# oooolga/Ctrl-V

Hardware: AMD Instinct MI355X
Metric: denoising steps/sec, SVD+ControlNet 25f 576x1024 (higher is better)
Workload: dtype bf16; 1 GPU; box2video: ControlNet + UNet forward, CFG batch 2, 25 frames, latent 72x128, 25-step Karras Euler schedule, random-init SVD-XT weights; clips_per_gpu=1, parallelism=clip-shard x1, hip_graph=True

## Files before the change

ctrlv_amd/_lib.py:

```python
import ctypes
import os
import threading

_HERE = os.path.dirname(os.path.abspath(__file__))
LIB_PATH = os.path.join(_HERE, "lib", "libctrlv_hip.so")
LIB_PATH_F16 = os.path.join(_HERE, "lib", "libctrlv_hip_f16.so")

c_void_p, c_int, c_float, c_size_t = ctypes.c_void_p, ctypes.c_int32, ctypes.c_float, ctypes.c_size_t


class GemmDesc(ctypes.Structure):
    _fields_ = [
        ("A", c_void_p), ("A2", c_void_p), ("W", c_void_p), ("out", c_void_p),
        ("bias", c_void_p), ("R1", c_void_p), ("R2", c_void_p), ("V", c_void_p),
        ("M", c_int), ("N", c_int), ("Cin", c_int), ("taps", c_int),
        ("lda", c_int), ("lda2", c_int), ("c_split", c_int),
        ("mode", c_int),
        ("H", c_int), ("Wd", c_int), ("Ho", c_int), ("Wo", c_int), ("stride", c_int), ("up", c_int),
        ("F", c_int), ("S", c_int),
        ("ldo", c_int), ("n_store", c_int),
        ("ldr1", c_int), ("ldr2", c_int),
        ("s_acc", c_float), ("s1", c_float), ("s2", c_float),
        ("vmode", c_int), ("vdiv", c_int), ("vmod", c_int), ("vS", c_int), ("ldv", c_int),
        ("act", c_int), ("geglu", c_int), ("out_f32", c_int), ("tile", c_int),
# ... 30 lines not shown

class TemporalFusedDesc(ctypes.Structure):
    _fields_ = [
        ("x", c_void_p), ("ldx", c_int), ("wf", c_void_p), ("bias", c_void_p),
        ("R1", c_void_p), ("R1_lo", c_void_p), ("ldr1", c_int),
        ("V", c_void_p), ("vmode", c_int), ("vdiv", c_int), ("vmod", c_int), ("vS", c_int), ("ldv", c_int),
        ("out", c_void_p), ("out_lo", c_void_p), ("ldo", c_int),
        ("B", c_int), ("F", c_int), ("S", c_int), ("C", c_int),
        ("ln_gamma", c_void_p), ("ln_beta", c_void_p), ("ln_eps", c_float),
    ]


class SpatialEntryDesc(ctypes.Structure):
    _fields_ = [
        ("x", c_void_p), ("x_lo", c_void_p), ("ldx", c_int), ("wf", c_void_p),
        ("bias_in", c_void_p), ("bias_qkv", c_void_p), ("stats", c_void_p),
        ("gn_gamma", c_void_p), ("gn_beta", c_void_p),
        ("ln_gamma", c_void_p), ("ln_beta", c_void_p), ("ln_eps", c_float),
        ("h0", c_void_p), ("h0_lo", c_void_p), ("ldh", c_int),
        ("qkv", c_void_p), ("ldq", c_int),
        ("n_img", c_int), ("S", c_int), ("C", c_int), ("head_dim", c_int),
        ("q_scale", c_float),
    ]


class LoraDesc(ctypes.Structure):
    _fields_ = [
        ("X", c_void_p), ("dY", c_void_p), ("A", c_void_p), ("B", c_void_p), ("dA", c_void_p), ("dB", c_void_p),
        ("M", c_int), ("Cin", c_int), ("N", c_int), ("g", c_int), ("r", c_int), ("ldx", c_int), ("ldy", c_int),
        ("scale", c_float),
    ]


class TensorDesc(ctypes.Structure):
    _fields_ = [("name", ctypes.c_char_p), ("data", c_void_p), ("dtype", c_int), ("on_device", c_int),
                ("numel", ctypes.c_int64)]


class GemmTokensDesc(ctypes.Structure):
    _fields_ = [
        ("A", c_void_p), ("W", c_void_p), ("bias", c_void_p), ("R1", c_void_p), ("out", c_void_p),
        ("workspace", c_void_p), ("workspace_bytes", c_size_t),
        ("M", c_int), ("N", c_int), ("K", c_int), ("lda", c_int), ("ldr1", c_int), ("ldo", c_int),
        ("act", c_int), ("ws_zeroed", c_int),
    ]


class ClipConfig(ctypes.Structure):
    _fields_ = [
        ("hidden_size", c_int), ("intermediate_size", c_int), ("num_hidden_layers", c_int), ("num_attention_heads", c_int),
        ("image_size", c_int), ("patch_size", c_int), ("projection_dim", c_int), ("hidden_act", c_int),
        ("layer_norm_eps", c_float),
    ]


class VaeConfig(ctypes.Structure):
    _fields_ = [
        ("in_channels", c_int), ("out_channels", c_int), ("latent_channels", c_int), ("layers_per_block", c_int),
        ("n_blocks", c_int), ("block_out_channels", c_int * CTRLV_MAX_BLOCKS), ("scaling_factor", c_float),
        ("offset_limit_bytes", ctypes.c_int64),
    ]


class ClipRequest(ctypes.Structure):
    _fields_ = [
        ("n_clips", c_int), ("num_frames", c_int), ("height", c_int), ("width", c_int),
        ("image_u8", c_void_p), ("cond", c_void_p), ("cond_channels", c_int), ("cond_dtype", c_int),
        ("aug_noise", c_void_p), ("noise_aug_strength", c_float), ("num_steps", c_int),
        ("latents", c_void_p), ("sigmas", ctypes.POINTER(c_float)), ("timesteps", ctypes.POINTER(c_float)),
        ("fps", c_int), ("motion_bucket_id", c_int),
        ("min_guidance", c_float), ("max_guidance", c_float), ("conditioning_scale", c_float), ("decode_chunk", c_int),
        ("clip_mean", c_float * 3), ("clip_std", c_float * 3),
        ("out_latents", c_void_p), ("out_frames", c_void_p), ("out_frames_u8", c_void_p),
    ]


class BoxCondition(ctypes.Structure):
    _fields_ = [("frames", c_void_p), ("channels", c_int), ("dtype", c_int), ("num_cond_frames", c_int), ("reserved", c_int)]


class TwoStageRequest(ctypes.Structure):
    _fields_ = [("boxes", ClipRequest), ("box_cond", BoxCondition), ("video", ClipRequest), ("out_box_frames_u8", c_void_p),
                ("clean_threshold", c_float), ("reserved", c_int)]


class SeedRequest(ctypes.Structure):
    _fields_ = [("seed", ctypes.c_uint64), ("clip_index0", ctypes.c_uint32), ("call", ctypes.c_uint32),
                ("src_image_u8", c_void_p), ("src_height", c_int), ("src_width", c_int),
                ("sigma_min", c_float), ("sigma_max", c_float),
                ("sigmas_host", ctypes.POINTER(c_float)), ("timesteps_host", ctypes.POINTER(c_float)), ("reserved", c_int)]


class BestBoxesRequest(ctypes.Structure):
    _fields_ = [("n_candidates", c_int), ("reserved", c_int), ("candidates", ctypes.POINTER(ClipRequest)),
                ("box_cond", BoxCondition), ("gt_u8", c_void_p), ("clean_threshold", c_float), ("reserved2", c_int),
                ("out_pt", c_void_p), ("out_cond", c_void_p), ("out_u8", c_void_p), ("out_counts", c_void_p),
                ("out_winner", c_void_p)]


class BestChainRequest(ctypes.Structure):
    _fields_ = [("boxes", BestBoxesRequest), ("video", ClipRequest), ("reserved", c_int)]


class TrainBatchRequest(ctypes.Structure):
    _fields_ = [
        ("n_clips", c_int), ("num_frames", c_int), ("height", c_int), ("width", c_int),
        ("clips", c_void_p), ("box_frames", c_void_p), ("clips_dtype", c_int), ("box_dtype", c_int),
        ("mode", c_int), ("num_cond_frames", c_int), ("dropout_prob", ctypes.c_double),
        ("seed", ctypes.c_uint64), ("clip_index0", ctypes.c_uint32), ("call", ctypes.c_uint32),
        ("sigma_table", c_void_p), ("timestep_table", c_void_p), ("table_size", c_int), ("scaling_factor", c_float),
        ("clip_mean", c_float * 3), ("clip_std", c_float * 3), ("sample_dtype", c_int), ("reserved", c_int),
        ("target_latents", c_void_p), ("noisy_latents", c_void_p), ("sample", c_void_p), ("control_cond", c_void_p),
        ("encoder_hidden_states", c_void_p), ("sigmas", c_void_p), ("timesteps", c_void_p), ("indices", c_void_p),
        ("random_p", c_void_p), ("noise", c_void_p),
    ]


SIGNATURES = {
    "ctrlv_abi_version": (c_int, []),
    "ctrlv_elem_dtype": (c_int, []),
    "ctrlv_build_id": (c_int, [ctypes.c_char_p, c_size_t]),
    "ctrlv_last_error": (c_int, [ctypes.c_char_p, c_size_t]),
    "ctrlv_gemm": (c_int, [ctypes.POINTER(GemmDesc), c_void_p]),
    "ctrlv_gemm_gn_partials_serves": (c_int, [ctypes.POINTER(GemmDesc)]),
    "ctrlv_gemm_splitk_ws_bytes": (c_size_t, [ctypes.POINTER(GemmDesc)]),
    "ctrlv_gemm_up_phase_serves": (c_int, [ctypes.POINTER(GemmDesc)]),
    "ctrlv_pack_up_phase_weight": (c_int, [c_void_p, c_int, c_int, c_int, c_void_p, c_void_p]),
    "ctrlv_groupnorm_from_partials": (c_int, [c_void_p, c_int, c_int, c_int, c_int, c_float, c_void_p, c_void_p, c_void_p,
                                              c_int, c_void_p, c_void_p]),
    "ctrlv_groupnorm_from_partials_split": (c_int, [c_void_p, c_void_p, c_int, c_int, c_int, c_int, c_float, c_void_p, c_void_p, c_void_p,
                                              c_int, c_void_p, c_void_p]),
    "ctrlv_groupnorm_chunks": (c_int, [c_int, c_int, c_int, c_int]),
    "ctrlv_groupnorm_stats_split": (c_int, [c_void_p, c_void_p, c_void_p, c_void_p, c_int, c_int, c_int, c_int, c_int, c_float,
                                            c_void_p, c_void_p]),
    "ctrlv_groupnorm_apply_split": (c_int, [c_void_p, c_void_p, c_void_p, c_void_p, c_int, c_int, c_int, c_int, c_int, c_void_p,
                                            c_void_p, c_void_p, c_int, c_void_p, c_void_p]),
    "ctrlv_layernorm_split": (c_int, [c_void_p, c_void_p, c_int, c_int, c_void_p, c_void_p, c_float, c_void_p, c_int, c_int,
                                      c_int, c_void_p, c_void_p]),
    "ctrlv_axpby_split": (c_int, [c_void_p, c_void_p, c_void_p, c_float, c_float, c_void_p, c_void_p, c_size_t, c_void_p]),
    "ctrlv_plan_set_trunk_mode": (c_int, [c_void_p, c_int]),
    "ctrlv_plan_set_ff_precision": (c_int, [c_void_p, c_int]),
    "ctrlv_groupnorm_stats": (c_int, [c_void_p, c_void_p, c_int, c_int, c_int, c_int, c_int, c_float, c_void_p,
                                      c_void_p]),
    "ctrlv_groupnorm_apply": (c_int, [c_void_p, c_void_p, c_int, c_int, c_int, c_int, c_int, c_void_p, c_void_p,
                                      c_void_p, c_int, c_void_p, c_void_p]),
    "ctrlv_layernorm": (c_int, [c_void_p, c_int, c_int, c_void_p, c_void_p, c_float, c_void_p, c_int, c_int, c_int,
                                c_void_p, c_void_p]),
    "ctrlv_softmax_rows": (c_int, [c_void_p, c_int, c_int, ctypes.c_long, c_void_p, ctypes.c_long, c_void_p]),
    "ctrlv_softmax_rows_bwd": (c_int, [c_void_p, ctypes.c_long, c_void_p, ctypes.c_long, c_int, c_int, c_float, c_void_p,
                                       ctypes.c_long, c_void_p]),
    "ctrlv_ff_fused_w1f_bytes": (c_int, []),
    "ctrlv_ff_fused_pack": (c_int, [c_void_p, c_void_p, c_void_p, c_void_p, c_void_p, c_void_p]),
    "ctrlv_ff_fused_serves": (c_int, [ctypes.POINTER(GemmDesc), c_int]),
    "ctrlv_ff_fused": (c_int, [c_void_p, c_int, c_void_p, c_void_p, ctypes.POINTER(GemmDesc), c_void_p]),
    "ctrlv_ff_fused_ln": (c_int, [c_void_p, c_int, c_void_p, c_void_p, c_float, c_void_p, c_int, c_int, c_int, c_void_p,
                                  c_void_p, ctypes.POINTER(GemmDesc), c_void_p]),
    "ctrlv_quant_rows_f8": (c_int, [c_void_p, c_int, c_int, c_int, c_void_p, c_void_p, c_float, c_void_p, c_int, c_int, c_int,
                                    c_void_p, c_int, c_void_p, c_void_p]),
    "ctrlv_gemm_f8": (c_int, [ctypes.POINTER(GemmDesc), c_void_p, c_void_p, c_void_p]),
    "ctrlv_gemm_f8_serves": (c_int, [ctypes.POINTER(GemmDesc)]),
    "ctrlv_temporal_fused_weight_bytes": (c_size_t, []),
    "ctrlv_temporal_fused_pack": (c_int, [c_void_p, c_int, c_void_p, c_int, c_void_p, c_void_p]),
    "ctrlv_temporal_fused": (c_int, [ctypes.POINTER(TemporalFusedDesc), c_void_p]),
    "ctrlv_temporal_fused_serves": (c_int, [ctypes.POINTER(TemporalFusedDesc)]),
    "ctrlv_spatial_entry_fused_weight_bytes": (c_size_t, []),
    "ctrlv_spatial_entry_fused_pack": (c_int, [c_void_p, c_int, c_void_p, c_int, c_void_p, c_void_p]),
    "ctrlv_spatial_entry_fused": (c_int, [ctypes.POINTER(SpatialEntryDesc), c_void_p]),
    "ctrlv_spatial_entry_fused_serves": (c_int, [ctypes.POINTER(SpatialEntryDesc)]),
    "ctrlv_groupnorm_finalize": (c_int, [c_int, c_int, c_int, c_int, c_float, c_void_p, c_void_p]),
    "ctrlv_attention_spatial": (c_int, [c_void_p, c_void_p, c_int, c_int, c_int, c_void_p]),
    "ctrlv_attention_spatial_prescaled": (c_int, [c_void_p, c_void_p, c_int, c_int, c_int, c_void_p]),
    "ctrlv_attention_temporal": (c_int, [c_void_p, c_void_p, c_int, c_int, c_int, c_int, c_void_p]),
    "ctrlv_attention_spatial_lse": (c_int, [c_void_p, c_void_p, c_void_p, c_int, c_int, c_int, c_void_p]),
    "ctrlv_attention_bwd_scratch_floats": (ctypes.c_size_t, [c_int, c_int, c_int]),
    "ctrlv_attention_spatial_bwd": (c_int, [c_void_p, c_void_p, c_void_p, c_void_p, c_void_p, c_void_p, c_int, c_int, c_int,
                                            c_void_p]),
    "ctrlv_attention_temporal_bwd": (c_int, [c_void_p, c_void_p, c_void_p, c_void_p, c_int, c_int, c_int, c_int, c_void_p]),
    "ctrlv_attention_tokens": (c_int, [c_void_p, c_void_p, c_int, c_int, c_int, c_int, c_void_p]),
    "ctrlv_clip_patch_rows": (c_int, [c_void_p, c_int, c_int, c_int, c_int, c_int, c_void_p, c_int, c_void_p]),
    "ctrlv_clip_tokens": (c_int, [c_void_p, c_void_p, c_void_p, c_int, c_int, c_int, c_void_p, c_void_p]),
    "ctrlv_act_rows": (c_int, [c_void_p, c_int, c_int, c_int, c_int, c_void_p]),
    "ctrlv_gemm_tokens": (c_int, [ctypes.POINTER(GemmTokensDesc), c_void_p]),
    "ctrlv_gemm_tokens_plan": (c_int, [c_int, c_int, ctypes.POINTER(c_int), ctypes.POINTER(c_int)]),
    "ctrlv_gemm_tokens_ws_bytes": (c_size_t, [c_int, c_int, c_int]),
    "ctrlv_nchw_to_rows": (c_int, [c_void_p, c_int, c_int, c_int, c_int, c_void_p, c_int, c_int, c_void_p]),
    "ctrlv_rows_to_nchw": (c_int, [c_void_p, c_int, c_int, c_int, c_int, c_void_p, c_int, c_void_p]),
    "ctrlv_time_conv_rows_to_nchw": (c_int, [c_void_p, c_int, c_int, c_int, c_int, c_void_p, c_void_p, c_void_p, c_int,
                                             c_void_p]),
    "ctrlv_vae_posterior": (c_int, [c_void_p, c_int, c_int, c_int, c_int, c_void_p, c_void_p, c_void_p, c_float, c_void_p,
                                    c_void_p, c_int, c_void_p]),
    "ctrlv_time_conv_rows_to_nchw_bwd": (c_int, [c_void_p, c_void_p, c_int, c_int, c_int, c_int, c_int, c_void_p, c_void_p,
                                                 c_int, c_void_p, c_void_p, c_void_p, c_void_p]),
    "ctrlv_im2col3x3": (c_int, [c_void_p, c_int, c_int, c_int, c_int, c_void_p, c_int, c_void_p]),
    "ctrlv_axpby": (c_int, [c_void_p, c_void_p, c_float, c_float, c_void_p, c_size_t, c_void_p]),
    "ctrlv_timestep_embedding": (c_int, [c_void_p, c_int, c_int, c_void_p, c_void_p]),
    "ctrlv_silu": (c_int, [c_void_p, c_void_p, c_size_t, c_void_p]),
    "ctrlv_cfg_euler_step": (c_int, [c_void_p, c_void_p, c_int, c_int, c_void_p, c_int, c_int, c_int, c_float,
                                     c_float, c_void_p, c_void_p]),
    "ctrlv_pack_weight": (c_int, [c_void_p, c_int, c_int, c_int, c_int, c_int, c_int, c_void_p, c_int, c_void_p]),
    "ctrlv_gemm_wgrad_scratch_bytes": (c_size_t, [ctypes.POINTER(GemmDesc)]),
    "ctrlv_gemm_wgrad": (c_int, [ctypes.POINTER(GemmDesc), c_void_p, c_int, c_void_p, c_void_p, c_float, c_int, c_void_p, c_size_t,
                                 c_void_p]),
    "ctrlv_colsum_scratch_floats": (c_size_t, [c_int, c_int, c_int, c_int]),
    "ctrlv_colsum": (c_int, [c_void_p, c_int, c_int, c_int, c_int, c_int, c_int, c_float, c_void_p, c_int, c_void_p, c_void_p]),
    "ctrlv_dot_diff": (c_int, [c_void_p, c_void_p, c_void_p, c_size_t, c_float, c_void_p, c_void_p, c_void_p]),
    "ctrlv_groupnorm_bwd_scratch_floats": (c_int, [c_int, c_int, c_int, c_int]),
    "ctrlv_groupnorm_bwd": (c_int, [c_void_p, c_void_p, c_int, c_int, c_int, c_int, c_void_p, c_void_p, c_void_p, c_int,
                                    c_void_p, c_void_p, c_void_p, c_void_p, c_void_p]),
    "ctrlv_groupnorm_bwd_add": (c_int, [c_void_p, c_void_p, c_void_p, c_int, c_int, c_int, c_int, c_void_p, c_void_p, c_void_p, c_int,
                                        c_void_p, c_void_p, c_void_p, c_void_p, c_void_p]),
    "ctrlv_layernorm_bwd_add": (c_int, [c_void_p, c_void_p, c_void_p, c_int, c_int, c_void_p, c_float, c_void_p, c_int, c_int, c_int,
                                        c_void_p, c_void_p, c_void_p, c_void_p, c_void_p]),
    "ctrlv_layernorm_bwd_scratch_floats": (ctypes.c_size_t, [c_int, c_int]),
    "ctrlv_layernorm_bwd": (c_int, [c_void_p, c_void_p, c_int, c_int, c_void_p, c_float, c_void_p, c_int, c_int, c_int,
                                    c_void_p, c_void_p, c_void_p, c_void_p, c_void_p]),
    "ctrlv_geglu_bwd": (c_int, [c_void_p, c_void_p, c_size_t, c_int, c_void_p, c_void_p]),
    "ctrlv_lora_grad_scratch_bytes": (c_size_t, [ctypes.POINTER(LoraDesc)]),
    "ctrlv_lora_grad": (c_int, [ctypes.POINTER(LoraDesc), c_void_p, c_size_t, c_void_p]),
    "ctrlv_lora_merge": (c_int, [c_void_p, c_int, c_void_p, c_void_p, c_int, c_int, c_int, c_float, c_void_p, c_void_p]),
    "ctrlv_plan_create": (c_int, [ctypes.POINTER(ModelConfig), c_int, ctypes.POINTER(c_void_p)]),
    "ctrlv_plan_load_weights": (c_int, [c_void_p, ctypes.POINTER(TensorDesc), c_size_t]),
    "ctrlv_plan_set_time_context_order": (c_int, [c_void_p, c_int]),
    "ctrlv_plan_workspace_bytes": (c_size_t, [c_void_p, c_int, c_int, c_int, c_int]),
    "ctrlv_plan_num_down_residuals": (c_int, [c_void_p]),
    "ctrlv_plan_residual_shape": (c_int, [c_void_p, c_int, c_int, c_int, c_int, c_int, ctypes.POINTER(ctypes.c_int64),
                                          ctypes.POINTER(c_int)]),
    "ctrlv_unet_forward": (c_int, [c_void_p, c_void_p, c_int, c_void_p, c_int, c_void_p, c_void_p, c_int,
                                   ctypes.POINTER(c_void_p), c_void_p, c_void_p, c_void_p, c_int, c_int, c_int, c_int,
                                   c_void_p, c_size_t, c_void_p]),
    "ctrlv_unet_encoder_forward": (c_int, [c_void_p, c_void_p, c_int, c_void_p, c_int, c_void_p, c_void_p, c_int,
                                           ctypes.POINTER(c_void_p), c_void_p, c_int, c_int, c_int, c_int, c_void_p,
                                           c_size_t, c_void_p]),
    "ctrlv_controlnet_forward": (c_int, [c_void_p, c_void_p, c_void_p, c_int, c_void_p, c_int, c_void_p, c_void_p, c_int,
                                         c_float, ctypes.POINTER(c_void_p), c_void_p, c_int, c_int, c_int, c_int, c_void_p,
                                         c_size_t, c_void_p]),
    "ctrlv_plan_destroy": (c_int, [c_void_p]),
    "ctrlv_plan_profile": (c_int, [c_void_p, c_int]),
    "ctrlv_plan_profile_read": (c_int, [c_void_p, ctypes.POINTER(ProfileRecord), c_int]),
    "ctrlv_clip_plan_create": (c_int, [ctypes.POINTER(ClipConfig), c_int, ctypes.POINTER(c_void_p)]),
    "ctrlv_clip_plan_load_weights": (c_int, [c_void_p, ctypes.POINTER(TensorDesc), c_size_t]),
    "ctrlv_clip_plan_workspace_bytes": (c_size_t, [c_void_p, c_int]),
    "ctrlv_clip_forward": (c_int, [c_void_p, c_void_p, c_int, c_int, c_void_p, c_void_p, c_void_p, c_size_t, c_void_p]),
    "ctrlv_clip_plan_destroy": (c_int, [c_void_p]),
    "ctrlv_vae_plan_create": (c_int, [ctypes.POINTER(VaeConfig), c_int, ctypes.POINTER(c_void_p)]),
    "ctrlv_vae_plan_load_weights": (c_int, [c_void_p, ctypes.POINTER(TensorDesc), c_size_t]),
    "ctrlv_vae_plan_workspace_bytes": (c_size_t, [c_void_p, c_int, c_int, c_int, c_int, c_int]),
    "ctrlv_vae_encode": (c_int, [c_void_p, c_void_p, c_int, c_int, c_int, c_int, c_void_p, c_float, c_void_p, c_void_p, c_int,
                                 c_void_p, c_size_t, c_void_p]),
    "ctrlv_vae_decode": (c_int, [c_void_p, c_void_p, c_int, c_int, c_int, c_int, c_int, c_void_p, c_int, c_void_p, c_size_t,
                                 c_void_p]),
    "ctrlv_vae_plan_destroy": (c_int, [c_void_p]),
    "ctrlv_resize_antialias": (c_int, [c_void_p, c_int, c_int, c_int, c_int, c_void_p, c_int, c_int, c_int,
                                       ctypes.POINTER(c_float), ctypes.POINTER(c_float), c_void_p]),
    "ctrlv_pixels_prepare": (c_int, [c_void_p, c_void_p, c_float, c_int, c_int, c_int, c_void_p, c_void_p]),
    "ctrlv_frames_to_u8": (c_int, [c_void_p, c_int, c_int, c_int, c_void_p, c_void_p]),
    "ctrlv_pipeline_create": (c_int, [c_void_p, c_void_p, c_void_p, c_void_p, c_int, ctypes.POINTER(c_void_p)]),
    "ctrlv_pipeline_set_overlap": (c_int, [c_void_p, c_int]),
    "ctrlv_pipeline_workspace_bytes": (c_size_t, [c_void_p, ctypes.POINTER(ClipRequest)]),
    "ctrlv_pipeline_generate": (c_int, [c_void_p, ctypes.POINTER(ClipRequest), c_void_p, c_size_t, c_void_p]),
    "ctrlv_pipeline_destroy": (c_int, [c_void_p]),
    "ctrlv_pipeline_boxes_workspace_bytes": (c_size_t, [c_void_p, ctypes.POINTER(ClipRequest), ctypes.POINTER(BoxCondition)]),
    "ctrlv_pipeline_predict_boxes": (c_int, [c_void_p, ctypes.POINTER(ClipRequest), ctypes.POINTER(BoxCondition), c_void_p,
                                             c_size_t, c_void_p]),
    "ctrlv_box_frames_post_ws_bytes": (c_size_t, [c_int, c_int]),
    "ctrlv_box_frames_post": (c_int, [c_void_p, c_int, c_int, c_int, c_int, c_float, c_void_p, c_void_p, c_void_p, c_void_p,
                                      c_size_t, c_void_p]),
    "ctrlv_mask_counts": (c_int, [c_void_p, c_void_p, c_int, c_int, c_int, c_int, c_void_p, c_void_p]),
    "ctrlv_pipeline_chain_workspace_bytes": (c_size_t, [c_void_p, c_void_p, ctypes.POINTER(TwoStageRequest)]),
    "ctrlv_pipeline_boxes_to_video": (c_int, [c_void_p, c_void_p, ctypes.POINTER(TwoStageRequest), c_void_p, c_size_t, c_void_p]),
    "ctrlv_randn": (c_int, [ctypes.c_uint64, ctypes.c_uint32, ctypes.c_uint32, ctypes.c_uint32, c_int, c_size_t, c_float, c_int,
                            c_void_p, c_int, c_void_p]),
    "ctrlv_euler_schedule": (c_int, [c_int, c_float, c_float, ctypes.POINTER(c_float), ctypes.POINTER(c_float),
                                     ctypes.POINTER(ctypes.c_double)]),
    "ctrlv_resize_lanczos_ws_bytes": (c_size_t, [c_int, c_int, c_int, c_int, c_int]),
    "ctrlv_resize_lanczos_u8": (c_int, [c_void_p, c_int, c_int, c_int, c_void_p, c_int, c_int, c_void_p, c_size_t, c_void_p]),
    "ctrlv_pipeline_prepare_bytes": (c_size_t, [c_void_p, ctypes.POINTER(ClipRequest), ctypes.POINTER(SeedRequest)]),
    "ctrlv_pipeline_prepare": (c_int, [c_void_p, ctypes.POINTER(ClipRequest), ctypes.POINTER(SeedRequest),
                                       ctypes.POINTER(ClipRequest), c_void_p, c_size_t, c_void_p]),
    "ctrlv_pipeline_seeded_workspace_bytes": (c_size_t, [c_void_p, ctypes.POINTER(ClipRequest), ctypes.POINTER(SeedRequest)]),
    "ctrlv_pipeline_generate_seeded": (c_int, [c_void_p, ctypes.POINTER(ClipRequest), ctypes.POINTER(SeedRequest), c_void_p,
                                               c_size_t, c_void_p]),
    "ctrlv_best_candidate": (c_int, [c_void_p, c_int, c_int, c_void_p, c_void_p]),
    "ctrlv_gather_clips": (c_int, [c_void_p, c_void_p, c_int, c_int, c_size_t, c_void_p, c_void_p]),
    "ctrlv_pipeline_best_boxes_workspace_bytes": (c_size_t, [c_void_p, ctypes.POINTER(BestBoxesRequest)]),
    "ctrlv_pipeline_best_boxes": (c_int, [c_void_p, ctypes.POINTER(BestBoxesRequest), c_void_p, c_size_t, c_void_p]),
    "ctrlv_pipeline_best_chain_workspace_bytes": (c_size_t, [c_void_p, c_void_p, ctypes.POINTER(BestChainRequest)]),
    "ctrlv_pipeline_best_boxes_to_video": (c_int, [c_void_p, c_void_p, ctypes.POINTER(BestChainRequest), c_void_p, c_size_t,
                                                   c_void_p]),
    "ctrlv_boundary_radius": (c_int, [c_int, c_int, ctypes.c_double]),
    "ctrlv_boundary_counts": (c_int, [c_void_p, c_void_p, c_int, c_int, c_int, c_int, c_int, c_int, c_void_p, c_void_p]),
    "ctrlv_frame_stats": (c_int, [c_void_p, c_void_p, c_int, c_int, c_int, c_int, c_void_p, c_void_p]),
    "ctrlv_frame_ssim_ws_bytes": (c_size_t, [c_int, c_int, c_int, c_int]),
    "ctrlv_frame_ssim": (c_int, [c_void_p, c_void_p, c_int, c_int, c_int, c_int, c_void_p, c_void_p, c_void_p, c_size_t, c_void_p]),
    "ctrlv_resize_frames_ws_bytes": (c_size_t, [c_int, c_int, c_int, c_int, c_int, c_int]),
    "ctrlv_resize_frames_u8": (c_int, [c_void_p, c_int, c_int, c_int, c_void_p, c_int, c_int, c_int, c_void_p, c_size_t, c_void_p]),
    "ctrlv_lpips_im2col_split": (c_int, [c_void_p, c_int, c_int, c_int, c_int, c_int, c_int, c_int, c_int, c_void_p, c_void_p]),
    "ctrlv_lpips_pack_weight": (c_int, [c_void_p, c_int, c_int, c_int, c_int, c_int, c_void_p, c_void_p]),
    "ctrlv_relu_maxpool_rows": (c_int, [c_void_p, c_int, c_int, c_int, c_int, c_int, c_void_p, c_int, c_void_p]),
    "ctrlv_lpips_distance_blocks": (c_int, [c_int]),
    "ctrlv_lpips_layer_distance": (c_int, [c_void_p, c_void_p, c_int, c_void_p, c_int, c_int, c_int, c_void_p, c_void_p]),
    "ctrlv_lpips_finish": (c_int, [c_void_p, c_int, c_int, ctypes.POINTER(c_int), c_void_p, c_void_p]),
    "ctrlv_lpips_plan_create": (c_int, [c_int, ctypes.POINTER(c_void_p)]),
    "ctrlv_lpips_plan_load_weights": (c_int, [c_void_p, ctypes.POINTER(TensorDesc), c_size_t]),
    "ctrlv_lpips_ws_bytes": (c_size_t, [c_void_p, c_int, c_int, c_int]),
    "ctrlv_lpips_frames": (c_int, [c_void_p, c_void_p, c_void_p, c_int, c_int, c_int, c_int, c_int, c_void_p, c_void_p, c_size_t,
                                   c_void_p]),
    "ctrlv_lpips_plan_destroy": (c_int, [c_void_p]),
    "ctrlv_resize_antialias_clamped": (c_int, [c_void_p, c_int, c_int, c_int, c_int, c_void_p, c_int, c_int, c_int,
                                               ctypes.POINTER(c_float), ctypes.POINTER(c_float), c_void_p]),
    "ctrlv_train_draws": (c_int, [ctypes.c_uint64, ctypes.c_uint32, ctypes.c_uint32, c_int, c_void_p, c_void_p, c_int,
                                  ctypes.c_double, c_void_p, c_void_p, c_void_p, c_void_p, c_void_p, c_void_p, c_void_p]),
    "ctrlv_train_assemble": (c_int, [c_void_p, c_void_p, c_void_p, c_void_p, c_void_p, c_void_p, c_int, c_int, c_int, c_int, c_int,
                                     c_int, c_int, ctypes.c_uint64, ctypes.c_uint32, ctypes.c_uint32, c_void_p, c_void_p, c_int,
                                     c_void_p, c_void_p]),
    "ctrlv_train_batch_workspace_bytes": (c_size_t, [c_void_p, c_void_p, ctypes.POINTER(TrainBatchRequest)]),
    "ctrlv_train_batch_prepare": (c_int, [c_void_p, c_void_p, ctypes.POINTER(TrainBatchRequest), c_void_p, c_size_t, c_void_p]),
    "ctrlv_adamw_step": (c_int, [c_void_p, c_void_p, c_void_p, c_void_p, c_void_p, c_size_t, c_float, c_float, c_float, c_float,
                                 c_float, c_float, c_float, c_float, c_float, c_void_p]),
    "ctrlv_ema_step": (c_int, [c_void_p, c_void_p, c_size_t, c_float, c_void_p]),
    "ctrlv_grad_sumsq_partials": (c_size_t, [c_size_t]),
    "ctrlv_grad_sumsq": (c_int, [c_void_p, c_size_t, c_void_p, c_size_t, c_size_t, c_void_p]),
    "ctrlv_grad_finish": (c_int, [c_void_p, c_size_t, c_float, c_float, c_void_p, c_void_p]),
    "ctrlv_adamw_step_dev": (c_int, [c_void_p, c_void_p, c_void_p, c_void_p, c_void_p, c_size_t, c_float, c_float, c_float, c_float,
                                     c_float, c_float, c_float, c_float, c_float, c_void_p, c_void_p]),
    "ctrlv_grad_finish_scaled": (c_int, [c_void_p, c_size_t, c_float, c_float, c_void_p, c_void_p, c_void_p]),
    "ctrlv_adamw_step_scaled": (c_int, [c_void_p, c_void_p, c_void_p, c_void_p, c_void_p, c_size_t, c_float, c_float, c_float, c_float,
                                        c_float, c_float, c_float, c_float, c_void_p, c_void_p, c_void_p]),
}

_libs = {}
_tls = threading.local()
_NO_STATUS = {"ctrlv_abi_version", "ctrlv_elem_dtype", "ctrlv_build_id", "ctrlv_last_error", "ctrlv_ff_fused_w1f_bytes",
              "ctrlv_gemm_gn_partials_serves", "ctrlv_gemm_up_phase_serves", "ctrlv_ff_fused_serves", "ctrlv_plan_num_down_residuals",
              "ctrlv_temporal_fused_serves", "ctrlv_gemm_f8_serves", "ctrlv_spatial_entry_fused_serves",
              "ctrlv_gemm_tokens_ws_bytes", "ctrlv_clip_plan_workspace_bytes", "ctrlv_vae_plan_workspace_bytes",
              "ctrlv_pipeline_workspace_bytes", "ctrlv_pipeline_boxes_workspace_bytes", "ctrlv_box_frames_post_ws_bytes",
              "ctrlv_pipeline_chain_workspace_bytes", "ctrlv_resize_lanczos_ws_bytes", "ctrlv_pipeline_prepare_bytes",
              "ctrlv_pipeline_seeded_workspace_bytes", "ctrlv_pipeline_best_boxes_workspace_bytes",
              "ctrlv_pipeline_best_chain_workspace_bytes", "ctrlv_frame_ssim_ws_bytes", "ctrlv_resize_frames_ws_bytes",
              "ctrlv_train_batch_workspace_bytes", "ctrlv_lpips_ws_bytes",
              "ctrlv_lpips_distance_blocks",
              "ctrlv_boundary_radius"}


def _status_recorder(lib, fn):
    def call(*args):
        rc = fn(*args)
        _tls.failed = lib if rc < 0 else None
        return rc
    call.__name__ = getattr(fn, "__name__", "ctrlv_fn")
    return call
ABI_VERSION = 22


class CtrlvHipError(RuntimeError):
    pass


def source_build_id():
    import hashlib
    csrc = os.path.join(_HERE, "csrc")
    inc = os.path.join(os.path.dirname(_HERE), "include")
    if not os.path.isdir(csrc) or not os.path.isdir(inc):
        return None
    files = [os.path.join(csrc, f) for f in sorted(os.listdir(csrc)) if f.endswith((".hip", ".h"))]
    files += [os.path.join(inc, f) for f in sorted(os.listdir(inc)) if f.endswith(".h")]
    h = hashlib.sha256()
    for f in files:
        h.update(os.path.basename(f).encode() + b"\0")
        h.update(open(f, "rb").read())
    return h.hexdigest()[:16]


def build_id(lib=None):
    buf = ctypes.create_string_buffer(128)
    (lib or load()).ctrlv_build_id(buf, 128)
    return buf.value.decode()


def elem_code(dtype=None):
    if dtype is None or dtype == 2:
        return 2
    if dtype == 1:
        return 1
    name = str(dtype)
    if name == "torch.float16":
        return 1
    if name == "torch.bfloat16":
        return 2
    raise CtrlvHipError(f"ctrlv_amd: activations are stored as bf16 or fp16, not {dtype}")


def load(dtype=None):
    code = elem_code(dtype)
    lib = _libs.get(code)
    if lib is not None:
        return lib
    env = "CTRLV_HIP_LIB" if code == 2 else "CTRLV_HIP_LIB_F16"
    path = os.environ.get(env, LIB_PATH if code == 2 else LIB_PATH_F16)
    if not os.path.exists(path):
        raise CtrlvHipError(
            f"{path} not found: build it with `python -c 'import __graft_entry__ as g; g.build()'` "
            "(hipcc --offload-arch=gfx950).  ctrlv_amd has no CPU / eager fallback.")
    lib = ctypes.CDLL(path)
    for name, (res, args) in SIGNATURES.items():
        fn = getattr(lib, name)
        fn.restype, fn.argtypes = res, args
        if res is c_int and name not in _NO_STATUS:
            setattr(lib, name, _status_recorder(lib, fn))
    if lib.ctrlv_abi_version() != ABI_VERSION:
        raise CtrlvHipError(f"{path}: ABI version {lib.ctrlv_abi_version()}, this host layer needs {ABI_VERSION}")
    if lib.ctrlv_elem_dtype() != code:
        raise CtrlvHipError(f"{path}: element dtype code {lib.ctrlv_elem_dtype()}, expected {code}")
    want = source_build_id()
    if want is not None and env not in os.environ and build_id(lib) != want:
        raise CtrlvHipError(f"{path} is stale: built from sources {build_id(lib)}, tree is {want}; rebuild with "
                            "`python -c 'import __graft_entry__ as g; g.build()'`")
    _libs[code] = lib
    return lib


def last_error(lib=None):
    buf = ctypes.create_string_buffer(512)
    if lib is not None:
        lib.ctrlv_last_error(buf, 512)
        return buf.value.decode("utf-8", "replace")
    msgs = []
    for l in (_libs.values() or [load()]):
        l.ctrlv_last_error(buf, 512)
        if buf.value:
            msgs.append(buf.value.decode("utf-8", "replace"))
    return " | ".join(msgs)


def check(rc, what, lib=None):
    if rc == 0:
        return
    failed, _tls.failed = getattr(_tls, "failed", None), None
    msg = f"{what}: {last_error(lib or failed)} (status {rc})"
    if rc in (-1, -2, -4, -5):
        raise ValueError(msg)
    raise CtrlvHipError(msg)
```

ctrlv_amd/csrc/abi.hip:

```cpp
#include <stdarg.h>
#include <stdlib.h>

#include <mutex>

#include "common.h"

#ifndef CTRLV_BUILD_ID
#define CTRLV_BUILD_ID "unstamped"
#endif

static thread_local char g_err[512] = "";
void ctrlv_set_error(const char* fmt, ...) {
  va_list ap;
  va_start(ap, fmt);
  vsnprintf(g_err, sizeof(g_err), fmt, ap);
  va_end(ap);
}

const ctrlv_debug_t& ctrlv_debug() {
  static const ctrlv_debug_t dbg = [] {
    auto env = [](const char* name, int dflt) { const char* e = getenv(name); return e ? atoi(e) : dflt; };
    ctrlv_debug_t d;
    d.w16 = env("CTRLV_W16", 1);
    d.splitk = env("CTRLV_SPLITK", 1);
    d.force_tile = env("CTRLV_GEMM_FORCE_TILE", 0);
    d.conv_halo = env("CTRLV_CONV_HALO", 1);
    d.gn_fused = env("CTRLV_GN_FUSED", 1);
    d.gn_cross = env("CTRLV_GN_CROSS", 1);
    d.gn_rev = env("CTRLV_GN_REV", 1);
    d.gn_rows = env("CTRLV_GN_ROWS", 256);
    if (d.gn_rows < 32 || d.gn_rows > 1024) d.gn_rows = 256;
    d.ln_rows = env("CTRLV_LN_ROWS", 1);
    d.ff_fused = env("CTRLV_FF_FUSED", 1);
    d.ff_ln = env("CTRLV_FF_LN", 0);
    d.pp_balanced = env("CTRLV_PP_BALANCED", 1);
    d.pp_cgrp = env("CTRLV_PP_CGRP", 0);
    d.attn_rows = env("CTRLV_ATTN_ROWS", 0);
    d.temporal_fused = env("CTRLV_TEMPORAL_FUSED", 1);
    d.wgrad_pp = env("CTRLV_WGRAD_PP", 1);
    d.wgrad_slabs = env("CTRLV_WGRAD_SLABS", 0);
    d.up_phase = env("CTRLV_UP_PHASE", 1);
    d.spatial_entry = env("CTRLV_SPATIAL_ENTRY", 1);
    return d;
  }();
  return dbg;
}

int ctrlv_current_device() {
  int dev = 0;
  if (hipGetDevice(&dev) != hipSuccess || dev < 0 || dev >= CTRLV_MAX_DEVICES) dev = 0;
  return dev;
}

int ctrlv_num_cu(int dev) {
  static int cu[CTRLV_MAX_DEVICES] = {};
  static std::mutex mu;
  std::lock_guard<std::mutex> lk(mu);
  if (cu[dev] == 0) {
    int n = 0;
    if (hipDeviceGetAttribute(&n, hipDeviceAttributeMultiprocessorCount, dev) != hipSuccess || n <= 0) n = 256;
    cu[dev] = n;
  }
  return cu[dev];
}

extern "C" int ctrlv_last_error(char* buf, size_t n) {
  if (buf && n) {
    strncpy(buf, g_err, n - 1);
    buf[n - 1] = 0;
  }
  return (int)strlen(g_err);
}

extern "C" int ctrlv_abi_version(void) { return 22; }
static_assert(sizeof(ctrlv_gemm_desc) == 264 && offsetof(ctrlv_gemm_desc, ld_raw) == 192 && offsetof(ctrlv_gemm_desc, pad_br) == 196 &&
                  offsetof(ctrlv_gemm_desc, raw_out) == 200,
              "ctrlv_gemm_desc layout changed: that is an ABI bump");
extern "C" int ctrlv_elem_dtype(void) { return CTRLV_ELEM_DTYPE; }

extern "C" int ctrlv_build_id(char* buf, size_t n) {
  static const char marker[] = "CTRLV_BUILD_ID=" CTRLV_BUILD_ID;
  const char* id = marker + 15;
  if (buf && n) {
    strncpy(buf, id, n - 1);
    buf[n - 1] = 0;
  }
  return (int)strlen(id);
}
```

ctrlv_amd/csrc/common.h:

```cpp
#pragma once
#include <hip/hip_runtime.h>
#include <stdint.h>
#include <stdio.h>
#include <string.h>

#include "../../include/ctrlv_hip.h"

#ifdef CTRLV_ELEM_F16
typedef _Float16 el_native_t;
#define CTRLV_ELEM_DTYPE 1
#define CTRLV_MFMA_32x32x16_ASM "v_mfma_f32_32x32x16_f16"
#else
typedef __bf16 el_native_t;
#define CTRLV_ELEM_DTYPE 2
#define CTRLV_MFMA_32x32x16_ASM "v_mfma_f32_32x32x16_bf16"
#endif
typedef __attribute__((ext_vector_type(8))) el_native_t elx8;
typedef __attribute__((ext_vector_type(4))) el_native_t elx4;
typedef __attribute__((ext_vector_type(2))) el_native_t elx2;
typedef __attribute__((ext_vector_type(16))) float f32x16;
typedef __attribute__((ext_vector_type(4))) float f32x4;
typedef __attribute__((ext_vector_type(4))) short s16x4;
typedef uint16_t el_t;
typedef uint16_t bf16_t;

#define LDS_PTR(p) ((__attribute__((address_space(3))) void*)(p))
#define GLB_PTR(p) ((const __attribute__((address_space(1))) void*)(p))

static __device__ __attribute__((aligned(256), used)) unsigned char g_ctrlv_zeros[256];

__device__ __forceinline__ f32x16 mfma_32x32x16(const elx8& a, const elx8& b, const f32x16& c) {
#ifdef CTRLV_ELEM_F16
  return __builtin_amdgcn_mfma_f32_32x32x16_f16(a, b, c, 0, 0, 0);
#else
  return __builtin_amdgcn_mfma_f32_32x32x16_bf16(a, b, c, 0, 0, 0);
#endif
}

__device__ __forceinline__ float bf16_to_f32(bf16_t v) { return __uint_as_float(((uint32_t)v) << 16); }
__device__ __forceinline__ bf16_t f32_to_bf16(float f) {
  __bf16 b = (__bf16)f;
  return __builtin_bit_cast(bf16_t, b);
}
#ifdef CTRLV_ELEM_F16
__device__ __forceinline__ float el_to_f32(el_t v) { return (float)__builtin_bit_cast(_Float16, v); }
__device__ __forceinline__ el_t f32_to_el(float f) { return __builtin_bit_cast(el_t, (_Float16)f); }
__device__ __forceinline__ uint32_t pack_elx2(float lo, float hi) {
  typedef _Float16 h2 __attribute__((ext_vector_type(2)));
  const h2 v = {(_Float16)lo, (_Float16)hi};
  return __builtin_bit_cast(uint32_t, v);
}
__device__ __forceinline__ void unpack_elx8(const uint4& v, float* f) {
  typedef _Float16 h2 __attribute__((ext_vector_type(2)));
  const h2 a = __builtin_bit_cast(h2, v.x), b = __builtin_bit_cast(h2, v.y), c = __builtin_bit_cast(h2, v.z),
           d = __builtin_bit_cast(h2, v.w);
  f[0] = (float)a.x; f[1] = (float)a.y; f[2] = (float)b.x; f[3] = (float)b.y;
  f[4] = (float)c.x; f[5] = (float)c.y; f[6] = (float)d.x; f[7] = (float)d.y;
}
#else
__device__ __forceinline__ float el_to_f32(el_t v) { return bf16_to_f32(v); }
__device__ __forceinline__ el_t f32_to_el(float f) { return f32_to_bf16(f); }
__device__ __forceinline__ uint32_t pack_elx2(float lo, float hi) {
  typedef __bf16 b2 __attribute__((ext_vector_type(2)));
  const b2 v = {(__bf16)lo, (__bf16)hi};
  return __builtin_bit_cast(uint32_t, v);
}
__device__ __forceinline__ void unpack_elx8(const uint4& v, float* f) {
  f[0] = __uint_as_float(v.x << 16); f[1] = __uint_as_float(v.x & 0xffff0000u);
  f[2] = __uint_as_float(v.y << 16); f[3] = __uint_as_float(v.y & 0xffff0000u);
  f[4] = __uint_as_float(v.z << 16); f[5] = __uint_as_float(v.z & 0xffff0000u);
  f[6] = __uint_as_float(v.w << 16); f[7] = __uint_as_float(v.w & 0xffff0000u);
}
#endif
__device__ __forceinline__ float el_lo_f32(uint32_t v) { return el_to_f32((el_t)(v & 0xffffu)); }
__device__ __forceinline__ float el_hi_f32(uint32_t v) { return el_to_f32((el_t)(v >> 16)); }
__device__ __forceinline__ uint4 pack_elx8(const float* f) {
  uint4 v;
  v.x = pack_elx2(f[0], f[1]); v.y = pack_elx2(f[2], f[3]);
  v.z = pack_elx2(f[4], f[5]); v.w = pack_elx2(f[6], f[7]);
  return v;
}
typedef uint8_t lo_t;
__device__ __forceinline__ uint2 split_lo8(const float* v, const uint4& hi) {
#pragma clang fp contract(off)
  float h[8], dl[8];
  unpack_elx8(hi, h);
#pragma unroll
  for (int e = 0; e < 8; ++e) dl[e] = v[e] - h[e];
  int w0 = 0, w1 = 0;
  w0 = __builtin_amdgcn_cvt_pk_bf8_f32(dl[0], dl[1], w0, false);
  w0 = __builtin_amdgcn_cvt_pk_bf8_f32(dl[2], dl[3], w0, true);
  w1 = __builtin_amdgcn_cvt_pk_bf8_f32(dl[4], dl[5], w1, false);
  w1 = __builtin_amdgcn_cvt_pk_bf8_f32(dl[6], dl[7], w1, true);
  return make_uint2((unsigned)w0, (unsigned)w1);
}
__device__ __forceinline__ lo_t split_lo1(float v, el_t hi) {
#pragma clang fp contract(off)
  const float dl = v - el_to_f32(hi);
  return (lo_t)(__builtin_amdgcn_cvt_pk_bf8_f32(dl, 0.f, 0, false) & 0xff);
}
__device__ __forceinline__ void unpack_lo4(unsigned w, float* l) {
  typedef float f32x2_lo __attribute__((ext_vector_type(2)));
  const f32x2_lo a = __builtin_amdgcn_cvt_pk_f32_bf8((int)w, false), b = __builtin_amdgcn_cvt_pk_f32_bf8((int)w, true);
  l[0] = a.x; l[1] = a.y; l[2] = b.x; l[3] = b.y;
}
__device__ __forceinline__ unsigned pack_lo4(float l0, float l1, float l2, float l3) {
  int w = 0;
  w = __builtin_amdgcn_cvt_pk_bf8_f32(l0, l1, w, false);
  w = __builtin_amdgcn_cvt_pk_bf8_f32(l2, l3, w, true);
  return (unsigned)w;
}
__device__ __forceinline__ void unpack_lo8(const uint2& lo, float* l) {
  typedef float f32x2_lo __attribute__((ext_vector_type(2)));
  const f32x2_lo a = __builtin_amdgcn_cvt_pk_f32_bf8((int)lo.x, false), b = __builtin_amdgcn_cvt_pk_f32_bf8((int)lo.x, true);
  const f32x2_lo c = __builtin_amdgcn_cvt_pk_f32_bf8((int)lo.y, false), d = __builtin_amdgcn_cvt_pk_f32_bf8((int)lo.y, true);
  l[0] = a.x; l[1] = a.y; l[2] = b.x; l[3] = b.y; l[4] = c.x; l[5] = c.y; l[6] = d.x; l[7] = d.y;
}
__device__ __forceinline__ void add_lo8(float* f, const uint2& lo) {
#pragma clang fp contract(off)
  float l[8];
  unpack_lo8(lo, l);
#pragma unroll
  for (int e = 0; e < 8; ++e) f[e] = f[e] + l[e];
}

__device__ __forceinline__ float silu_f(float x) {
  return x * __builtin_amdgcn_rcpf(1.0f + __builtin_amdgcn_exp2f(-1.44269504088896340736f * x));
}
typedef float f32x2_t __attribute__((ext_vector_type(2)));
typedef float f32x4_t __attribute__((ext_vector_type(4)));
__device__ __forceinline__ f32x4_t fma4(f32x4_t a, f32x4_t b, f32x4_t c) {
  f32x4_t r;
  r.x = __builtin_fmaf(a.x, b.x, c.x); r.y = __builtin_fmaf(a.y, b.y, c.y);
  r.z = __builtin_fmaf(a.z, b.z, c.z); r.w = __builtin_fmaf(a.w, b.w, c.w);
  return r;
}
__device__ __forceinline__ f32x4_t splat4(float v) { return f32x4_t{v, v, v, v}; }
__device__ __forceinline__ f32x4_t gelu_phi4(f32x4_t x) {
#pragma clang fp contract(off)
  f32x4_t xc;
  xc.x = __builtin_amdgcn_fmed3f(x.x, -5.0f, 5.0f);
  xc.y = __builtin_amdgcn_fmed3f(x.y, -5.0f, 5.0f);
  xc.z = __builtin_amdgcn_fmed3f(x.z, -5.0f, 5.0f);
  xc.w = __builtin_amdgcn_fmed3f(x.w, -5.0f, 5.0f);
  const f32x4_t t = fma4(xc * xc, splat4(0.08f), splat4(-1.0f));
  f32x4_t p = fma4(t, splat4(7.353763795e-04f), splat4(-1.676730928e-03f));
  p = fma4(p, t, splat4(1.374596148e-03f));
  p = fma4(p, t, splat4(-2.526916796e-03f));
  p = fma4(p, t, splat4(6.766527425e-03f));
  p = fma4(p, t, splat4(-1.130712498e-02f));
  p = fma4(p, t, splat4(1.623608917e-02f));
  p = fma4(p, t, splat4(-2.321312763e-02f));
  p = fma4(p, t, splat4(3.147675842e-02f));
  p = fma4(p, t, splat4(-4.045128077e-02f));
  p = fma4(p, t, splat4(5.151792988e-02f));
  p = fma4(p, t, splat4(-7.029590756e-02f));
  p = fma4(p, t, splat4(1.413638145e-01f));
  return fma4(xc, p, splat4(0.5f));
}
__device__ __forceinline__ f32x4_t gelu_erf4(f32x4_t x) {
#pragma clang fp contract(off)
  return x * gelu_phi4(x);
}
__device__ __forceinline__ float gelu_phi1(float x) {
#pragma clang fp contract(off)
  const float xc = __builtin_amdgcn_fmed3f(x, -5.0f, 5.0f);
  const float t = __builtin_fmaf(xc * xc, 0.08f, -1.0f);
  float p = __builtin_fmaf(t, 7.353763795e-04f, -1.676730928e-03f);
  p = __builtin_fmaf(p, t, 1.374596148e-03f);
  p = __builtin_fmaf(p, t, -2.526916796e-03f);
  p = __builtin_fmaf(p, t, 6.766527425e-03f);
  p = __builtin_fmaf(p, t, -1.130712498e-02f);
  p = __builtin_fmaf(p, t, 1.623608917e-02f);
  p = __builtin_fmaf(p, t, -2.321312763e-02f);
  p = __builtin_fmaf(p, t, 3.147675842e-02f);
  p = __builtin_fmaf(p, t, -4.045128077e-02f);
  p = __builtin_fmaf(p, t, 5.151792988e-02f);
  p = __builtin_fmaf(p, t, -7.029590756e-02f);
  p = __builtin_fmaf(p, t, 1.413638145e-01f);
  return __builtin_fmaf(xc, p, 0.5f);
}

constexpr int kGeluTabN = 1024;
constexpr int kGeluTabBytes = kGeluTabN * 8;
__device__ __forceinline__ void gelu_table_fill(char* tab, int tid, int nthreads) {
#pragma clang fp contract(off)
  for (int i = tid; i < kGeluTabN; i += nthreads) {
    const float a = gelu_phi1(__builtin_fmaf((float)i, 0.01f, -5.12f));
    const float b = gelu_phi1(__builtin_fmaf((float)(i + 1), 0.01f, -5.12f));
    *(float2*)(tab + i * 8) = make_float2(a, b - a);
  }
}
__device__ __forceinline__ float gelu_phi_tab(float x, const char* tab) {
#pragma clang fp contract(off)
  float t = __builtin_fmaf(x, 100.0f, 512.0f);
  t = __builtin_amdgcn_fmed3f(t, 0.0f, 1023.99994f);
  const float fr = __builtin_amdgcn_fractf(t);
  const int i = (int)t;
  const float2 e = *(const float2*)(tab + i * 8);
  return __builtin_fmaf(fr, e.y, e.x);
}
__device__ __forceinline__ float geglu_tab(float a, float g, const char* tab) {
#pragma clang fp contract(off)
  return a * (g * gelu_phi_tab(g, tab));
}
__device__ __forceinline__ void gelu_tab_lookup(float x, const char* tab, float& fr, float2& e) {
#pragma clang fp contract(off)
  float t = __builtin_fmaf(x, 100.0f, 512.0f);
  t = __builtin_amdgcn_fmed3f(t, 0.0f, 1023.99994f);
  fr = __builtin_amdgcn_fractf(t);
  e = *(const float2*)(tab + (int)t * 8);
}
__device__ __forceinline__ float geglu_tab_finish(float a, float g, float fr, float2 e) {
#pragma clang fp contract(off)
  float phi;
  asm volatile("v_fma_f32 %0, %1, %2, %3" : "=v"(phi) : "v"(fr), "v"(e.y), "v"(e.x));
  return a * (g * phi);
}

typedef __attribute__((ext_vector_type(2))) el_native_t elx2n;
__device__ __forceinline__ float el_pair_sum(elx2n a, float acc) {
  const elx2n ones = {(el_native_t)1.0f, (el_native_t)1.0f};
#ifdef CTRLV_ELEM_F16
  return __builtin_amdgcn_fdot2(a, ones, acc, false);
#else
  return __builtin_amdgcn_fdot2_f32_bf16(a, ones, acc, false);
#endif
}
__device__ __forceinline__ float wave_sum(float v) {
#pragma unroll
  for (int o = 32; o > 0; o >>= 1) v += __shfl_xor(v, o);
  return v;
}
// ... 111 lines not shown
```

ctrlv_amd/csrc/ff_fused.hip:

```cpp
#include <type_traits>

#include "common.h"
#include "gemm_pp_kernel.h"

namespace {

constexpr int kC = 320, kHid = 1280, kChunks = kHid / 16;
constexpr int kTileM = 128;
#ifndef CTRLV_FF_GEA
#define CTRLV_FF_GEA 6
#endif
constexpr int kGeA = CTRLV_FF_GEA;
constexpr int kNQ = 6;
constexpr int kW1Pieces = 21;
constexpr int kW1Slot = kW1Pieces * 1024, kW2Slot = 10 * 1024;
constexpr int kStgOff = 0;
constexpr int kHfOff = kStgOff + 8 * 4096;
constexpr int kW1Off = kHfOff + 16 * 1024;
constexpr int kW2Off = kW1Off + 3 * kW1Slot;
constexpr int kTabOff = kW2Off + 4 * kW2Slot;
constexpr int kSmem = kTabOff + kGeluTabBytes;
static_assert(kSmem <= 160 * 1024, "fused feed-forward tile does not fit the LDS");

struct FfArgs {
  const el_t* x; int ldx;
  const el_t* w1f; const el_t* w2f;
  ctrlv_gemm_desc o;
  const float* vtab; int vdiv, vmod, ldv;
  const float* ln_g; const float* ln_b; float ln_eps;
  const float* lnv; int ln_vdiv, ln_vmod, ln_ldv;
};

template <int EPI, bool LO = false, bool LN = false>
__global__ __launch_bounds__(512) void ff_fused_kernel(const FfArgs a) {
#if defined(__HIP_DEVICE_COMPILE__)
  extern __shared__ __attribute__((aligned(1024))) char smem[];
  const int lane = threadIdx.x & 63;
  const int wid = __builtin_amdgcn_readfirstlane(threadIdx.x >> 6);
  const int rg = wid & 3, hh = wid >> 2;
  const int r32 = lane & 31, hsel = lane >> 5;
  const ctrlv_gemm_desc& d = a.o;
  const int M = d.M;
  const int tiles = (M + kTileM - 1) / kTileM, G = gridDim.x;

  CTRLV_CLOCK_BEGIN();
  gelu_table_fill(smem + kTabOff, threadIdx.x, 512);

  const __amdgpu_buffer_rsrc_t rsW1 = __builtin_amdgcn_make_buffer_rsrc((void*)a.w1f, 0, kChunks * kW1Slot, 0x00020000);
  const __amdgpu_buffer_rsrc_t rsW2 = __builtin_amdgcn_make_buffer_rsrc((void*)a.w2f, 0, kChunks * kW2Slot, 0x00020000);
  const __amdgpu_buffer_rsrc_t rsX = __builtin_amdgcn_make_buffer_rsrc((void*)a.x, 0, (int)((long)d.M * a.ldx * 2), 0x00020000);
  const __amdgpu_buffer_rsrc_t rsB2 = __builtin_amdgcn_make_buffer_rsrc((void*)(d.bias ? d.bias : (const float*)a.w1f), 0,
                                                                         d.bias ? kC * 4 : 0, 0x00020000);
  auto dma_w1 = [&](int chunk, int g) {
    char* s1 = smem + kW1Off + (g % 3) * kW1Slot;
#pragma unroll
    for (int k = 0; k < 6; ++k) {
      const int pi = k * 4 + rg;
      if (pi < kW1Pieces)
        __builtin_amdgcn_raw_ptr_buffer_load_lds(rsW1, LDS_PTR(s1 + pi * 1024), 16, lane * 16, chunk * kW1Slot + pi * 1024, 0, 0);
    }
  };
  auto dma_w2 = [&](int chunk, int g) {
    char* s2 = smem + kW2Off + (g & 3) * kW2Slot;
#pragma unroll
    for (int k = 0; k < 3; ++k) {
      const int pi = k * 4 + rg;
      if (pi < 10)
        __builtin_amdgcn_raw_ptr_buffer_load_lds(rsW2, LDS_PTR(s2 + pi * 1024), 16, lane * 16, chunk * kW2Slot + pi * 1024, 0, 0);
    }
  };
  for (int i = threadIdx.x * 16; i < 4 * kW2Slot; i += 512 * 16) *(uint4*)(smem + kW2Off + i) = make_uint4(0, 0, 0, 0);
  if (hh == 0) dma_w1(0, 0); else dma_w1(1, 1);
  wait_vmcnt<0>();
  __syncthreads();
  const char* tab = smem + kTabOff;
  const unsigned tab_lds = (unsigned)(unsigned long)LDS_PTR(smem + kTabOff);
  char* const hfx = smem + kHfOff + rg * 4096 + lane * 16;
  const unsigned xone1 = hsel == 0 ? (CTRLV_ELEM_DTYPE == 1 ? 0x3C003C00u : 0x3F803F80u) : 0u;

  int gbase = 0;
  elx8 xr[20];
  u32x4_t ini_b, ini_v;
  const __amdgpu_buffer_rsrc_t rsVt = __builtin_amdgcn_make_buffer_rsrc(
      (void*)(a.vtab ? a.vtab : (const float*)a.w1f), 0, a.vtab ? (int)((long)a.vmod * a.ldv * 4) : 0, 0x00020000);
  auto tile_loads = [&](int tile) {
    const int bm = tile * kTileM;
    const unsigned xoff = (unsigned)(bm + rg * 32 + r32) * (unsigned)(a.ldx * 2) + 16 * hsel;
#pragma unroll
    for (int ks = 0; ks < 20; ++ks)
      xr[ks] = __builtin_bit_cast(elx8, __builtin_amdgcn_raw_buffer_load_b128(rsX, xoff, ks * 32, 0));
    const unsigned col4 = lane < 40 ? (unsigned)(hh * 160 + lane * 4) * 4 : 0xFFFFFFFFu;
    ini_b = __builtin_amdgcn_raw_buffer_load_b128(rsB2, col4, 0, 0);
    ini_v = __builtin_amdgcn_raw_buffer_load_b128(rsVt, col4, a.vtab ? ((bm / a.vdiv) % a.vmod) * (a.ldv * 4) : 0, 0);
  };
  tile_loads(blockIdx.x);
  for (int tile = blockIdx.x; tile < tiles; tile += G, gbase += kChunks) {
    const int bm = tile * kTileM;
    const int m = bm + rg * 32 + r32;
#ifdef CTRLV_FF_STAMP
    unsigned long long st_tb; asm volatile("s_memtime %0\n\ts_waitcnt lgkmcnt(0)" : "=s"(st_tb)::"memory");
#endif
    if constexpr (LN) {
      const float* lv = a.lnv ? a.lnv + (long)((m / a.ln_vdiv) % a.ln_vmod) * a.ln_ldv + 8 * hsel : nullptr;
      auto raw8 = [&](int ks, float* f) {
        unpack_elx8(__builtin_bit_cast(uint4, xr[ks]), f);
        if (lv) {
          const float4 p = *(const float4*)(lv + ks * 16), q = *(const float4*)(lv + ks * 16 + 4);
          f[0] += p.x; f[1] += p.y; f[2] += p.z; f[3] += p.w; f[4] += q.x; f[5] += q.y; f[6] += q.z; f[7] += q.w;
        }
      };
      float pilot;
      {
        float f0[8];
        raw8(0, f0);
        pilot = __shfl(f0[0], r32);
      }
      float sm = 0.f, sq = 0.f;
#pragma unroll
      for (int ks = 0; ks < 20; ++ks) {
        float f[8];
        raw8(ks, f);
#pragma unroll
        for (int e = 0; e < 8; ++e) { const float dl = f[e] - pilot; sm += dl; sq += dl * dl; }
        if (ks % 5 == 4) __builtin_amdgcn_sched_barrier(0);
      }
      sm += __shfl_xor(sm, 32);
      sq += __shfl_xor(sq, 32);
      const float dm = sm * (1.0f / kC);
      const float var = sq * (1.0f / kC) - dm * dm;
      const float mean = pilot + dm, rstd = rsqrtf((var > 0.f ? var : 0.f) + a.ln_eps);
      const float* gp = a.ln_g + 8 * hsel;
      const float* bp = a.ln_b + 8 * hsel;
#pragma unroll
      for (int ks = 0; ks < 20; ++ks) {
        float f[8];
        raw8(ks, f);
        const float4 g0 = *(const float4*)(gp + ks * 16), g1 = *(const float4*)(gp + ks * 16 + 4);
        const float4 b0 = *(const float4*)(bp + ks * 16), b1v = *(const float4*)(bp + ks * 16 + 4);
        const float gg[8] = {g0.x, g0.y, g0.z, g0.w, g1.x, g1.y, g1.z, g1.w};
        const float bb[8] = {b0.x, b0.y, b0.z, b0.w, b1v.x, b1v.y, b1v.z, b1v.w};
#pragma unroll
        for (int e = 0; e < 8; ++e) f[e] = (f[e] - mean) * rstd * gg[e] + bb[e];
        uint4 o = pack_elx8(f);
        if (!(m < M)) o = make_uint4(0, 0, 0, 0);
        xr[ks] = __builtin_bit_cast(elx8, o);
        if (ks % 5 == 4) __builtin_amdgcn_sched_barrier(0);
      }
    }
    f32x16 acc[1][5];
    char* const stg = smem + kStgOff + wid * 4096;
    {
      const f32x4 b = __builtin_bit_cast(f32x4, ini_b), w = __builtin_bit_cast(f32x4, ini_v);
      if (lane < 40) *(float4*)(stg + lane * 16) = make_float4(b.x + w.x, b.y + w.y, b.z + w.z, b.w + w.w);
      __builtin_amdgcn_wave_barrier();
#pragma unroll
      for (int i = 0; i < 20; ++i) {
        const int n = i >> 2, q = i & 3;
        const float4 v = *(const float4*)(stg + (n * 32 + 8 * q + 4 * hsel) * 4);
        acc[0][n][4 * q] = v.x; acc[0][n][4 * q + 1] = v.y; acc[0][n][4 * q + 2] = v.z; acc[0][n][4 * q + 3] = v.w;
      }
      asm volatile("s_waitcnt lgkmcnt(0)" ::: "memory");
    }
#ifdef CTRLV_FF_STAMP
#define FSTAMP(v) unsigned long long v; asm volatile("s_memtime %0\n\ts_waitcnt lgkmcnt(0)" : "=s"(v)::"memory")
    unsigned long long st_g1 = 0, st_ge = 0, st_b = 0, st_bar = 0, st_dma = 0, st_tile0;
    { FSTAMP(tt0); st_tile0 = tt0; }
#else
#define FSTAMP(v)
#endif
    elx8 hcur, hprev;
    {
      const uint4 z = make_uint4(0, 0, 0, 0);
      hcur = hprev = __builtin_bit_cast(elx8, z);
    }
    auto geglu_part = [&](auto e0c, auto e1c, const float* av, const float* gv, float* h) {
      constexpr int E0 = decltype(e0c)::value, E1 = decltype(e1c)::value, NE = E1 - E0;
      float fr[NE ? NE : 1];
      f32x2_t te[NE ? NE : 1];
#pragma unroll
      for (int e = 0; e < NE; ++e) {
#pragma clang fp contract(off)
        float tq = __builtin_fmaf(gv[E0 + e], 100.0f, 512.0f);
        tq = __builtin_amdgcn_fmed3f(tq, 0.0f, 1023.99994f);
        fr[e] = __builtin_amdgcn_fractf(tq);
        const unsigned addr = tab_lds + (unsigned)((int)tq) * 8u;
        asm volatile("ds_read_b64 %0, %1" : "=v"(te[e]) : "v"(addr));
      }
      static_assert(NE == 0 || NE == 2 || NE == 4 || NE == 6 || NE == 8, "columns per part");
      if constexpr (NE == 8)
        asm volatile("s_waitcnt lgkmcnt(0)"
                     : "+v"(te[0]), "+v"(te[1]), "+v"(te[2]), "+v"(te[3]), "+v"(te[4]), "+v"(te[5]), "+v"(te[6]), "+v"(te[7]));
      if constexpr (NE == 2) asm volatile("s_waitcnt lgkmcnt(0)" : "+v"(te[0]), "+v"(te[1]));
      if constexpr (NE == 4) asm volatile("s_waitcnt lgkmcnt(0)" : "+v"(te[0]), "+v"(te[1]), "+v"(te[2]), "+v"(te[3]));
      if constexpr (NE == 6)
        asm volatile("s_waitcnt lgkmcnt(0)" : "+v"(te[0]), "+v"(te[1]), "+v"(te[2]), "+v"(te[3]), "+v"(te[4]), "+v"(te[5]));
#pragma unroll
      for (int e = 0; e < NE; ++e) h[E0 + e] = geglu_tab_finish(av[E0 + e], gv[E0 + e], fr[e], make_float2(te[e].x, te[e].y));
    };
    uint32_t hpk[kGeA / 2];
    float ak[kGeA < 8 ? 8 - kGeA : 1], gk[kGeA < 8 ? 8 - kGeA : 1];
    auto seg_g1 = [&](int t) {
      FSTAMP(t0);
      __builtin_amdgcn_s_setprio(2);
      const char* s1 = smem + kW1Off + ((gbase + t) % 3) * kW1Slot + lane * 16;
      elx8 wq[kNQ];
#pragma unroll
      for (int i = 0; i < kNQ; ++i) wq[i] = *(const elx8*)(s1 + i * 1024);
      f32x16 a1;
#pragma unroll
      for (int e = 0; e < 16; ++e) a1[e] = 0.f;
      __builtin_amdgcn_sched_barrier(0);
#pragma unroll
      for (int ks = 0; ks < 21; ++ks) {
        elx8 xf;
        if (ks == 20) {
          unsigned one = xone1;
          asm volatile("" : "+v"(one));
          xf = __builtin_bit_cast(elx8, make_uint4(one, 0, 0, 0));
        } else {
          xf = xr[ks];
        }
        a1 = mfma_32x32x16(wq[ks % kNQ], xf, a1);
        if (ks + kNQ < 21) wq[ks % kNQ] = *(const elx8*)(s1 + (ks + kNQ) * 1024);
        __builtin_amdgcn_sched_barrier(0);
      }
      FSTAMP(t1);
      float av[8], gv[8], h[8];
#pragma unroll
      for (int e = 0; e < 8; ++e) { av[e] = a1[e]; gv[e] = a1[8 + e]; }
      geglu_part(std::integral_constant<int, 0>{}, std::integral_constant<int, kGeA>{}, av, gv, h);
#pragma unroll
      for (int e = 0; e < kGeA / 2; ++e) hpk[e] = pack_elx2(h[2 * e], h[2 * e + 1]);
#pragma unroll
      for (int e = 0; e < 8 - kGeA; ++e) { ak[e] = av[kGeA + e]; gk[e] = gv[kGeA + e]; }
      __builtin_amdgcn_s_setprio(0);
#ifdef CTRLV_FF_STAMP
      FSTAMP(t2);
      st_g1 += t1 - t0; st_ge += t2 - t1;
#endif
    };
    auto seg_ge = [&](int t) {
      FSTAMP(t1b);
      float av[8], gv[8], h[8];
#pragma unroll
      for (int e = 0; e < 8 - kGeA; ++e) { av[kGeA + e] = ak[e]; gv[kGeA + e] = gk[e]; }
      geglu_part(std::integral_constant<int, kGeA>{}, std::integral_constant<int, 8>{}, av, gv, h);
      uint32_t hw[4];
#pragma unroll
      for (int e = 0; e < 4; ++e) hw[e] = e < kGeA / 2 ? hpk[e] : pack_elx2(h[2 * e], h[2 * e + 1]);
      const uint4 hp = make_uint4(hw[0], hw[1], hw[2], hw[3]);
      *(uint4*)(hfx + (t & 3) * 1024) = hp;
      hprev = hcur;
      hcur = __builtin_bit_cast(elx8, hp);
#ifdef CTRLV_FF_STAMP
      FSTAMP(t2);
      st_ge += t2 - t1b;
#endif
    };
    auto seg_dma = [&](int t) {
      FSTAMP(t0);
      dma_w1((t + 2) % kChunks, gbase + t + 2);
      if ((t & 1) == 0) { dma_w2(t, gbase + t); dma_w2(t + 1, gbase + t + 1); }
#ifdef CTRLV_FF_STAMP
      FSTAMP(t1);
      st_dma += t1 - t0;
#endif
    };
    auto seg_b = [&](int j) {
      FSTAMP(t0);
      const int c0 = 2 * j;
      const bool live = j >= 0 && j < kChunks / 2;
      const elx8 hpart = *(const elx8*)(hfx + ((c0 + (hh ^ 1)) & 3) * 1024);
      const char* s2a = smem + kW2Off + ((gbase + c0) & 3) * kW2Slot + (5 * hh) * 1024 + lane * 16;
      const char* s2b = smem + kW2Off + ((gbase + c0 + 1) & 3) * kW2Slot + (5 * hh) * 1024 + lane * 16;
      elx8 vq[6];
#pragma unroll
      for (int i = 0; i < 6; ++i) vq[i] = *(const elx8*)((i < 5 ? s2a + i * 1024 : s2b + (i - 5) * 1024));
      const uint4 hz = make_uint4(0, 0, 0, 0);
      const uint4 hp_u = __builtin_bit_cast(uint4, hpart);
      const uint4 own_u = hh == 0 ? __builtin_bit_cast(uint4, hprev) : __builtin_bit_cast(uint4, hcur);
      const uint4 h0_u = !live ? hz : hh == 0 ? own_u : hp_u;
      const uint4 h1_u = !live ? hz : hh == 0 ? hp_u : own_u;
      const elx8 h0 = __builtin_bit_cast(elx8, h0_u), h1 = __builtin_bit_cast(elx8, h1_u);
      __builtin_amdgcn_sched_barrier(0);
#pragma unroll
      for (int i = 0; i < 10; ++i) {
        acc[0][i % 5] = mfma_32x32x16(vq[i % 6], i < 5 ? h0 : h1, acc[0][i % 5]);
        if (i + 6 < 10) vq[i % 6] = *(const elx8*)(s2b + (i + 6 - 5) * 1024);
        __builtin_amdgcn_sched_barrier(0);
      }
#ifdef CTRLV_FF_STAMP
      FSTAMP(t1);
      st_b += t1 - t0;
#endif
    };
    auto slot_barrier = [&](bool dma_wave) {
      FSTAMP(b0);
      if (dma_wave) wait_vmcnt<0>();
      lds_done_barrier();
#ifdef CTRLV_FF_STAMP
      FSTAMP(b1);
      st_bar += b1 - b0;
#endif
    };
    if (hh == 1) { slot_barrier(true); seg_dma(0); }
    for (int k = 0; k < kChunks / 2; ++k) {
      slot_barrier(false);
      seg_g1(2 * k + hh);
      slot_barrier(true);
      seg_ge(2 * k + hh);
      if (2 * k + 1 + hh < kChunks) seg_dma(2 * k + 1 + hh);
      seg_b(k - 1 + hh);
    }
    tile_loads(tile + G);
    slot_barrier(false);
    if (hh == 0) {
      FSTAMP(b0);
      wait_vmcnt<22>();
      lds_done_barrier();
#ifdef CTRLV_FF_STAMP
      FSTAMP(b1);
      st_bar += b1 - b0;
#endif
    }
    hprev = hcur;
    seg_b(kChunks / 2 - 1 + hh);
#ifdef CTRLV_FF_STAMP
    if (lane == 0 && a.lnv) {
      FSTAMP(tt1);
      unsigned long long* o = (unsigned long long*)a.lnv + ((long)blockIdx.x * 8 + wid) * 8;
      o[0] += st_g1; o[1] += st_ge; o[2] += st_dma; o[3] += st_b; o[4] += st_bar; o[5] += tt1 - st_tile0;
      o[6] += st_tile0 - st_tb;
    }
    unsigned long long st_e0; asm volatile("s_memtime %0\n\ts_waitcnt lgkmcnt(0)" : "=s"(st_e0)::"memory");
#endif
    int lane_e = lane;
    asm volatile("" : "+v"(lane_e));
    gemm_epilogue_lds<1, 5, false, EPI, false, false, LO>(d, acc, bm, 0, rg, hh, 32, 160, lane_e, stg, stg + 1024, stg + 2048,
                                                          stg + 3072, nullptr, tab);
    asm volatile("s_waitcnt lgkmcnt(0)" ::: "memory");
#ifdef CTRLV_FF_STAMP
    if (lane == 0 && a.lnv) {
      asm volatile("s_waitcnt vmcnt(0)" ::: "memory");
      unsigned long long st_e1; asm volatile("s_memtime %0\n\ts_waitcnt lgkmcnt(0)" : "=s"(st_e1)::"memory");
      ((unsigned long long*)a.lnv + ((long)blockIdx.x * 8 + wid) * 8)[7] += st_e1 - st_e0;
    }
#endif
  }
  wait_vmcnt<0>();
  CTRLV_CLOCK_END();
#endif
}

__global__ void ff_pack_kernel(const el_t* __restrict__ w1p, const float* __restrict__ b1, const el_t* __restrict__ w2p,
                               el_t* __restrict__ w1f, el_t* __restrict__ w2f) {
  const long i = (long)blockIdx.x * blockDim.x + threadIdx.x;
  const long n1 = (long)kChunks * kW1Pieces * 64 * 8, n2 = (long)kChunks * 10 * 64 * 8;
  if (i < n1) {
    const int j = i & 7, lane = (i >> 3) & 63;
    const int ks = (int)((i >> 9) % kW1Pieces), chunk = (int)(i / (kW1Pieces * 512));
    el_t v = 0;
    if (ks < 20) {
      v = w1p[(long)(chunk * 32 + (lane & 31)) * kC + ks * 16 + 8 * (lane >> 5) + j];
    } else if (lane < 32 && j < 2) {
      const float b = b1[chunk * 32 + lane];
      const el_t hi = f32_to_el(b);
      v = j == 0 ? hi : f32_to_el(b - el_to_f32(hi));
    }
    w1f[i] = v;
  } else if (i < n1 + n2) {
    const long k = i - n1;
    const int j = k & 7, lane = (k >> 3) & 63;
    const int n = (int)((k >> 9) % 10), chunk = (int)(k / (10 * 512));
    w2f[k] = w2p[(long)(n * 32 + (lane & 31)) * kHid + chunk * 16 + 8 * (j >> 2) + 4 * (lane >> 5) + (j & 3)];
  }
}

template <int EPI, bool LO, bool LN>
int launch_ff_ln(const FfArgs& a, hipStream_t stream) {
  static bool attr_set[CTRLV_MAX_DEVICES] = {};
  auto kfn = ff_fused_kernel<EPI, LO, LN>;
  const int dev = ctrlv_current_device();
  if (!attr_set[dev]) {
    CTRLV_HIP_TRY(hipFuncSetAttribute((const void*)kfn, hipFuncAttributeMaxDynamicSharedMemorySize, kSmem));
    attr_set[dev] = true;
  }
  const int num_cu = ctrlv_num_cu(dev);
  const int tiles = (a.o.M + kTileM - 1) / kTileM;
  int grid = tiles;
  if (tiles > num_cu) {
    const int rounds = (tiles + num_cu - 1) / num_cu;
    grid = (tiles + rounds - 1) / rounds;
  }
  hipLaunchKernelGGL(kfn, dim3(grid), dim3(512), kSmem, stream, a);
  CTRLV_LAUNCH_CHECK();
  return CTRLV_OK;
}

template <int EPI, bool LO = false>
int launch_ff(const FfArgs& a, hipStream_t stream) {
  return a.ln_g ? launch_ff_ln<EPI, LO, true>(a, stream) : launch_ff_ln<EPI, LO, false>(a, stream);
}

}

CTRLV_CLOCK_READER(ff_fused)

extern "C" int ctrlv_ff_fused_w1f_bytes(void) { return kChunks * kW1Slot; }

extern "C" int ctrlv_ff_fused_pack(const void* w1_packed, const float* b1, const void* w2_packed, void* w1f, void* w2f,
                                   ctrlv_stream_t stream) {
  CTRLV_CHECK_ARG(w1_packed && b1 && w2_packed && w1f && w2f, "ctrlv_ff_fused_pack: null pointer");
  const long n = (long)kChunks * (kW1Pieces + 10) * 64 * 8;
  hipLaunchKernelGGL(ff_pack_kernel, dim3((unsigned)((n + 255) / 256)), dim3(256), 0, (hipStream_t)stream,
                     (const el_t*)w1_packed, b1, (const el_t*)w2_packed, (el_t*)w1f, (el_t*)w2f);
  CTRLV_LAUNCH_CHECK();
  return CTRLV_OK;
}

static int ff_check(const ctrlv_gemm_desc& d, int ldx, bool report, bool* fold) {
#define FF_REQ(cond, code, ...)                        \
  do {                                                 \
    if (!(cond)) {                                     \
      if (report) ctrlv_set_error(__VA_ARGS__);        \
      return code;                                     \
    }                                                  \
  } while (0)
  *fold = false;
  FF_REQ(d.out != nullptr, CTRLV_E_BAD_ARG, "ctrlv_ff_fused: null pointer");
  FF_REQ(d.M > 0 && d.N == kC && d.Cin == kHid && d.taps == 1 && d.mode == 0 && ldx >= kC && ldx % 8 == 0, CTRLV_E_BAD_SHAPE,
         "ctrlv_ff_fused: serves M x 320 <- 1280 <- 320 only (N=%d Cin=%d ldx=%d)", d.N, d.Cin, ldx);
  FF_REQ(!d.geglu && !d.act && !d.out_f32 && !d.raw_out && !d.A2 && d.n_scale2 == 0, CTRLV_E_BAD_ARG,
         "ctrlv_ff_fused: plain element-type output only");
  FF_REQ(d.n_store == kC && d.ldo % 8 == 0 && (!d.R1 || d.ldr1 % 8 == 0) && (!d.R2 || d.ldr2 % 8 == 0), CTRLV_E_BAD_SHAPE,
         "ctrlv_ff_fused: n_store must be 320 and the row pitches multiples of 8");
  FF_REQ(d.ldo >= kC && (!d.R1 || d.ldr1 >= kC) && (!d.R2 || d.ldr2 >= kC), CTRLV_E_BAD_SHAPE,
         "ctrlv_ff_fused: a row pitch is smaller than the 320 stored columns (ldo=%d ldr1=%d ldr2=%d)", d.ldo, d.ldr1, d.ldr2);
  const long lim = 0xFFFFFFF0L;
  FF_REQ((long)d.M * d.ldo * 2 <= lim && (long)d.M * ldx * 2 <= lim && (!d.R1 || (long)d.M * d.ldr1 * 2 <= lim) &&
             (!d.R2 || (long)d.M * d.ldr2 * 2 <= lim),
         CTRLV_E_BAD_SHAPE, "ctrlv_ff_fused: operands beyond 32-bit byte offsets");
  FF_REQ(!d.R2 || d.R1, CTRLV_E_BAD_ARG, "ctrlv_ff_fused: R2 without R1");
  if (pp_split_io(d)) {
    FF_REQ(CTRLV_ELEM_DTYPE == 1 && d.R1 && (!d.R1_lo || d.R1) && (!d.R2_lo || d.R2), CTRLV_E_BAD_ARG,
           "ctrlv_ff_fused: split trunk planes need the fp16 element library and an R1 operand");
  }
  if (d.vmode) {
    FF_REQ((d.vmode == 1 || d.vmode == 2) && d.V && d.vdiv > 0 && d.vmod > 0 && d.ldv >= kC && d.ldv % 4 == 0 &&
               (d.vmode == 1 || d.vS > 0),
           CTRLV_E_BAD_ARG, "ctrlv_ff_fused: bad row-vector operand");
    *fold = d.vmode == 1 && d.vdiv % 256 == 0 && d.s_acc == 1.0f;
    FF_REQ(*fold || !d.R2, CTRLV_E_BAD_ARG,
           "ctrlv_ff_fused: R1 + R2 + a row vector is served only in the per-tile form (vmode 1, vdiv %% 256 == 0, s_acc 1)");
    FF_REQ(*fold || !pp_split_io(d), CTRLV_E_BAD_ARG, "ctrlv_ff_fused: split trunk planes with a row vector: per-tile form only");
  }
  return CTRLV_OK;
#undef FF_REQ
}

extern "C" int ctrlv_ff_fused_ln(const void* x, int ldx, const float* ln_gamma, const float* ln_beta, float ln_eps,
                                 const float* ln_V, int ln_vdiv, int ln_vmod, int ln_ldv, const void* w1f, const void* w2f,
                                 const ctrlv_gemm_desc* out_desc, ctrlv_stream_t stream) {
  CTRLV_CHECK_ARG(x && w1f && w2f && out_desc && out_desc->out, "ctrlv_ff_fused: null pointer");
  CTRLV_CHECK_ARG((ln_gamma == nullptr) == (ln_beta == nullptr), "ctrlv_ff_fused: LayerNorm needs gamma and beta");
#ifndef CTRLV_FF_STAMP
  CTRLV_CHECK_ARG(!ln_V || (ln_gamma && ln_vdiv > 0 && ln_vmod > 0 && ln_ldv >= 320 && ln_ldv % 4 == 0),
                  "ctrlv_ff_fused: bad LayerNorm row-vector table");
#endif
  FfArgs a;
  a.ln_g = ln_gamma; a.ln_b = ln_beta; a.ln_eps = ln_eps;
  a.lnv = ln_V; a.ln_vdiv = ln_V ? ln_vdiv : 1; a.ln_vmod = ln_V ? ln_vmod : 1; a.ln_ldv = ln_ldv;
  a.x = (const el_t*)x; a.ldx = ldx; a.w1f = (const el_t*)w1f; a.w2f = (const el_t*)w2f;
  a.o = *out_desc;
  a.vtab = nullptr; a.vdiv = 1; a.vmod = 1; a.ldv = 0;
  bool fold = false;
  const int rc = ff_check(a.o, ldx, true, &fold);
  if (rc != CTRLV_OK) return rc;
  if (fold) {
    a.vtab = a.o.V; a.vdiv = a.o.vdiv; a.vmod = a.o.vmod; a.ldv = a.o.ldv;
    a.o.vmode = 0; a.o.V = nullptr;
  }
  const ctrlv_gemm_desc& d = a.o;
  hipStream_t st = (hipStream_t)stream;
#ifdef CTRLV_ELEM_F16
  if (pp_split_io(d)) {
    if (pp_epi_of(d) == 2) return launch_ff<2, true>(a, st);
    if (pp_epi_of(d) == 6) return launch_ff<6, true>(a, st);
  }
#endif
  switch (pp_split_io(d) ? -1 : pp_epi_of(d)) {
    case 0: return launch_ff<0>(a, st);
    case 1: return launch_ff<1>(a, st);
    case 2: return launch_ff<2>(a, st);
    case 3: return launch_ff<3>(a, st);
    case 6: return launch_ff<6>(a, st);
    default: break;
  }
  ctrlv_set_error("ctrlv_ff_fused: epilogue operand combination not served (bias [+ V], + R1 [+ V], + R1 + R2 [+ a per-tile V])");
  return CTRLV_E_BAD_ARG;
}

extern "C" int ctrlv_ff_fused(const void* x, int ldx, const void* w1f, const void* w2f,
                              const ctrlv_gemm_desc* out_desc, ctrlv_stream_t stream) {
  return ctrlv_ff_fused_ln(x, ldx, nullptr, nullptr, 0.f, nullptr, 1, 1, 0, w1f, w2f, out_desc, stream);
}

extern "C" int ctrlv_ff_fused_serves(const ctrlv_gemm_desc* out_desc, int ldx) {
  if (!out_desc) return 0;
  bool fold = false;
  if (ff_check(*out_desc, ldx, false, &fold) != CTRLV_OK) return 0;
  return (out_desc->act || (out_desc->out_f32 & 1)) ? 0 : 1;
}
```

ctrlv_amd/csrc/norm.hip:

```cpp
#include <stdlib.h>

#include "common.h"

namespace {

struct GnShape {
  int n_img, S, C, imgs_per_stat, c_split, n_chunks, rows_per_chunk, CV, RPP;
  int rev_stats, rev_apply;
};

__device__ __forceinline__ uint4 gn_load(const el_t* x, const el_t* x2, int c_split, int C, long row, int c0) {
  if (x2 != nullptr && c0 >= c_split) return *(const uint4*)(x2 + row * (C - c_split) + (c0 - c_split));
  const int ld = x2 != nullptr ? c_split : C;
  return *(const uint4*)(x + row * ld + c0);
}
struct GnLo { const lo_t* x; const lo_t* x2; };
__device__ __forceinline__ const lo_t* gn_lo_plane(const GnLo& lo, const el_t* x2, int c_split, int C, int c0, int* ld, int* first) {
  if (x2 != nullptr && c0 >= c_split) { *ld = C - c_split; *first = c_split; return lo.x2; }
  *ld = x2 != nullptr ? c_split : C; *first = 0;
  return lo.x;
}

template <bool SPLIT>
__global__ void gn_stats_kernel(const el_t* __restrict__ x, const el_t* __restrict__ x2, GnLo lo, GnShape s,
// ... 229 lines not shown
        }
#pragma unroll
        for (int e = 0; e < 8; ++e) s += f[k][e];
      }
    }
    const float mean = wave_sum(s) * inv_c;
    float q = 0.f;
#pragma unroll
    for (int k = 0; k < NV; ++k) {
      const int cv = lane + k * 64;
      if (cv < CV) {
#pragma unroll
        for (int e = 0; e < 8; ++e) { const float dlt = f[k][e] - mean; q += dlt * dlt; }
      }
    }
    const float rstd = rsqrtf(wave_sum(q) * inv_c + eps);
#pragma unroll
    for (int k = 0; k < NV; ++k) {
      const int cv = lane + k * 64;
      if (cv < CV) {
        float o[8];
#pragma unroll
        for (int e = 0; e < 8; ++e) o[e] = (f[k][e] - mean) * rstd * g[k][e] + b[k][e];
        *(uint4*)(y + m * C + cv * 8) = pack_elx8(o);
      }
    }
  }
}

constexpr int kSmxPer = 64;
__global__ __launch_bounds__(256) void softmax_rows_kernel(const float* __restrict__ s, int cols, long lds, el_t* __restrict__ p,
                                                           long ldp) {
  __shared__ float red[8];
  const float* row = s + (long)blockIdx.x * lds;
  el_t* out = p + (long)blockIdx.x * ldp;
  const int tid = threadIdx.x, lane = tid & 63, wid = tid >> 6;
  float v[kSmxPer];
  float mx = -INFINITY;
#pragma unroll
  for (int k = 0; k < kSmxPer; k += 4) {
    const int c = (k / 4 * 256 + tid) * 4;
    float4 q = make_float4(-INFINITY, -INFINITY, -INFINITY, -INFINITY);
    if (c < cols) q = *(const float4*)(row + c);
    v[k] = q.x; v[k + 1] = q.y; v[k + 2] = q.z; v[k + 3] = q.w;
    mx = fmaxf(fmaxf(mx, fmaxf(q.x, q.y)), fmaxf(q.z, q.w));
  }
#pragma unroll
  for (int o = 32; o > 0; o >>= 1) mx = fmaxf(mx, __shfl_xor(mx, o));
  if (lane == 0) red[wid] = mx;
  __syncthreads();
  mx = fmaxf(fmaxf(red[0], red[1]), fmaxf(red[2], red[3]));
  float sum = 0.f;
#pragma unroll
  for (int k = 0; k < kSmxPer; ++k) {
    v[k] = __builtin_amdgcn_exp2f((v[k] - mx) * 1.44269504088896340736f);
    sum += v[k];
  }
  sum = wave_sum(sum);
  if (lane == 0) red[4 + wid] = sum;
  __syncthreads();
  const float inv = 1.0f / ((red[4] + red[5]) + (red[6] + red[7]));
#pragma unroll
  for (int k = 0; k < kSmxPer; k += 4) {
    const int c = (k / 4 * 256 + tid) * 4;
    if (c < cols)
      *(uint2*)(out + c) = make_uint2(pack_elx2(v[k] * inv, v[k + 1] * inv), pack_elx2(v[k + 2] * inv, v[k + 3] * inv));
  }
}

__global__ __launch_bounds__(256) void softmax_rows_bwd_kernel(const el_t* __restrict__ p, long ldp, const float* __restrict__ dp,
                                                               long lddp, int cols, float scale, el_t* __restrict__ ds,
                                                               long ldds) {
  __shared__ float red[4];
  const el_t* prow = p + (long)blockIdx.x * ldp;
  const float* grow = dp + (long)blockIdx.x * lddp;
  el_t* out = ds + (long)blockIdx.x * ldds;
  const int tid = threadIdx.x, lane = tid & 63, wid = tid >> 6;
  float pv[kSmxPer], g[kSmxPer];
  float sum = 0.f;
#pragma unroll
  for (int k = 0; k < kSmxPer; k += 4) {
    const int c = (k / 4 * 256 + tid) * 4;
    uint2 q = make_uint2(0, 0);
    float4 d = make_float4(0.f, 0.f, 0.f, 0.f);
    if (c < cols) { q = *(const uint2*)(prow + c); d = *(const float4*)(grow + c); }
    pv[k] = el_lo_f32(q.x); pv[k + 1] = el_hi_f32(q.x); pv[k + 2] = el_lo_f32(q.y); pv[k + 3] = el_hi_f32(q.y);
    g[k] = d.x; g[k + 1] = d.y; g[k + 2] = d.z; g[k + 3] = d.w;
#pragma unroll
    for (int e = 0; e < 4; ++e) sum = __builtin_fmaf(pv[k + e], g[k + e], sum);
  }
  sum = wave_sum(sum);
  if (lane == 0) red[wid] = sum;
  __syncthreads();
  const float delta = (red[0] + red[1]) + (red[2] + red[3]);
#pragma unroll
  for (int k = 0; k < kSmxPer; k += 4) {
    const int c = (k / 4 * 256 + tid) * 4;
    if (c < cols)
      *(uint2*)(out + c) = make_uint2(pack_elx2(scale * pv[k] * (g[k] - delta), scale * pv[k + 1] * (g[k + 1] - delta)),
                                      pack_elx2(scale * pv[k + 2] * (g[k + 2] - delta), scale * pv[k + 3] * (g[k + 3] - delta)));
  }
}

template <int NCH, bool SPLIT>
__global__ __launch_bounds__(256) void ln_rows_kernel(const el_t* __restrict__ x, const lo_t* __restrict__ xlo, int M, int C, int lpr_log2,
                                                      const float* __restrict__ gamma, const float* __restrict__ beta,
                                                      float eps, const float* __restrict__ V, int vdiv, int vmod, int ldv,
                                                      el_t* __restrict__ y) {
  extern __shared__ float gb[];
  for (int i = threadIdx.x; i < C; i += 256) { gb[i] = gamma[i]; gb[C + i] = beta[i]; }
  __syncthreads();
  const int lane = threadIdx.x & 63, wid = threadIdx.x >> 6;
  const int LPR = 1 << lpr_log2, RPW = 64 >> lpr_log2;
  const int j = lane & (LPR - 1), rsub = lane >> lpr_log2;
  const float inv_c = 1.0f / (float)C;
  const long step = (long)gridDim.x * 4 * RPW;
  long m = ((long)blockIdx.x * 4 + wid) * RPW + rsub;
  uint4 nxt[NCH];
  uint2 nxl[SPLIT ? NCH : 1];
#pragma unroll
  for (int k = 0; k < NCH; ++k) {
    nxt[k] = m < M ? *(const uint4*)(x + m * C + (j + k * LPR) * 8) : make_uint4(0, 0, 0, 0);
    if (SPLIT) nxl[k] = m < M ? *(const uint2*)(xlo + m * C + (j + k * LPR) * 8) : make_uint2(0, 0);
  }
  for (; m - rsub < M; m += step) {
    uint4 cur[NCH];
    uint2 cul[SPLIT ? NCH : 1];
#pragma unroll
    for (int k = 0; k < NCH; ++k) {
      cur[k] = nxt[k];
      nxt[k] = (m + step < M) ? *(const uint4*)(x + (m + step) * C + (j + k * LPR) * 8) : make_uint4(0, 0, 0, 0);
      if (SPLIT) {
        cul[k] = nxl[k];
        nxl[k] = (m + step < M) ? *(const uint2*)(xlo + (m + step) * C + (j + k * LPR) * 8) : make_uint2(0, 0);
      }
    }
    const bool ok = m < M;
    const float* vrow = (V && ok) ? V + (long)((m / vdiv) % vmod) * ldv : nullptr;
    float f[NCH][8];
    float sm = 0.f;
#pragma unroll
    for (int k = 0; k < NCH; ++k) {
      unpack_elx8(cur[k], f[k]);
      if (SPLIT) add_lo8(f[k], cul[k]);
      if (vrow) {
        const float4 a = *(const float4*)(vrow + (j + k * LPR) * 8), b = *(const float4*)(vrow + (j + k * LPR) * 8 + 4);
        f[k][0] += a.x; f[k][1] += a.y; f[k][2] += a.z; f[k][3] += a.w;
        f[k][4] += b.x; f[k][5] += b.y; f[k][6] += b.z; f[k][7] += b.w;
      }
#pragma unroll
      for (int e = 0; e < 8; ++e) sm += f[k][e];
    }
    for (int o = LPR >> 1; o > 0; o >>= 1) sm += __shfl_xor(sm, o);
    const float mean = sm * inv_c;
    float sq = 0.f;
#pragma unroll
    for (int k = 0; k < NCH; ++k)
#pragma unroll
      for (int e = 0; e < 8; ++e) { const float dl = f[k][e] - mean; sq += dl * dl; }
    for (int o = LPR >> 1; o > 0; o >>= 1) sq += __shfl_xor(sq, o);
    const float rstd = rsqrtf(sq * inv_c + eps);
    if (ok) {
#pragma unroll
      for (int k = 0; k < NCH; ++k) {
        const int c0 = (j + k * LPR) * 8;
        const float4 g0 = *(const float4*)(gb + c0), g1 = *(const float4*)(gb + c0 + 4);
        const float4 b0 = *(const float4*)(gb + C + c0), b1 = *(const float4*)(gb + C + c0 + 4);
        const float gg[8] = {g0.x, g0.y, g0.z, g0.w, g1.x, g1.y, g1.z, g1.w};
        const float bb[8] = {b0.x, b0.y, b0.z, b0.w, b1.x, b1.y, b1.z, b1.w};
        float o[8];
#pragma unroll
        for (int e = 0; e < 8; ++e) o[e] = (f[k][e] - mean) * rstd * gg[e] + bb[e];
        *(uint4*)(y + m * C + c0) = pack_elx8(o);
      }
    }
  }
}

}

extern "C" int ctrlv_softmax_rows(const float* scores, int rows, int cols, long ld_scores, void* probs, long ld_probs,
                                  ctrlv_stream_t stream) {
  CTRLV_CHECK_ARG(scores && probs, "softmax_rows: null pointer");
  CTRLV_CHECK_SHAPE(rows > 0 && cols > 0 && cols % 4 == 0 && cols <= kSmxPer * 256 && ld_scores % 4 == 0 && ld_probs % 4 == 0,
                    "softmax_rows: cols=%d must be a multiple of 4, <= %d", cols, kSmxPer * 256);
  hipLaunchKernelGGL(softmax_rows_kernel, dim3(rows), dim3(256), 0, (hipStream_t)stream, scores, cols, ld_scores,
                     (el_t*)probs, ld_probs);
  CTRLV_LAUNCH_CHECK();
  return CTRLV_OK;
}

extern "C" int ctrlv_softmax_rows_bwd(const void* probs, long ld_probs, const float* dprobs, long ld_dprobs, int rows, int cols,
                                      float scale, void* dscores, long ld_dscores, ctrlv_stream_t stream) {
  CTRLV_CHECK_ARG(probs && dprobs && dscores, "softmax_rows_bwd: null pointer");
  CTRLV_CHECK_SHAPE(rows > 0 && cols > 0 && cols % 4 == 0 && cols <= kSmxPer * 256 && ld_probs % 4 == 0 && ld_dprobs % 4 == 0 &&
                        ld_dscores % 4 == 0 && ld_probs >= cols && ld_dprobs >= cols && ld_dscores >= cols,
                    "softmax_rows_bwd: cols=%d must be a multiple of 4, <= %d, pitches multiples of 4 and >= cols", cols,
                    kSmxPer * 256);
  hipLaunchKernelGGL(softmax_rows_bwd_kernel, dim3(rows), dim3(256), 0, (hipStream_t)stream, (const el_t*)probs, ld_probs,
                     dprobs, ld_dprobs, cols, scale, (el_t*)dscores, ld_dscores);
  CTRLV_LAUNCH_CHECK();
  return CTRLV_OK;
}

extern "C" int ctrlv_groupnorm_chunks(int n_img, int S, int C, int imgs_per_stat) {
  GnShape s;
  int rc = gn_shape(n_img, S, C, imgs_per_stat, 0, false, &s);
  return rc < 0 ? rc : s.n_chunks;
}

extern "C" int ctrlv_groupnorm_stats(const void* x, const void* x2, int c_split, int n_img, int S, int C,
                                     int imgs_per_stat, float eps, float* partials, ctrlv_stream_t stream) {
  return ctrlv_groupnorm_stats_split(x, nullptr, x2, nullptr, c_split, n_img, S, C, imgs_per_stat, eps, partials, stream);
}
extern "C" int ctrlv_groupnorm_stats_split(const void* x, const void* x_lo, const void* x2, const void* x2_lo, int c_split,
                                           int n_img, int S, int C, int imgs_per_stat, float eps, float* partials,
                                           ctrlv_stream_t stream) {
  CTRLV_CHECK_ARG(x && partials, "groupnorm_stats: null pointer");
  CTRLV_CHECK_ARG(x2 || !x2_lo, "groupnorm_stats: x2_lo without x2");
  const GnLo lo{(const lo_t*)x_lo, (const lo_t*)x2_lo};
  GnShape s;
  int rc = gn_shape(n_img, S, C, imgs_per_stat, c_split, x2 != nullptr, &s);
  if (rc < 0) return rc;
  const int nt = s.CV * s.RPP;
  const size_t smem = ((size_t)s.RPP * C * 2 + C) * sizeof(float);
  if (x_lo || x2_lo)
    hipLaunchKernelGGL(gn_stats_kernel<true>, dim3(s.n_chunks, n_img), dim3(nt), smem, (hipStream_t)stream,
                       (const el_t*)x, (const el_t*)x2, lo, s, partials);
  else
    hipLaunchKernelGGL(gn_stats_kernel<false>, dim3(s.n_chunks, n_img), dim3(nt), smem, (hipStream_t)stream,
                       (const el_t*)x, (const el_t*)x2, lo, s, partials);
  CTRLV_LAUNCH_CHECK();
  hipLaunchKernelGGL(gn_finalize_kernel, dim3(n_img / imgs_per_stat, 32 / kFinGroups), dim3(1024), 0, (hipStream_t)stream, s,
                     partials, eps, partials + (size_t)n_img * s.n_chunks * 64);
  CTRLV_LAUNCH_CHECK();
  return CTRLV_OK;
}

extern "C" int ctrlv_groupnorm_apply(const void* x, const void* x2, int c_split, int n_img, int S, int C,
                                     int imgs_per_stat, const float* partials, const float* gamma, const float* beta,
                                     int silu, void* y, ctrlv_stream_t stream) {
  return ctrlv_groupnorm_apply_split(x, nullptr, x2, nullptr, c_split, n_img, S, C, imgs_per_stat, partials, gamma, beta, silu,
                                     y, stream);
}
extern "C" int ctrlv_groupnorm_apply_split(const void* x, const void* x_lo, const void* x2, const void* x2_lo, int c_split,
                                           int n_img, int S, int C, int imgs_per_stat, const float* partials,
                                           const float* gamma, const float* beta, int silu, void* y, ctrlv_stream_t stream) {
  CTRLV_CHECK_ARG(x && partials && gamma && beta && y, "groupnorm_apply: null pointer");
  CTRLV_CHECK_ARG(x2 || !x2_lo, "groupnorm_apply: x2_lo without x2");
  const GnLo lo{(const lo_t*)x_lo, (const lo_t*)x2_lo};
  GnShape s;
  int rc = gn_shape(n_img, S, C, imgs_per_stat, c_split, x2 != nullptr, &s);
  if (rc < 0) return rc;
  const int nt = s.CV * s.RPP;
  if (x_lo || x2_lo)
    hipLaunchKernelGGL(gn_apply_kernel<true>, dim3(s.n_chunks, n_img), dim3(nt), 0, (hipStream_t)stream, (const el_t*)x,
                       (const el_t*)x2, lo, s, partials + (size_t)n_img * s.n_chunks * 64, gamma, beta, silu, (el_t*)y);
  else
    hipLaunchKernelGGL(gn_apply_kernel<false>, dim3(s.n_chunks, n_img), dim3(nt), 0, (hipStream_t)stream, (const el_t*)x,
                       (const el_t*)x2, lo, s, partials + (size_t)n_img * s.n_chunks * 64, gamma, beta, silu, (el_t*)y);
  CTRLV_LAUNCH_CHECK();
  return CTRLV_OK;
}

extern "C" int ctrlv_groupnorm_from_partials(const void* x, int n_img, int S, int C, int imgs_per_stat, float eps,
                                             float* partials, const float* gamma, const float* beta, int silu, void* y,
                                             ctrlv_stream_t stream) {
  return ctrlv_groupnorm_from_partials_split(x, nullptr, n_img, S, C, imgs_per_stat, eps, partials, gamma, beta, silu, y, stream);
}
extern "C" int ctrlv_groupnorm_from_partials_split(const void* x, const void* x_lo, int n_img, int S, int C, int imgs_per_stat,
                                                   float eps, float* partials, const float* gamma, const float* beta, int silu,
                                                   void* y, ctrlv_stream_t stream) {
  CTRLV_CHECK_ARG(x && partials && gamma && beta && y, "groupnorm_from_partials: null pointer");
  CTRLV_CHECK_SHAPE(S > 0 && S % 64 == 0, "groupnorm_from_partials: S=%d must be a multiple of 64", S);
  GnShape s;
  int rc = gn_shape(n_img, S, C, imgs_per_stat, 0, false, &s);
  if (rc < 0) return rc;
  GnShape sp = s;
  sp.rows_per_chunk = 64;
  sp.n_chunks = S / 64;
  float* stats = partials + (size_t)n_img * sp.n_chunks * 64;
  hipLaunchKernelGGL(gn_finalize_kernel, dim3(n_img / imgs_per_stat, 32 / kFinGroups), dim3(1024), 0, (hipStream_t)stream, sp,
                     partials, eps, stats);
  CTRLV_LAUNCH_CHECK();
  const int nt = s.CV * s.RPP;
  if (x_lo)
    hipLaunchKernelGGL(gn_apply_kernel<true>, dim3(s.n_chunks, n_img), dim3(nt), 0, (hipStream_t)stream, (const el_t*)x,
                       (const el_t*)nullptr, GnLo{(const lo_t*)x_lo, nullptr}, s, stats, gamma, beta, silu, (el_t*)y);
  else
    hipLaunchKernelGGL(gn_apply_kernel<false>, dim3(s.n_chunks, n_img), dim3(nt), 0, (hipStream_t)stream, (const el_t*)x,
                       (const el_t*)nullptr, GnLo{nullptr, nullptr}, s, stats, gamma, beta, silu, (el_t*)y);
  CTRLV_LAUNCH_CHECK();
  return CTRLV_OK;
}

extern "C" int ctrlv_groupnorm_finalize(int n_img, int S, int C, int imgs_per_stat, float eps, float* partials,
                                        ctrlv_stream_t stream) {
  CTRLV_CHECK_ARG(partials, "groupnorm_finalize: null pointer");
  CTRLV_CHECK_SHAPE(S > 0 && S % 64 == 0, "groupnorm_finalize: S=%d must be a multiple of 64", S);
  GnShape sp;
  int rc = gn_shape(n_img, S, C, imgs_per_stat, 0, false, &sp);
  if (rc < 0) return rc;
  sp.rows_per_chunk = 64;
  sp.n_chunks = S / 64;
  hipLaunchKernelGGL(gn_finalize_kernel, dim3(n_img / imgs_per_stat, 32 / kFinGroups), dim3(1024), 0, (hipStream_t)stream, sp,
                     partials, eps, partials + (size_t)n_img * sp.n_chunks * 64);
  CTRLV_LAUNCH_CHECK();
  return CTRLV_OK;
}

extern "C" int ctrlv_layernorm(const void* x, int M, int C, const float* gamma, const float* beta, float eps,
                               const float* V, int vdiv, int vmod, int ldv, void* y, ctrlv_stream_t stream) {
  return ctrlv_layernorm_split(x, nullptr, M, C, gamma, beta, eps, V, vdiv, vmod, ldv, y, stream);
}
extern "C" int ctrlv_layernorm_split(const void* x, const void* x_lo, int M, int C, const float* gamma, const float* beta,
                                     float eps, const float* V, int vdiv, int vmod, int ldv, void* y, ctrlv_stream_t stream) {
  CTRLV_CHECK_ARG(x && gamma && beta && y, "layernorm: null pointer");
  CTRLV_CHECK_SHAPE(M > 0 && C > 0 && C % 8 == 0 && C <= 2048, "layernorm: C=%d must be a multiple of 8, <= 2048", C);
  if (V) CTRLV_CHECK_ARG(vdiv > 0 && vmod > 0 && ldv >= C, "layernorm: bad row-vector table");
  const int nv = (C / 8 + 63) / 64;
  hipStream_t st = (hipStream_t)stream;
  const int rows_path = ctrlv_debug().ln_rows;
  const int lpr = C / 40;
  if (rows_path && C % 40 == 0 && (lpr == 8 || lpr == 16 || lpr == 32) && (!V || (ldv % 4 == 0 && ((uintptr_t)V & 15) == 0))) {
    const int lg = lpr == 8 ? 3 : (lpr == 16 ? 4 : 5), rpb = 4 * (64 >> lg);
// ... 27 lines not shown
```

ctrlv_amd/csrc/plan.hip:

```cpp
#include <math.h>

#include <string>
#include <vector>

#include "plan_walk.h"
#include "weight_loader.h"

namespace {

using ctrlv_load::WeightLoader;
using ctrlv_walk::conv2d;
using ctrlv_walk::conv_t;
using ctrlv_walk::DeviceScope;
using ctrlv_walk::resid;
using Linear = ctrlv_load::PackedLinear;
using Norm = ctrlv_load::NormParams;

__global__ void arange_kernel(float* dst, int n) {
  const int i = blockIdx.x * blockDim.x + threadIdx.x;
  if (i < n) dst[i] = (float)i;
}
__global__ void expand_f32_kernel(const float* __restrict__ src, int n_src, float* __restrict__ dst, int n) {
  const int i = blockIdx.x * blockDim.x + threadIdx.x;
  if (i < n) dst[i] = src[n_src == 1 ? 0 : i];
// ... 341 lines not shown
              float eps, int silu, el_t* y) {
  const int chunks = ctrlv_groupnorm_chunks(n_img, S, C, ips);
  if (chunks < 0) return chunks;
  const size_t m = c.mark();
  float* part = (float*)c.alloc(((size_t)n_img * chunks + n_img / ips) * 64 * 4);
  const int rc = c.launch(gn_work(n_img, S, C, 0), [&]() -> int {
    CTRLV_TRY(ctrlv_groupnorm_stats_split(x.hi, x.lo, x2.hi, x2.lo, c_split, n_img, S, C, ips, eps, part, c.st));
    return ctrlv_groupnorm_apply_split(x.hi, x.lo, x2.hi, x2.lo, c_split, n_img, S, C, ips, part, nm.g, nm.b, silu, y, c.st);
  });
  c.release(m);
  return rc;
}
int gemm_groupnorm(Ctx& c, ctrlv_gemm_desc d, int n_img, int S, int C, int ips, const Norm& nm, float eps, int silu, el_t* y) {
  const Trk dout{(el_t*)d.out, (lo_t*)d.out_lo};
  if (S % 64 != 0) {
    CTRLV_TRY(gemm(c, d));
    return groupnorm(c, dout, Trk{}, 0, n_img, S, C, ips, nm, eps, silu, y);
  }
  const size_t m = c.mark();
  float* part = (float*)c.alloc(((size_t)n_img * (S / 64) + n_img / ips) * 64 * 4);
  if (!c.dry && ctrlv_gemm_gn_partials_serves(&d)) {
    d.gn_partials = part;
    int rc = gemm(c, d);
    if (rc == CTRLV_OK)
      rc = c.launch(gn_work(n_img, S, C, 1), [&] {
        return ctrlv_groupnorm_from_partials_split(d.out, d.out_lo, n_img, S, C, ips, eps, part, nm.g, nm.b, silu, y, c.st);
      });
    c.release(m);
    return rc;
  }
  c.release(m);
  CTRLV_TRY(gemm(c, d));
  return groupnorm(c, dout, Trk{}, 0, n_img, S, C, ips, nm, eps, silu, y);
}
int layernorm(Ctx& c, const Trk& x, int M, int C, const Norm& nm, el_t* y, const float* V = nullptr, int vdiv = 1,
              int vmod = 1 << 30, int ldv = 0) {
  return c.launch({CTRLV_FAM_LAYERNORM, 0.0, 2.0 * 2 * (double)M * C, M, C},
                  [&] { return ctrlv_layernorm_split(x.hi, x.lo, M, C, nm.g, nm.b, 1e-5f, V, vdiv, vmod, ldv, y, c.st); });
}

int run_res(Ctx& c, const ResBlock& r, const Trk& x, const Trk& x2, int c1, int H, int W, Trk* out_,
            bool feeds_norm = false) {
  const int N = c.B * c.F, S = H * W, F = c.F;
  const long M = (long)N * S;
  const int cin = r.cin, cout = r.cout;
  c.gn_cross_valid = false;
  if (feeds_norm && S % 64 == 0) {
    const size_t need = ((size_t)N * (S / 64) + N) * 64;
    if (c.gn_cross_floats < need) { c.gn_cross = (float*)c.alloc(need * 4); c.gn_cross_floats = need; }
  }
  const Trk out = c.trunk(M, cout);
  const size_t mk = c.mark();
  const int lda_x = x2.hi ? c1 : cin;
  el_t* xn = c.rows(M, cin);
  CTRLV_TRY(groupnorm(c, x, x2, x2.hi ? c1 : 0, N, S, cin, 1, r.n1, r.eps, 1, xn));
  el_t* h = c.rows(M, cout);
  el_t* hn = nullptr;
  {
    ctrlv_gemm_desc d = ctrlv_linear_desc(xn, cin, r.c1, h, cout, (int)M, cout, cin, cout);
    conv2d(d, H, W, H, W);
    d.V = c.temb + r.temb_off[0]; d.ldv = c.ldtemb; d.vmode = 1; d.vdiv = F * S;
    hn = c.rows(M, cout);
    CTRLV_TRY(gemm_groupnorm(c, d, N, S, cout, 1, r.n2, r.eps, 1, hn));
  }
  Trk res = x;
  int ldres = cin;
  if (r.has_sc) {
    const Trk rs = c.trunk(M, cout);
    ctrlv_gemm_desc d = ctrlv_linear_desc(x.hi, lda_x, r.sc, rs.hi, cout, (int)M, cout, cin, cout);
    set_out(d, rs);
    if (x2.hi) { d.A2 = x2.hi; d.lda2 = cin - c1; d.c_split = c1; }
    CTRLV_TRY(gemm(c, d));
    res = rs;
    ldres = cout;
  }
  const Trk xs = c.trunk(M, cout);
  {
    ctrlv_gemm_desc d = ctrlv_linear_desc(hn, cout, r.c2, xs.hi, cout, (int)M, cout, cout, cout);
    conv2d(d, H, W, H, W);
    set_out(d, xs);
    set_r1(d, res, ldres);
    CTRLV_TRY(gemm_groupnorm(c, d, N, S, cout, F, r.tn1, r.eps, 1, hn));
  }
  {
    ctrlv_gemm_desc d = ctrlv_linear_desc(hn, cout, r.tc1, h, cout, (int)M, cout, cout, cout);
    conv_t(d, F, S);
    d.V = c.temb + r.temb_off[1]; d.ldv = c.ldtemb; d.vmode = 1; d.vdiv = F * S;
    CTRLV_TRY(gemm_groupnorm(c, d, N, S, cout, F, r.tn2, r.eps, 1, hn));
  }
  {
    ctrlv_gemm_desc d = ctrlv_linear_desc(hn, cout, r.tc2, out.hi, cout, (int)M, cout, cout, cout);
    conv_t(d, F, S);
    d.s_acc = (float)(1.0 - r.alpha);
    set_out(d, out);
    set_r1(d, xs, cout);
    if (feeds_norm && S % 64 == 0 && !c.dry && ctrlv_gemm_gn_partials_serves(&d)) {
      d.gn_partials = c.gn_cross;
      c.gn_cross_valid = true;
    }
    CTRLV_TRY(gemm(c, d));
  }
  c.release(mk);
  *out_ = out;
  return CTRLV_OK;
}

int frame_embedding(Ctx& c, const Transformer& t, int F, float* e) {
  const int C = t.C, kp = t.tpe1.k;
  const size_t mk = c.mark();
  float* ar = (float*)c.alloc((size_t)F * 4);
  el_t* te = c.rows(F, kp);
  el_t* hh = c.rows(F, 4 * C);
  el_t* tmp = kp != C ? c.rows(F, C) : nullptr;
  CTRLV_TRY(c.launch({}, [&]() -> int {
    hipLaunchKernelGGL(arange_kernel, dim3((F + 63) / 64), dim3(64), 0, c.st, ar, F);
    CTRLV_LAUNCH_CHECK();
    if (kp == C) return ctrlv_timestep_embedding(ar, F, C, te, c.st);
    CTRLV_HIP_TRY(hipMemsetAsync(te, 0, (size_t)F * kp * 2, c.st));
    CTRLV_TRY(ctrlv_timestep_embedding(ar, F, C, tmp, c.st));
    CTRLV_HIP_TRY(hipMemcpy2DAsync(te, (size_t)kp * 2, tmp, (size_t)C * 2, (size_t)C * 2, F, hipMemcpyDeviceToDevice, c.st));
    return CTRLV_OK;
  }));
  {
    ctrlv_gemm_desc d = ctrlv_linear_desc(te, kp, t.tpe1, hh, 4 * C, F, t.tpe1.n, kp, 4 * C);
    d.act = 1;
    CTRLV_TRY(gemm(c, d));
  }
  {
    ctrlv_gemm_desc d = ctrlv_linear_desc(hh, 4 * C, t.tpe2, e, C, F, t.tpe2.n, 4 * C, C);
    d.out_f32 = 1;
    CTRLV_TRY(gemm(c, d));
  }
  c.release(mk);
  return CTRLV_OK;
}

int ff_pair(Ctx& c, const FeedFwd& f, ctrlv_gemm_desc proj, ctrlv_gemm_desc outd, int C, el_t** u) {
  if (ctrlv_debug().ff_fused && f.w1f && ctrlv_ff_fused_serves(&outd, proj.lda)) {
    return c.launch({CTRLV_FAM_GEMM_LINEAR, 2.0 * outd.M * 320.0 * (2560 + 1280),
                     (double)outd.M * 320 * (2 * (2 + (outd.R1 ? 1 : 0) + (outd.R2 ? 1 : 0)) + (outd.R1_lo ? 1 : 0) + (outd.R2_lo ? 1 : 0) +
                                             (outd.out_lo ? 1 : 0)), outd.M, 320, 320, 0x100},
                    [&] { return ctrlv_ff_fused(proj.A, proj.lda, f.w1f, f.w2f, &outd, c.st); });
  }
  if (*u == nullptr) *u = c.rows(proj.M, 4 * C);
  proj.out = *u;
  outd.A = *u;
  CTRLV_TRY(gemm(c, proj));
  CTRLV_TRY(gemm(c, outd));
  return CTRLV_OK;
}

int ln_ff(Ctx& c, const FeedFwd& f, const Norm& nm, const Trk& xraw, const float* lnV, int lnvdiv, int lnvmod, int lnldv,
          el_t* tt, const ctrlv_gemm_desc& proj, const ctrlv_gemm_desc& outd, int C, el_t** u) {
  if (ctrlv_debug().ff_fused && ctrlv_debug().ff_ln && f.w1f && !xraw.lo && ctrlv_ff_fused_serves(&outd, C)) {
    return c.launch({CTRLV_FAM_GEMM_LINEAR, 2.0 * outd.M * 320.0 * (2560 + 1280),
                     (double)outd.M * 320 * 2 * (2 + (outd.R1 ? 1 : 0) + (outd.R2 ? 1 : 0)), outd.M, 320, 320, 0x300}, [&] {
      return ctrlv_ff_fused_ln(xraw.hi, C, nm.g, nm.b, 1e-5f, lnV, lnvdiv, lnvmod, lnldv, f.w1f, f.w2f, &outd, c.st);
    });
  }
  if (c.p->ff_precision == 1 && f.proj8 && f.out8 && !xraw.lo) {
    ctrlv_gemm_desc p8 = proj, o8 = outd;
    p8.W = f.proj8; o8.W = f.out8; o8.lda = 4 * C; o8.S = 0;
    if (ctrlv_gemm_f8_serves(&p8) && ctrlv_gemm_f8_serves(&o8)) {
      if (*u == nullptr) *u = c.rows(proj.M, 4 * C);
      const size_t mk = c.mark();
      const long M = proj.M;
      uint8_t* q = (uint8_t*)c.alloc((size_t)M * 4 * C);
      float* qs = (float*)c.alloc((size_t)M * 4);
      p8.A = q; p8.lda = C; p8.out = *u;
      o8.A = q; o8.lda = 4 * C;
      int rc = c.launch({CTRLV_FAM_LAYERNORM, 0.0, 3.0 * (double)M * C, (int)M, C, 0, 0x400}, [&] {
        return ctrlv_quant_rows_f8(xraw.hi, (int)M, C, C, nm.g, nm.b, 1e-5f, lnV, lnvdiv, lnvmod, lnldv, q, C, qs, c.st);
      });
      if (rc == CTRLV_OK)
        rc = c.launch({CTRLV_FAM_GEMM_LINEAR, 2.0 * M * 8.0 * C * C, (double)M * C + (double)M * 4 * C * 2 + 8.0 * C * C, (int)M, 8 * C, C, 0x401},
                      [&] { return ctrlv_gemm_f8(&p8, qs, f.proj8_s, c.st); });
      if (rc == CTRLV_OK)
        rc = c.launch({CTRLV_FAM_LAYERNORM, 0.0, 3.0 * (double)M * 4 * C, (int)M, 4 * C, 0, 0x400}, [&] {
          return ctrlv_quant_rows_f8(*u, (int)M, 4 * C, 4 * C, nullptr, nullptr, 0.f, nullptr, 1, 1, 0, q, 4 * C, qs, c.st);
        });
      if (rc == CTRLV_OK)
        rc = c.launch({CTRLV_FAM_GEMM_LINEAR, 2.0 * M * 4.0 * C * C,
                       (double)M * 4 * C + (double)M * C * 2 * (1 + (o8.R1 ? 1 : 0) + (o8.R2 ? 1 : 0)) + 4.0 * C * C, (int)M, C, 4 * C,
                       0x400 | ((o8.R1 ? 1 : 0) + (o8.R2 ? 1 : 0)) << 1 | o8.vmode << 3},
                      [&] { return ctrlv_gemm_f8(&o8, qs, f.out8_s, c.st); });
      c.release(mk);
      return rc;
    }
  }
  CTRLV_TRY(layernorm(c, xraw, proj.M, C, nm, tt, lnV, lnvdiv, lnvmod, lnldv));
  return ff_pair(c, f, proj, outd, C, u);
}

int run_tr(Ctx& c, const Transformer& t, const Trk& x, int H, int W, Trk* out_) {
  const int B = c.B, F = c.F, C = t.C, N = B * F, S = H * W;
  const long M = (long)N * S;
  const Trk out = c.trunk(M, C);
  const size_t mk = c.mark();
  const float* emb = t.frame_emb;
  if (F != c.p->cfg.num_frames || emb == nullptr) {
    float* e = (float*)c.alloc((size_t)F * C * 4);
    CTRLV_TRY(frame_embedding(c, t, F, e));
    emb = e;
  }
  el_t* tt = c.rows(M, C);
  Trk h0;
  el_t* qkv = nullptr;
  ctrlv_spatial_entry_desc sd;
  memset(&sd, 0, sizeof(sd));
  sd.ldx = C; sd.ldh = C; sd.ldq = 3 * C; sd.n_img = N; sd.S = S; sd.C = C; sd.head_dim = 64;
  const bool split = c.p->trunk_mode == 1;
  const bool entry_fused = ctrlv_debug().spatial_entry && t.se_wf && !split && ctrlv_spatial_entry_fused_serves(&sd);
  if (entry_fused) {
    h0 = c.trunk(M, C);
    qkv = c.rows(M, 3 * C);
    const size_t mk2 = c.mark();
    if (c.gn_cross_valid) {
      c.gn_cross_valid = false;
      CTRLV_TRY(c.launch({CTRLV_FAM_GROUPNORM, 0.0, 0.0, N * S, C, 0, 3},
                         [&] { return ctrlv_groupnorm_finalize(N, S, C, 1, 1e-6f, c.gn_cross, c.st); }));
      sd.stats = c.gn_cross + (size_t)N * (S / 64) * 64;
    } else {
      const int chunks = ctrlv_groupnorm_chunks(N, S, C, 1);
      if (chunks < 0) return chunks;
      float* part = (float*)c.alloc(((size_t)N * chunks + N) * 64 * 4);
      CTRLV_TRY(c.launch({CTRLV_FAM_GROUPNORM, 0.0, 2.0 * (double)M * C, N * S, C, 0, 2},
                         [&] { return ctrlv_groupnorm_stats_split(x.hi, nullptr, nullptr, nullptr, 0, N, S, C, 1, 1e-6f, part, c.st); }));
      sd.stats = part + (size_t)N * chunks * 64;
    }
    sd.x = x.hi; sd.wf = t.se_wf; sd.bias_in = t.pin.b; sd.bias_qkv = t.s_qkv.b;
    sd.gn_gamma = t.gn.g; sd.gn_beta = t.gn.b; sd.ln_gamma = t.s_ln1.g; sd.ln_beta = t.s_ln1.b; sd.ln_eps = 1e-5f;
    sd.h0 = h0.hi; sd.qkv = qkv; sd.q_scale = 0.125f * 1.44269504088896340736f;
    CTRLV_TRY(c.launch({CTRLV_FAM_GEMM_SPATIAL_ENTRY, 2.0 * M * C * 4.0 * C, (double)M * C * 2 * 5, (int)M, 4 * C, C},
                       [&] { return ctrlv_spatial_entry_fused(&sd, c.st); }));
    c.release(mk2);
  } else {
    if (c.gn_cross_valid) {
      c.gn_cross_valid = false;
      CTRLV_TRY(c.launch(gn_work(N, S, C, 1), [&] {
        return ctrlv_groupnorm_from_partials_split(x.hi, x.lo, N, S, C, 1, 1e-6f, c.gn_cross, t.gn.g, t.gn.b, 0, tt, c.st);
      }));
    } else {
      CTRLV_TRY(groupnorm(c, x, Trk{}, 0, N, S, C, 1, t.gn, 1e-6f, 0, tt));
    }
    h0 = c.trunk(M, C);
    {
      ctrlv_gemm_desc d = ctrlv_linear_desc(tt, C, t.pin, h0.hi, C, (int)M, C, C, C);
      set_out(d, h0);
      CTRLV_TRY(gemm(c, d));
    }
    CTRLV_TRY(layernorm(c, h0, (int)M, C, t.s_ln1, tt));
    qkv = c.rows(M, 3 * C);
    {
      ctrlv_gemm_desc d = ctrlv_linear_desc(tt, C, t.s_qkv, qkv, 3 * C, (int)M, 3 * C, C, 3 * C);
      d.n_scale2 = C; d.s_acc2 = 0.125f * 1.44269504088896340736f;
      CTRLV_TRY(gemm(c, d));
    }
  }
  el_t* a = c.rows(M, C);
  CTRLV_TRY(c.launch({CTRLV_FAM_ATTENTION_SPATIAL, 4.0 * N * (C / 64) * (double)S * S * 64, 2.0 * 4 * N * (double)S * C, N, S, C},
                     [&] { return ctrlv_attention_spatial_prescaled(qkv, a, N, S, C, c.st); }));
  const Trk h1 = c.trunk(M, C);
  {
    ctrlv_gemm_desc d = ctrlv_linear_desc(a, C, t.s_o, h1.hi, C, (int)M, C, C, C);
    set_out(d, h1);
    set_r1(d, h0, C);
    d.V = c.xattn + t.xattn_off[0]; d.ldv = c.ldx; d.vmode = 1; d.vdiv = F * S;
    CTRLV_TRY(gemm(c, d));
  }
  el_t* u = nullptr;
  const Trk h2 = h0;
  {
    ctrlv_gemm_desc dp = ctrlv_linear_desc(tt, C, t.s_ff.proj, u, 4 * C, (int)M, 8 * C, C, 4 * C);
    dp.geglu = 1;
    ctrlv_gemm_desc d = ctrlv_linear_desc(u, 4 * C, t.s_ff.out, h2.hi, C, (int)M, C, 4 * C, C);
    set_out(d, h2);
    set_r1(d, h1, C);
    d.S = S;
    CTRLV_TRY(ln_ff(c, t.s_ff, t.s_ln3, h1, nullptr, 1, 1 << 30, 0, tt, dp, d, C, &u));
  }
  const Trk g0 = h1;
  {
    ctrlv_gemm_desc dp = ctrlv_linear_desc(tt, C, t.t_ffin.proj, u, 4 * C, (int)M, 8 * C, C, 4 * C);
    dp.geglu = 1;
    ctrlv_gemm_desc d = ctrlv_linear_desc(u, 4 * C, t.t_ffin.out, g0.hi, C, (int)M, C, 4 * C, C);
    set_out(d, g0);
    set_r1(d, h2, C);
    d.S = S;
    d.V = emb; d.ldv = C; d.vmode = 1; d.vdiv = S; d.vmod = F;
    CTRLV_TRY(ln_ff(c, t.t_ffin, t.t_lnin, h2, emb, S, F, C, tt, dp, d, C, &u));
  }
  const Trk g1 = c.trunk(M, C);
  {
    ctrlv_temporal_fused_desc fd;
    memset(&fd, 0, sizeof(fd));
    fd.x = tt; fd.ldx = C; fd.wf = t.t_wf; fd.bias = t.t_o.b;
    const bool fuse = ctrlv_debug().temporal_fused && t.t_wf;
    bool ln_in = fuse;
    if (ln_in) { fd.x = g0.hi; fd.ln_gamma = t.t_ln1.g; fd.ln_beta = t.t_ln1.b; fd.ln_eps = 1e-5f; }
    fd.R1 = g0.hi; fd.R1_lo = g0.lo; fd.ldr1 = C;
    fd.V = c.xattn + t.xattn_off[1]; fd.ldv = c.ldx; fd.vdiv = F * S; fd.vS = 1; fd.vmod = 1 << 30;
    if (c.quirk && B > 1) { fd.vmode = 2; fd.vS = S; fd.vmod = B; }
    else fd.vmode = 1;
    fd.out = g1.hi; fd.out_lo = g1.lo; fd.ldo = C;
    fd.B = B; fd.F = F; fd.S = S; fd.C = C;
    const bool fused = fuse && ctrlv_temporal_fused_serves(&fd);
    if (!fused || !ln_in) {
      if (ln_in) { ln_in = false; fd.x = tt; fd.ln_gamma = fd.ln_beta = nullptr; }
      CTRLV_TRY(layernorm(c, t.t_wf ? Trk{g0.hi, nullptr} : g0, (int)M, C, t.t_ln1, tt));
    }
    if (fused) {
      CTRLV_TRY(c.launch({CTRLV_FAM_GEMM_TEMPORAL_BLOCK, 2.0 * M * C * 4.0 * C + 4.0 * B * S * (C / 64) * (double)F * F * 64,
                          (double)M * C * (2 * (ln_in ? 2 : 3) + (g0.lo ? 1 : 0) + (g1.lo ? 1 : 0)), (int)M, 4 * C, C, ln_in ? 1 : 0},
                         [&] { return ctrlv_temporal_fused(&fd, c.st); }));
    } else {
      CTRLV_TRY(gemm(c, ctrlv_linear_desc(tt, C, t.t_qkv, qkv, 3 * C, (int)M, 3 * C, C, 3 * C)));
      CTRLV_TRY(c.launch({CTRLV_FAM_ATTENTION_TEMPORAL, 4.0 * B * S * (C / 64) * (double)F * F * 64, 2.0 * 4 * B * F * (double)S * C, B * S, F, C},
                         [&] { return ctrlv_attention_temporal(qkv, a, B, F, S, C, c.st); }));
      ctrlv_gemm_desc d = ctrlv_linear_desc(a, C, t.t_o, g1.hi, C, (int)M, C, C, C);
      set_out(d, g1);
      set_r1(d, g0, C);
      d.V = fd.V; d.ldv = fd.ldv; d.vdiv = fd.vdiv; d.vmode = fd.vmode;
      if (fd.vmode == 2) { d.vS = S; d.vmod = B; }
      CTRLV_TRY(gemm(c, d));
    }
  }
  const Trk h3 = g0;
  {
    ctrlv_gemm_desc dp = ctrlv_linear_desc(tt, C, t.t_ff.proj, u, 4 * C, (int)M, 8 * C, C, 4 * C);
    dp.geglu = 1;
    ctrlv_gemm_desc d = ctrlv_linear_desc(u, 4 * C, t.t_ff.out, h3.hi, C, (int)M, C, 4 * C, C);
    set_out(d, h3);
    d.s_acc = (float)(1.0 - t.alpha); d.s1 = (float)(1.0 - t.alpha); d.s2 = (float)t.alpha; d.S = S;
    set_r1(d, g1, C);
    set_r2(d, h2, C);
    CTRLV_TRY(ln_ff(c, t.t_ff, t.t_ln3, g1, nullptr, 1, 1 << 30, 0, tt, dp, d, C, &u));
  }
  {
    ctrlv_gemm_desc d = ctrlv_linear_desc(h3.hi, C, t.pout, out.hi, C, (int)M, C, C, C);
    set_out(d, out);
    set_r1(d, x, C);
// ... 564 lines not shown
```

ctrlv_amd/models/blocks.py:

```python
import math
import os

import torch
from torch import nn

from .. import ops, packing
from ..lora import merged_weight


class FwdCtx:

    def __init__(self, ws, B, F, temb, xattn, time_context_order):
        self.ws, self.B, self.F = ws, B, F
        self.temb = temb
        self.xattn = xattn
        self.quirk = time_context_order == "sb"
        self.gn_part = None
        self.gn_cross = None
        self.gn_cross_valid = False
        self.trace = None


def _sigmoid(x):
    return 1.0 / (1.0 + math.exp(-x))


class _TimestepEmbedding(nn.Module):
    def __init__(self, in_channels, time_embed_dim, out_dim=None):
        super().__init__()
        self.linear_1 = nn.Linear(in_channels, time_embed_dim)
        self.linear_2 = nn.Linear(time_embed_dim, out_dim if out_dim is not None else time_embed_dim)


class _ResnetBlock2D(nn.Module):
    def __init__(self, cin, cout, temb, eps):
        super().__init__()
        self.norm1 = nn.GroupNorm(32, cin, eps=eps)
        self.conv1 = nn.Conv2d(cin, cout, 3, padding=1)
        self.time_emb_proj = nn.Linear(temb, cout)
        self.norm2 = nn.GroupNorm(32, cout, eps=eps)
        self.conv2 = nn.Conv2d(cout, cout, 3, padding=1)
        self.conv_shortcut = nn.Conv2d(cin, cout, 1) if cin != cout else None


class _TemporalResnetBlock(nn.Module):
    def __init__(self, c, temb, eps):
        super().__init__()
        self.norm1 = nn.GroupNorm(32, c, eps=eps)
        self.conv1 = nn.Conv3d(c, c, (3, 1, 1), padding=(1, 0, 0))
        self.time_emb_proj = nn.Linear(temb, c)
        self.norm2 = nn.GroupNorm(32, c, eps=eps)
        self.conv2 = nn.Conv3d(c, c, (3, 1, 1), padding=(1, 0, 0))


class _AlphaBlender(nn.Module):
    def __init__(self, alpha=0.5):
        super().__init__()
        self.mix_factor = nn.Parameter(torch.Tensor([alpha]))


class _Attention(nn.Module):
    def __init__(self, query_dim, heads, dim_head, cross_attention_dim=None):
        super().__init__()
        inner = heads * dim_head
        kv = cross_attention_dim if cross_attention_dim is not None else query_dim
        self.to_q = nn.Linear(query_dim, inner, bias=False)
        self.to_k = nn.Linear(kv, inner, bias=False)
        self.to_v = nn.Linear(kv, inner, bias=False)
        self.to_out = nn.ModuleList([nn.Linear(inner, query_dim), nn.Dropout(0.0)])


class _GEGLU(nn.Module):
    def __init__(self, dim_in, dim_out):
        super().__init__()
        self.proj = nn.Linear(dim_in, dim_out * 2)


class _FeedForward(nn.Module):
    def __init__(self, dim, dim_out=None):
        super().__init__()
        self.net = nn.ModuleList([_GEGLU(dim, dim * 4), nn.Dropout(0.0), nn.Linear(dim * 4, dim_out or dim)])


class _BasicTransformerBlock(nn.Module):
    def __init__(self, dim, heads, dim_head, cross_dim):
        super().__init__()
        self.norm1 = nn.LayerNorm(dim)
        self.attn1 = _Attention(dim, heads, dim_head)
        self.norm2 = nn.LayerNorm(dim)
        self.attn2 = _Attention(dim, heads, dim_head, cross_dim)
        self.norm3 = nn.LayerNorm(dim)
        self.ff = _FeedForward(dim)


class _TemporalBasicTransformerBlock(nn.Module):
    def __init__(self, dim, heads, dim_head, cross_dim):
        super().__init__()
        self.norm_in = nn.LayerNorm(dim)
        self.ff_in = _FeedForward(dim, dim)
        self.norm1 = nn.LayerNorm(dim)
        self.attn1 = _Attention(dim, heads, dim_head)
        self.norm2 = nn.LayerNorm(dim)
        self.attn2 = _Attention(dim, heads, dim_head, cross_dim)
        self.norm3 = nn.LayerNorm(dim)
        self.ff = _FeedForward(dim)


def _f32(t):
    return t.detach().float().contiguous()


def _lo(t):
    return getattr(t, "lo", None) if t is not None else None


def _trk_epi(epi, out):
    e = dict(epi)
    for k in ("R1", "R2"):
        if _lo(e.get(k)) is not None:
            e[k + "_lo"] = _lo(e[k])
    if _lo(out) is not None:
        e["out_lo"] = _lo(out)
    return e


_FF_FUSED = os.environ.get("CTRLV_FF_FUSED", "1") != "0"
_TEMPORAL_FUSED = os.environ.get("CTRLV_TEMPORAL_FUSED", "1") != "0"
_SPATIAL_ENTRY = os.environ.get("CTRLV_SPATIAL_ENTRY", "1") != "0"


def _ff_pair(ws, x, ffp, ubox, out, C, rows_per_image=0, **epi):
    wproj, bproj, wout, bout = ffp[:4]
    epi = _trk_epi(epi, out)
    if _FF_FUSED and len(ffp) == 6 and ops.ff_fused_serves(x, out, **epi):
        ops.ff_fused(x, ffp[4], ffp[5], out, bias=bout, **epi)
        return
    M = x.shape[0]
    if ubox[0] is None:
        ubox[0] = ws.alloc((M, 4 * C))
    u = ubox[0]
    ops.gemm(x, wproj, u, N=8 * C, cin=C, bias=bproj, geglu=1)
    ops.gemm(u, wout, out, N=C, cin=4 * C, bias=bout, rows_per_image=rows_per_image, **epi)


def _f8_weight(w):
    f8 = getattr(w, "f8", None)
    if f8 is None:
        f8 = w.f8 = ops.quant_rows_f8(w.contiguous())
    return f8


def _ff_f8_route(ws, xraw, ln, ffp, ubox, out, C, ln_V, ln_vdiv, ln_vmod, epi):
    wproj, bproj, wout, bout = ffp[:4]
    if wproj.shape[1] % 128 or wout.shape[1] % 128 or wout.shape[1] > 5120:
        return False
    M = xraw.shape[0]
    epi = _trk_epi(epi, out)
    (q1w, s1w), (q2w, s2w) = _f8_weight(wproj), _f8_weight(wout)
    if ubox[0] is None:
        ubox[0] = ws.alloc((M, 4 * C))
    u = ubox[0]
    mk = ws.mark()
    q = ws.alloc((M * 4 * C,), torch.uint8)
    qs = ws.alloc((M,), torch.float32)
    qa, qu = q[:M * C].view(M, C), q.view(M, 4 * C)
    if not (ops.gemm_f8_serves(qa, q1w, u, N=8 * C, cin=C, bias=bproj, geglu=1)
            and ops.gemm_f8_serves(qu, q2w, out, N=C, cin=4 * C, bias=bout, **epi)):
        ws.release(mk)
        return False
    ops.quant_rows_f8(xraw, qa, qs, ln=(ln[0], ln[1], 1e-5), V=ln_V, vdiv=ln_vdiv, vmod=ln_vmod)
    ops.gemm_f8(qa, qs, q1w, s1w, u, N=8 * C, cin=C, bias=bproj, geglu=1)
    ops.quant_rows_f8(u, qu, qs)
    ops.gemm_f8(qu, qs, q2w, s2w, out, N=C, cin=4 * C, bias=bout, **epi)
    ws.release(mk)
    return True


_FF_LN = os.environ.get("CTRLV_FF_LN", "0") not in ("", "0")


def _ln_ff(ws, xraw, ln, t, ffp, ubox, out, C, ln_V=None, ln_vdiv=1, ln_vmod=1 << 30, rows_per_image=0, **epi):
    if _FF_FUSED and _FF_LN and len(ffp) == 6 and _lo(xraw) is None and ops.ff_fused_serves(xraw, out, **_trk_epi(epi, out)):
        ops.ff_fused(xraw, ffp[4], ffp[5], out, bias=ffp[3], ln=(ln[0], ln[1], 1e-5), ln_V=ln_V, ln_vdiv=ln_vdiv,
                     ln_vmod=ln_vmod, **_trk_epi(epi, out))
        return
    if getattr(ws, "ff_f8", False) and _lo(xraw) is None and _ff_f8_route(ws, xraw, ln, ffp, ubox, out, C, ln_V, ln_vdiv, ln_vmod, epi):
        return
    if ln_V is not None:
        ops.layernorm(xraw, ln[0], ln[1], 1e-5, t, V=ln_V, vdiv=ln_vdiv, vmod=ln_vmod, x_lo=_lo(xraw))
    else:
        ops.layernorm(xraw, ln[0], ln[1], 1e-5, t, x_lo=_lo(xraw))
    _ff_pair(ws, t, ffp, ubox, out, C, rows_per_image=rows_per_image, **epi)


def _gn_scratch(ctx, n_img, S, C, ips):
    need = ops.groupnorm_scratch_floats(n_img, S, C, ips)
    if ctx.gn_part is None or ctx.gn_part.numel() < need:
        ctx.gn_part = torch.empty(max(need, 1 << 18), dtype=torch.float32, device=ctx.ws.device)
    return ctx.gn_part


def _gemm_groupnorm(ctx, A, W, out, gkw, n_img, S, C, ips, gamma, beta, eps, y):
    gkw = _trk_epi(gkw, out)
    if S % 64 == 0 and ops.gemm_gn_partials_serves(A, W, out, **gkw):
        need = ops.groupnorm_fused_scratch_floats(n_img, S, ips)
        if ctx.gn_part is None or ctx.gn_part.numel() < need:
            ctx.gn_part = torch.empty(max(need, 1 << 18), dtype=torch.float32, device=ctx.ws.device)
        ops.gemm(A, W, out, gn_partials=ctx.gn_part, **gkw)
        ops.groupnorm_from_partials(out, n_img, S, C, ips, gamma, beta, eps, True, y, ctx.gn_part, x_lo=_lo(out))
    else:
        ops.gemm(A, W, out, **gkw)
        ops.groupnorm(out, None, n_img, S, C, ips, gamma, beta, eps, True, y, _gn_scratch(ctx, n_img, S, C, ips),
                      x_lo=_lo(out))


class SpatioTemporalResBlock(nn.Module):
    def __init__(self, in_channels, out_channels, temb_channels, eps=1e-6):
        super().__init__()
        self.cin, self.cout, self.eps = in_channels, out_channels, eps
        self.spatial_res_block = _ResnetBlock2D(in_channels, out_channels, temb_channels, eps)
        self.temporal_res_block = _TemporalResnetBlock(out_channels, temb_channels, eps)
        self.time_mixer = _AlphaBlender(0.5)
        self.temb_off = None
        self._pk = None

    def temb_projections(self):
        return [self.spatial_res_block.time_emb_proj, self.temporal_res_block.time_emb_proj]

    def pack(self):
        s, t = self.spatial_res_block, self.temporal_res_block
        pk = dict(
            g1=_f32(s.norm1.weight), b1=_f32(s.norm1.bias), w1=packing.pack_conv3x3(s.conv1.weight),
            cb1=_f32(s.conv1.bias),
            g2=_f32(s.norm2.weight), b2=_f32(s.norm2.bias), w2=packing.pack_conv3x3(s.conv2.weight),
            cb2=_f32(s.conv2.bias),
            tg1=_f32(t.norm1.weight), tb1=_f32(t.norm1.bias), tw1=packing.pack_conv_temporal(t.conv1.weight),
            tcb1=_f32(t.conv1.bias),
            tg2=_f32(t.norm2.weight), tb2=_f32(t.norm2.bias), tw2=packing.pack_conv_temporal(t.conv2.weight),
            tcb2=_f32(t.conv2.bias),
            alpha=_sigmoid(float(self.time_mixer.mix_factor.detach().float().cpu())),
        )
        if s.conv_shortcut is not None:
            pk["wsc"] = packing.pack_linear(s.conv_shortcut.weight)
            pk["bsc"] = _f32(s.conv_shortcut.bias)
        self._pk = pk

    def run(self, ctx, x, H, W, x2=None, feeds_norm=False):
        pk, ws = self._pk, ctx.ws
        B, F = ctx.B, ctx.F
        N, S = B * F, H * W
        M = N * S
        cin, cout = self.cin, self.cout
        out = ws.trunk((M, cout))
        mk = ws.mark()
        part = _gn_scratch(ctx, N, S, max(cin, cout), 1)
        xn = ws.alloc((M, cin))
        ops.groupnorm(x, x2, N, S, cin, 1, pk["g1"], pk["b1"], self.eps, True, xn, part, x_lo=_lo(x), x2_lo=_lo(x2))
        h = ws.alloc((M, cout))
        vs = ctx.temb[:, self.temb_off[0]:]
        hn = ws.alloc((M, cout))
        _gemm_groupnorm(ctx, xn, pk["w1"], h, dict(N=cout, cin=cin, taps=9, mode=1, conv=(H, W, H, W, 1, 0), bias=pk["cb1"],
                                                   V=vs, vmode=1, vdiv=F * S),
                        N, S, cout, 1, pk["g2"], pk["b2"], self.eps, hn)
        if "wsc" in pk:
            res = ws.trunk((M, cout))
            ops.gemm(x, pk["wsc"], res, N=cout, cin=cin, A2=x2, c_split=x.shape[1] if x2 is not None else 0,
                     bias=pk["bsc"], out_lo=_lo(res))
        else:
            res = x
        xs = ws.trunk((M, cout))
        _gemm_groupnorm(ctx, hn, pk["w2"], xs, dict(N=cout, cin=cout, taps=9, mode=1, conv=(H, W, H, W, 1, 0), bias=pk["cb2"],
                                                    R1=res),
                        N, S, cout, F, pk["tg1"], pk["tb1"], self.eps, hn)
        vt = ctx.temb[:, self.temb_off[1]:]
        _gemm_groupnorm(ctx, hn, pk["tw1"], h, dict(N=cout, cin=cout, taps=3, mode=2, temporal=(F, S), bias=pk["tcb1"],
                                                    V=vt, vmode=1, vdiv=F * S),
                        N, S, cout, F, pk["tg2"], pk["tb2"], self.eps, hn)
        kw2 = _trk_epi(dict(N=cout, cin=cout, taps=3, mode=2, temporal=(F, S), bias=pk["tcb2"], s_acc=1.0 - pk["alpha"], R1=xs),
                       out)
        ctx.gn_cross_valid = False
        if feeds_norm and S % 64 == 0 and ops.gemm_gn_partials_serves(hn, pk["tw2"], out, **kw2):
            need = ops.groupnorm_fused_scratch_floats(N, S, 1)
            if ctx.gn_cross is None or ctx.gn_cross.numel() < need:
                ctx.gn_cross = torch.empty(need, dtype=torch.float32, device=ws.device)
            kw2["gn_partials"] = ctx.gn_cross
            ctx.gn_cross_valid = True
        ops.gemm(hn, pk["tw2"], out, **kw2)
        ws.release(mk)
        if ctx.trace is not None:
            ctx.trace.append((self, out.clone(), H, W))
        return out


class TransformerSpatioTemporalModel(nn.Module):
    def __init__(self, num_attention_heads, attention_head_dim, in_channels, cross_attention_dim):
        super().__init__()
        if attention_head_dim != 64:
            raise ValueError(f"ctrlv_amd attention kernels are specialised for head_dim 64 (got {attention_head_dim})")
        inner = num_attention_heads * attention_head_dim
        if inner != in_channels:
            raise ValueError("TransformerSpatioTemporalModel: inner_dim must equal in_channels (SVD configuration)")
        self.C, self.heads, self.cross_dim = in_channels, num_attention_heads, cross_attention_dim
        self.norm = nn.GroupNorm(32, in_channels, eps=1e-6)
        self.proj_in = nn.Linear(in_channels, inner)
        self.transformer_blocks = nn.ModuleList(
            [_BasicTransformerBlock(inner, num_attention_heads, attention_head_dim, cross_attention_dim)])
        self.temporal_transformer_blocks = nn.ModuleList(
            [_TemporalBasicTransformerBlock(inner, num_attention_heads, attention_head_dim, cross_attention_dim)])
        self.time_pos_embed = _TimestepEmbedding(in_channels, in_channels * 4, out_dim=in_channels)
        self.time_mixer = _AlphaBlender(0.5)
        self.proj_out = nn.Linear(inner, in_channels)
        self.xattn_off = None
        self._pk = None
        self._frame_emb = {}

    def cross_attentions(self):
        return [self.transformer_blocks[0].attn2, self.temporal_transformer_blocks[0].attn2]

    def pack(self):
        sb, tb = self.transformer_blocks[0], self.temporal_transformer_blocks[0]

        def ff(f):
            w, b = packing.pack_geglu(f.net[0].proj.weight, f.net[0].proj.bias)
            w2 = packing.pack_linear(f.net[2].weight)
            if tuple(w.shape) == (2560, 320) and tuple(w2.shape) == (320, 1280) and w.is_cuda:
                return (w, b, w2, _f32(f.net[2].bias)) + ops.ff_fused_pack(w.contiguous(), b.float().contiguous(), w2.contiguous())
            return w, b, w2, _f32(f.net[2].bias)

        def ln(n):
            return _f32(n.weight), _f32(n.bias)

        pk = dict(
            gn=(_f32(self.norm.weight), _f32(self.norm.bias)),
            pin=(packing.pack_linear(self.proj_in.weight), _f32(self.proj_in.bias)),
            pout=(packing.pack_linear(self.proj_out.weight), _f32(self.proj_out.bias)),
            s_ln1=ln(sb.norm1), s_ln3=ln(sb.norm3),
            s_qkv=packing.pack_qkv(merged_weight(sb.attn1.to_q), merged_weight(sb.attn1.to_k), merged_weight(sb.attn1.to_v)),
            s_o=(packing.pack_linear(merged_weight(sb.attn1.to_out[0])), _f32(sb.attn1.to_out[0].bias)),
            s_ff=ff(sb.ff),
# ... 256 lines not shown
```

ctrlv_amd/ops.py:

```python
import ctypes

import torch

from . import _lib, profiler as _prof
from ._lib import GemmDesc, check

_DT = {torch.float32: 0, torch.float16: 1, torch.bfloat16: 2}


def _stream():
    return ctypes.c_void_p(torch.cuda.current_stream().cuda_stream)


def _p(t):
    return None if t is None else ctypes.c_void_p(t.data_ptr())


def _L(*tensors):
    els = {t.dtype for t in tensors if t is not None and t.dtype in (torch.float16, torch.bfloat16)}
    if len(els) > 1:
        raise ValueError("ctrlv_amd: one call mixes bf16 and fp16 element tensors (a library serves ONE element type)")
    return _lib.load(torch.float16 if torch.float16 in els else None)


# ... 193 lines not shown
    elif mode == 0 and rows_per_image:
        d.S = rows_per_image
    d.ldo = out.stride(0)
    d.n_store = out.shape[1] if n_store is None else n_store
    d.ldr1 = R1.stride(0) if R1 is not None else 0
    d.ldr2 = R2.stride(0) if R2 is not None else 0
    d.s_acc, d.s1, d.s2 = s_acc, s1, s2
    d.vmode = vmode if V is not None else 0
    d.vdiv, d.vmod, d.vS = vdiv, vmod, vS
    d.ldv = V.stride(0) if V is not None else 0
    d.act, d.geglu, d.out_f32, d.tile = act, geglu, (_dbg if _dbg else (1 if out_f32 else 0)), tile
    if raw_out is not None:
        d.raw_out, d.ld_raw = _p(raw_out), raw_out.stride(0)
    d.n_scale2, d.s_acc2 = n_scale2, s_acc2
    d.gn_partials = _p(gn_partials)
    d.R1_lo, d.R2_lo, d.out_lo = _p(R1_lo), _p(R2_lo), _p(out_lo)
    d.pad_br = int(pad_br)
    return d


def gemm_splitk_slices(A, W, out, **kw):
    d = _gemm_desc(A, W, out, **kw)
    return max(1, _L(A, W).ctrlv_gemm_splitk_ws_bytes(ctypes.byref(d)) // (d.M * d.N * 4))


def gemm_gn_partials_serves(A, W, out, **kw):
    return bool(_L(A, W).ctrlv_gemm_gn_partials_serves(ctypes.byref(_gemm_desc(A, W, out, **kw))))


def gemm_up_phase_serves(A, W, out, **kw):
    return bool(_L(A, W).ctrlv_gemm_up_phase_serves(ctypes.byref(_gemm_desc(A, W, out, **kw))))


def pack_up_phase_weight(weight, dtype=torch.bfloat16):
    w = weight.detach().contiguous()
    _need_gpu(w, "weight")
    if w.dim() != 4 or tuple(w.shape[2:]) != (3, 3) or w.dtype not in _DT:
        raise ValueError(f"pack_up_phase_weight: expected a float [N, Cin, 3, 3] parameter, got {tuple(w.shape)} {w.dtype}")
    N, C = w.shape[:2]
    dst = torch.empty(4, N, 4 * C, dtype=dtype, device=w.device)
    check(_L(dst).ctrlv_pack_up_phase_weight(_p(w), _DT[w.dtype], N, C, _p(dst), _stream()), "ctrlv_pack_up_phase_weight")
    return dst


def gemm(A, W, out, **kw):
    d = _gemm_desc(A, W, out, **kw)
    _need_gpu(A, "A")
    lib = _L(A, W)
    if kw.get("splitk", True):
        need = lib.ctrlv_gemm_splitk_ws_bytes(ctypes.byref(d))
        if need:
            d.splitk_ws = _p(_scratch(A.device, need, "splitk", floor=64 << 20))
    cin, taps, mode, geglu = d.Cin, d.taps, d.mode, d.geglu
    wf = 1
    if mode == 1 and d.up == 2:
        taps, wf = 4, 4
    R1, R2, raw_out, act = kw.get("R1"), kw.get("R2"), kw.get("raw_out"), kw.get("act", 0)
    out_f32 = kw.get("out_f32", False)
    ev = _prof.begin()
    check(lib.ctrlv_gemm(ctypes.byref(d), _stream()), "ctrlv_gemm")
    if ev is not None:
        n_alg = d.N if geglu else min(d.N, d.n_store)
        fam = "gemm_conv3x3" if mode == 1 else ("gemm_conv_temporal" if mode == 2 else "gemm_linear")
        esz = 4 if out_f32 else 2
        n_out = d.n_store if not geglu else min(d.n_store, d.N // 2)
        nbytes = (d.M * cin * 2 * (1 if mode == 0 else 1) + d.M * n_out * esz + d.N * taps * cin * 2 * wf
                  + (d.M * n_out * 2 if R1 is not None else 0) + (d.M * n_out * 2 if R2 is not None else 0)
                  + (d.M * n_out * 2 if raw_out is not None else 0))
        _prof.end(ev, fam, 2.0 * d.M * n_alg * taps * cin, float(nbytes),
                  detail=(fam, d.M, d.N, taps * cin, int(geglu), int(R1 is not None) + int(R2 is not None), d.vmode, act))
    return out


def quant_rows_f8(x, q=None, scale=None, ln=None, V=None, vdiv=1, vmod=1 << 30):
    _need_gpu(x, "x")
    M, K = x.shape
    if x.stride(1) != 1:
        raise ValueError("quant_rows_f8: rows must be contiguous")
    if q is None:
        q = torch.empty(M, K, dtype=torch.uint8, device=x.device)
    if scale is None:
        scale = torch.empty(M, dtype=torch.float32, device=x.device)
    if q.dtype != torch.uint8 or scale.dtype != torch.float32 or q.shape[0] != M or scale.numel() < M or q.stride(1) != 1:
        raise ValueError("quant_rows_f8: q must be uint8 [M, >= K] and scale fp32 [M]")
    g, b, eps = (ln[0], ln[1], float(ln[2])) if ln is not None else (None, None, 0.0)
    ev = _prof.begin()
    check(_L(x).ctrlv_quant_rows_f8(_p(x), M, K, x.stride(0), _p(g), _p(b), eps, _p(V), vdiv, vmod,
                                    V.stride(0) if V is not None else 0, _p(q), q.stride(0), _p(scale), _stream()),
          "ctrlv_quant_rows_f8")
    _prof.end(ev, "layernorm", 0.0, 3.0 * M * K, detail=("quant_rows_f8", M, K, 0, 0, 0, 0, 0))
    return q, scale


def _gemm_f8_desc(A, W, out, *, N, cin, el=None, **kw):
    if A.dtype != torch.uint8 or W.dtype != torch.uint8:
        raise ValueError("gemm_f8: A and W hold e4m3 codes as uint8 (quant_rows_f8)")
    lib = _lib.load(el) if el is not None else _L(out, kw.get("R1"), kw.get("R2"))
    return _gemm_desc(A, W, out, N=N, cin=cin, **kw), lib


def gemm_f8_serves(A, W, out, **kw):
    d, lib = _gemm_f8_desc(A, W, out, **kw)
    return bool(lib.ctrlv_gemm_f8_serves(ctypes.byref(d)))


def gemm_f8(A, a_scale, W, w_scale, out, **kw):
    d, lib = _gemm_f8_desc(A, W, out, **kw)
    _need_gpu(A, "A")
    ev = _prof.begin()
    check(lib.ctrlv_gemm_f8(ctypes.byref(d), _p(a_scale), _p(w_scale), _stream()), "ctrlv_gemm_f8")
    if ev is not None:
        n_out = d.n_store if not d.geglu else min(d.n_store, d.N // 2)
        R1, R2 = kw.get("R1"), kw.get("R2")
        nbytes = d.M * d.Cin + d.N * d.Cin + d.M * n_out * (4 if kw.get("out_f32") else 2) * (1 + (R1 is not None) + (R2 is not None))
        _prof.end(ev, "gemm_linear", 2.0 * d.M * d.N * d.Cin, float(nbytes),
                  detail=("gemm_f8", d.M, d.N, d.Cin, int(d.geglu), int(R1 is not None) + int(R2 is not None), d.vmode, 0))
    return out


def ff_fused_pack(w1_packed, b1, w2_packed):
    _need_gpu(w1_packed, "w1_packed")
    assert tuple(w1_packed.shape) == (2560, 320) and tuple(w2_packed.shape) == (320, 1280) and b1.numel() == 2560
    assert w1_packed.dtype in (torch.bfloat16, torch.float16) and w2_packed.dtype == w1_packed.dtype and b1.dtype == torch.float32
    assert w1_packed.is_contiguous() and w2_packed.is_contiguous() and b1.is_contiguous()
    lib = _L(w1_packed)
    w1f = torch.empty(lib.ctrlv_ff_fused_w1f_bytes() // 2, dtype=w1_packed.dtype, device=w1_packed.device)
    w2f = torch.empty_like(w2_packed)
    check(lib.ctrlv_ff_fused_pack(_p(w1_packed), _p(b1), _p(w2_packed), _p(w1f), _p(w2f), _stream()), "ctrlv_ff_fused_pack")
    return w1f, w2f


def _ff_out_desc(out, bias=None, R1=None, s1=1.0, R2=None, s2=1.0, s_acc=1.0, V=None, vmode=0, vdiv=1, vmod=1 << 30, vS=1,
                 R1_lo=None, R2_lo=None, out_lo=None):
    _need_rows("ff_fused", out=out, R1=R1, R2=R2, V=V, R1_lo=R1_lo, R2_lo=R2_lo, out_lo=out_lo)
    d = GemmDesc()
    d.out, d.bias, d.R1, d.R2, d.V = _p(out), _p(bias), _p(R1), _p(R2), _p(V)
    d.R1_lo, d.R2_lo, d.out_lo = _p(R1_lo), _p(R2_lo), _p(out_lo)
    d.M, d.N, d.Cin, d.taps, d.mode = out.shape[0], out.shape[1], 4 * out.shape[1], 1, 0
    d.ldo, d.n_store = out.stride(0), out.shape[1]
    d.ldr1 = R1.stride(0) if R1 is not None else 0
    d.ldr2 = R2.stride(0) if R2 is not None else 0
    d.s_acc, d.s1, d.s2 = s_acc, s1, s2
    d.vmode = vmode if V is not None else 0
    d.vdiv, d.vmod, d.vS = vdiv, vmod, vS
    d.ldv = V.stride(0) if V is not None else 0
    return d


def ff_fused_serves(x, out, **epi):
    d = _ff_out_desc(out, **{k: v for k, v in epi.items() if k != "bias"})
    return bool(_L(x).ctrlv_ff_fused_serves(ctypes.byref(d), x.stride(0)))


def ff_fused(x, w1f, w2f, out, *, bias=None, R1=None, s1=1.0, R2=None, s2=1.0, s_acc=1.0, V=None, vmode=0, vdiv=1,
             vmod=1 << 30, vS=1, ln=None, ln_V=None, ln_vdiv=1, ln_vmod=1 << 30, R1_lo=None, R2_lo=None, out_lo=None):
    _need_rows("ff_fused", x=x, ln_V=ln_V)
    d = _ff_out_desc(out, bias, R1, s1, R2, s2, s_acc, V, vmode, vdiv, vmod, vS, R1_lo, R2_lo, out_lo)
    _need_gpu(x, "x")
    ev = _prof.begin()
    if ln is None:
        check(_L(x).ctrlv_ff_fused(_p(x), x.stride(0), _p(w1f), _p(w2f), ctypes.byref(d), _stream()),
              "ctrlv_ff_fused")
    else:
        check(_L(x).ctrlv_ff_fused_ln(_p(x), x.stride(0), _p(ln[0]), _p(ln[1]), float(ln[2]), _p(ln_V), ln_vdiv,
                                      ln_vmod, ln_V.stride(0) if ln_V is not None else 0, _p(w1f), _p(w2f),
                                      ctypes.byref(d), _stream()), "ctrlv_ff_fused_ln")
    if ev is not None:
        M = out.shape[0]
        nbytes = M * 320 * 2 * (2 + (R1 is not None) + (R2 is not None))
        _prof.end(ev, "gemm_linear", 2.0 * M * 320 * (2560 + 1280), float(nbytes),
                  detail=("ff_fused", M, 320, 320, 1, int(R1 is not None) + int(R2 is not None), d.vmode, 0))
    return out


def groupnorm_chunks(n_img, S, C, imgs_per_stat):
    rc = _lib.load().ctrlv_groupnorm_chunks(n_img, S, C, imgs_per_stat)
    if rc < 0:
        check(rc, "ctrlv_groupnorm_chunks")
    return rc


def groupnorm_scratch_floats(n_img, S, C, imgs_per_stat):
    return (n_img * groupnorm_chunks(n_img, S, C, imgs_per_stat) + n_img // imgs_per_stat) * 64


def groupnorm_fused_scratch_floats(n_img, S, imgs_per_stat):
    return (n_img * (S // 64) + n_img // imgs_per_stat) * 64


def groupnorm_from_partials(x, n_img, S, C, imgs_per_stat, gamma, beta, eps, silu, y, partials, x_lo=None):
    _need_dense("groupnorm_from_partials", x=x, x_lo=x_lo, y=y, partials=partials, gamma=gamma, beta=beta)
    _need_gpu(x, "x")
    assert partials.numel() >= groupnorm_fused_scratch_floats(n_img, S, imgs_per_stat)
    ev = _prof.begin()
    check(_L(x).ctrlv_groupnorm_from_partials_split(_p(x), _p(x_lo), n_img, S, C, imgs_per_stat, eps, _p(partials), _p(gamma),
                                                    _p(beta), 1 if silu else 0, _p(y), _stream()),
          "ctrlv_groupnorm_from_partials")
    _prof.end(ev, "groupnorm", 0.0, 2.0 * 2 * n_img * S * C)
    return y


def groupnorm(x, x2, n_img, S, C, imgs_per_stat, gamma, beta, eps, silu, y, partials, x_lo=None, x2_lo=None):
    _need_dense("groupnorm", x=x, x2=x2, x_lo=x_lo, x2_lo=x2_lo, y=y, partials=partials, gamma=gamma, beta=beta)
    _need_gpu(x, "x")
    lib = _L(x)
    c_split = x.shape[1] if x2 is not None else 0
    st = _stream()
    ev = _prof.begin()
    check(lib.ctrlv_groupnorm_stats_split(_p(x), _p(x_lo), _p(x2), _p(x2_lo), c_split, n_img, S, C, imgs_per_stat, eps,
                                          _p(partials), st), "ctrlv_groupnorm_stats")
    check(lib.ctrlv_groupnorm_apply_split(_p(x), _p(x_lo), _p(x2), _p(x2_lo), c_split, n_img, S, C, imgs_per_stat,
                                          _p(partials), _p(gamma), _p(beta), 1 if silu else 0, _p(y), st),
          "ctrlv_groupnorm_apply")
    _prof.end(ev, "groupnorm", 0.0, 2.0 * 2 * n_img * S * C)
    return y


def layernorm(x, gamma, beta, eps, y, V=None, vdiv=1, vmod=1 << 30, x_lo=None):
    _need_dense("layernorm", x=x, x_lo=x_lo, y=y, gamma=gamma, beta=beta)
    _need_rows("layernorm", V=V)
    _need_gpu(x, "x")
    M, C = x.shape
    ev = _prof.begin()
    check(_L(x).ctrlv_layernorm_split(_p(x), _p(x_lo), M, C, _p(gamma), _p(beta), eps, _p(V), vdiv, vmod,
                                      V.stride(0) if V is not None else 0, _p(y), _stream()), "ctrlv_layernorm")
    _prof.end(ev, "layernorm", 0.0, 2.0 * 2 * M * C)
    return y


Q_PRESCALE = 0.125 * 1.44269504088896340736


def attention_spatial(qkv, out, n_img, S, C, prescaled=False):
    _need_dense("attention_spatial", qkv=qkv, out=out)
    _need_gpu(qkv, "qkv")
    ev = _prof.begin()
    fn = _L(qkv).ctrlv_attention_spatial_prescaled if prescaled else _L(qkv).ctrlv_attention_spatial
    check(fn(_p(qkv), _p(out), n_img, S, C, _stream()), "ctrlv_attention_spatial")
    _prof.end(ev, "attention_spatial", 4.0 * n_img * (C // 64) * S * S * 64, 2.0 * 4 * n_img * S * C)
    return out


def attention_spatial_lse(qkv, out, lse, n_img, S, C):
    _need_dense("attention_spatial_lse", qkv=qkv, out=out, lse=lse)
    _need_gpu(qkv, "qkv")
    ev = _prof.begin()
    check(_L(qkv).ctrlv_attention_spatial_lse(_p(qkv), _p(out), _p(lse), n_img, S, C, _stream()),
          "ctrlv_attention_spatial_lse")
    _prof.end(ev, "attention_spatial", 4.0 * n_img * (C // 64) * S * S * 64, 2.0 * 4 * n_img * S * C)
    return out


def attention_spatial_bwd(qkv, out, dout, lse, dqkv, n_img, S, C):
    _need_dense("attention_spatial_bwd", qkv=qkv, out=out, dout=dout, lse=lse, dqkv=dqkv)
    _need_gpu(qkv, "qkv")
    delta = torch.empty(_L(qkv).ctrlv_attention_bwd_scratch_floats(n_img, S, C), dtype=torch.float32, device=qkv.device)
    ev = _prof.begin()
    check(_L(qkv).ctrlv_attention_spatial_bwd(_p(qkv), _p(out), _p(dout), _p(lse), _p(dqkv), _p(delta), n_img, S, C,
                                                  _stream()), "ctrlv_attention_spatial_bwd")
    _prof.end(ev, "attention_spatial_bwd", 14.0 * n_img * (C // 64) * S * S * 64, 2.0 * 8 * n_img * S * C)
    return dqkv


def attention_temporal_bwd(qkv, out, dout, dqkv, B, F, S, C):
    _need_dense("attention_temporal_bwd", qkv=qkv, out=out, dout=dout, dqkv=dqkv)
    _need_gpu(qkv, "qkv")
    ev = _prof.begin()
    check(_L(qkv).ctrlv_attention_temporal_bwd(_p(qkv), _p(out), _p(dout), _p(dqkv), B, F, S, C, _stream()),
          "ctrlv_attention_temporal_bwd")
    _prof.end(ev, "attention_temporal_bwd", 14.0 * B * S * (C // 64) * F * F * 64, 2.0 * 8 * B * F * S * C)
    return dqkv


def attention_temporal(qkv, out, B, F, S, C):
    _need_dense("attention_temporal", qkv=qkv, out=out)
    _need_gpu(qkv, "qkv")
    ev = _prof.begin()
    check(_L(qkv).ctrlv_attention_temporal(_p(qkv), _p(out), B, F, S, C, _stream()), "ctrlv_attention_temporal")
    _prof.end(ev, "attention_temporal", 4.0 * B * S * (C // 64) * F * F * 64, 2.0 * 4 * B * F * S * C)
    return out


def attention_tokens(qkv, out, n_img, S, C, head_dim):
    _need_gpu(qkv, "qkv")
    if qkv.stride(0) != 3 * C or out.stride(0) != C or qkv.stride(1) != 1 or out.stride(1) != 1:
        raise ValueError("attention_tokens: qkv [rows, 3C] and out [rows, C] must be dense row-major")
    if qkv.shape[0] < n_img * S or out.shape[0] < n_img * S:
        raise ValueError(f"attention_tokens: {n_img} x {S} rows do not fit qkv {tuple(qkv.shape)} / out {tuple(out.shape)}")
    ev = _prof.begin()
    check(_L(qkv, out).ctrlv_attention_tokens(_p(qkv), _p(out), n_img, S, C, head_dim, _stream()), "ctrlv_attention_tokens")
    _prof.end(ev, "attention_tokens", 4.0 * n_img * S * S * C, 2.0 * 4 * n_img * S * C)
    return out


def clip_patch_rows(pixels, patch, rows):
    _need_gpu(pixels, "pixels")
    if pixels.dim() != 4 or pixels.shape[1] != 3 or not pixels.is_contiguous() or pixels.dtype not in _DT:
        raise ValueError("clip_patch_rows: pixels must be contiguous (n, 3, H, W) in fp32 / fp16 / bf16")
    n, _, H, W = pixels.shape
    if patch <= 0 or H % patch or W % patch or rows.shape[0] != n * (H // patch) * (W // patch) or rows.stride(1) != 1:
        raise ValueError(f"clip_patch_rows: image {H}x{W}, patch {patch}, rows {tuple(rows.shape)}")
    ev = _prof.begin()
    check(_L(rows).ctrlv_clip_patch_rows(_p(pixels), _DT[pixels.dtype], n, H, W, patch, _p(rows), rows.stride(0), _stream()),
          "ctrlv_clip_patch_rows")
    _prof.end(ev, "clip_patch_rows", 0.0, float(pixels.numel() * pixels.element_size() + rows.numel() * 2))
    return rows
# ... 679 lines not shown
```

include/ctrlv_hip.h:

```cpp
#ifndef CTRLV_HIP_H
#define CTRLV_HIP_H

#include <stddef.h>
#include <stdint.h>

#ifdef __cplusplus
extern "C" {
#endif

typedef void* ctrlv_stream_t;

enum {
  CTRLV_OK = 0,
  CTRLV_E_BAD_ARG = -1,
  CTRLV_E_BAD_SHAPE = -2,
  CTRLV_E_HIP = -3,
  CTRLV_E_BAD_DTYPE = -4,
  CTRLV_E_WORKSPACE = -5,
};

int ctrlv_abi_version(void);
int ctrlv_elem_dtype(void);
int ctrlv_build_id(char* buf, size_t n);
int ctrlv_last_error(char* buf, size_t n);

typedef struct ctrlv_gemm_desc {
  const void* A;
  const void* A2;
  const void* W;
  void* out;
  const float* bias;
  const void* R1;
  const void* R2;
  const float* V;
  int32_t M, N, Cin, taps;
  int32_t lda, lda2, c_split;
  int32_t mode;
  int32_t H, Wd, Ho, Wo, stride, up;
  int32_t F, S;
  int32_t ldo, n_store;
  int32_t ldr1, ldr2;
  float s_acc, s1, s2;
  int32_t vmode;
  int32_t vdiv, vmod, vS, ldv;
  int32_t act;
  int32_t geglu;
  int32_t out_f32;
  int32_t tile;
  int32_t ld_raw;
  int32_t pad_br;
  void* raw_out;
  int32_t n_scale2;
  float s_acc2;
  float* gn_partials;
  void* splitk_ws;
  int32_t ksplit, w_cin;
  const void* R1_lo;
  const void* R2_lo;
  void* out_lo;
} ctrlv_gemm_desc;

int ctrlv_gemm(const ctrlv_gemm_desc* d, ctrlv_stream_t stream);
size_t ctrlv_gemm_splitk_ws_bytes(const ctrlv_gemm_desc* d);
int ctrlv_gemm_gn_partials_serves(const ctrlv_gemm_desc* d);
int ctrlv_gemm_up_phase_serves(const ctrlv_gemm_desc* d);
int ctrlv_pack_up_phase_weight(const void* w, int dtype, int N, int Cin, void* dst, ctrlv_stream_t stream);

int ctrlv_groupnorm_chunks(int n_img, int S, int C, int imgs_per_stat);
int ctrlv_groupnorm_stats(const void* x, const void* x2, int c_split, int n_img, int S, int C, int imgs_per_stat,
                          float eps, float* partials, ctrlv_stream_t stream);
int ctrlv_groupnorm_apply(const void* x, const void* x2, int c_split, int n_img, int S, int C, int imgs_per_stat,
                          const float* partials, const float* gamma, const float* beta, int silu, void* y,
                          ctrlv_stream_t stream);
int ctrlv_groupnorm_from_partials(const void* x, int n_img, int S, int C, int imgs_per_stat, float eps, float* partials,
                                  const float* gamma, const float* beta, int silu, void* y, ctrlv_stream_t stream);
int ctrlv_groupnorm_from_partials_split(const void* x, const void* x_lo, int n_img, int S, int C, int imgs_per_stat, float eps,
                                        float* partials, const float* gamma, const float* beta, int silu, void* y,
                                        ctrlv_stream_t stream);
int ctrlv_groupnorm_finalize(int n_img, int S, int C, int imgs_per_stat, float eps, float* partials, ctrlv_stream_t stream);
int ctrlv_groupnorm_stats_split(const void* x, const void* x_lo, const void* x2, const void* x2_lo, int c_split, int n_img,
                                int S, int C, int imgs_per_stat, float eps, float* partials, ctrlv_stream_t stream);
int ctrlv_groupnorm_apply_split(const void* x, const void* x_lo, const void* x2, const void* x2_lo, int c_split, int n_img,
                                int S, int C, int imgs_per_stat, const float* partials, const float* gamma,
                                const float* beta, int silu, void* y, ctrlv_stream_t stream);

int ctrlv_layernorm(const void* x, int M, int C, const float* gamma, const float* beta, float eps,
                    const float* V, int vdiv, int vmod, int ldv, void* y, ctrlv_stream_t stream);
int ctrlv_layernorm_split(const void* x, const void* x_lo, int M, int C, const float* gamma, const float* beta, float eps,
                          const float* V, int vdiv, int vmod, int ldv, void* y, ctrlv_stream_t stream);

int ctrlv_ff_fused_w1f_bytes(void);
int ctrlv_ff_fused_pack(const void* w1_packed, const float* b1, const void* w2_packed, void* w1f, void* w2f,
                        ctrlv_stream_t stream);
int ctrlv_ff_fused(const void* x, int ldx, const void* w1f, const void* w2f, const ctrlv_gemm_desc* out_desc,
                   ctrlv_stream_t stream);
int ctrlv_ff_fused_ln(const void* x, int ldx, const float* ln_gamma, const float* ln_beta, float ln_eps,
                      const float* ln_V, int ln_vdiv, int ln_vmod, int ln_ldv, const void* w1f, const void* w2f,
                      const ctrlv_gemm_desc* out_desc, ctrlv_stream_t stream);
int ctrlv_ff_fused_serves(const ctrlv_gemm_desc* out_desc, int ldx);

int ctrlv_quant_rows_f8(const void* x, int M, int K, int ldx, const float* gamma, const float* beta, float eps,
                        const float* V, int vdiv, int vmod, int ldv, void* q, int ldq, float* scale, ctrlv_stream_t stream);
int ctrlv_gemm_f8(const ctrlv_gemm_desc* d, const float* a_scale, const float* w_scale, ctrlv_stream_t stream);
int ctrlv_gemm_f8_serves(const ctrlv_gemm_desc* d);

typedef struct ctrlv_temporal_fused_desc {
  const void* x; int32_t ldx;
  const void* wf;
  const float* bias;
  const void* R1; const void* R1_lo; int32_t ldr1;
  const float* V; int32_t vmode, vdiv, vmod, vS, ldv;
  void* out; void* out_lo; int32_t ldo;
  int32_t B, F, S, C;
  const float* ln_gamma; const float* ln_beta; float ln_eps;
} ctrlv_temporal_fused_desc;
size_t ctrlv_temporal_fused_weight_bytes(void);
int ctrlv_temporal_fused_pack(const void* wqkv_packed, int ld_qkv, const void* wo_packed, int ld_o, void* wf,
                              ctrlv_stream_t stream);
int ctrlv_temporal_fused(const ctrlv_temporal_fused_desc* d, ctrlv_stream_t stream);
int ctrlv_temporal_fused_serves(const ctrlv_temporal_fused_desc* d);

typedef struct ctrlv_spatial_entry_desc {
  const void* x; const void* x_lo; int32_t ldx;
  const void* wf;
  const float* bias_in; const float* bias_qkv;
  const float* stats;
  const float* gn_gamma; const float* gn_beta;
  const float* ln_gamma; const float* ln_beta; float ln_eps;
  void* h0; void* h0_lo; int32_t ldh;
  void* qkv; int32_t ldq;
  int32_t n_img, S, C, head_dim;
  float q_scale;
} ctrlv_spatial_entry_desc;
size_t ctrlv_spatial_entry_fused_weight_bytes(void);
int ctrlv_spatial_entry_fused_pack(const void* win_packed, int ld_in, const void* wqkv_packed, int ld_qkv, void* wf,
                                   ctrlv_stream_t stream);
int ctrlv_spatial_entry_fused(const ctrlv_spatial_entry_desc* d, ctrlv_stream_t stream);
int ctrlv_spatial_entry_fused_serves(const ctrlv_spatial_entry_desc* d);

int ctrlv_softmax_rows(const float* scores, int rows, int cols, long ld_scores, void* probs, long ld_probs,
                       ctrlv_stream_t stream);
int ctrlv_softmax_rows_bwd(const void* probs, long ld_probs, const float* dprobs, long ld_dprobs, int rows, int cols,
                           float scale, void* dscores, long ld_dscores, ctrlv_stream_t stream);

int ctrlv_attention_spatial(const void* qkv, void* out, int n_img, int S, int C, ctrlv_stream_t stream);
int ctrlv_attention_spatial_prescaled(const void* qkv, void* out, int n_img, int S, int C, ctrlv_stream_t stream);
int ctrlv_attention_temporal(const void* qkv, void* out, int B, int F, int S, int C, ctrlv_stream_t stream);
int ctrlv_attention_spatial_lse(const void* qkv, void* out, float* lse, int n_img, int S, int C, ctrlv_stream_t stream);
size_t ctrlv_attention_bwd_scratch_floats(int n_img, int S, int C);
int ctrlv_attention_spatial_bwd(const void* qkv, const void* out, const void* dout, const float* lse, void* dqkv,
                                float* delta, int n_img, int S, int C, ctrlv_stream_t stream);
int ctrlv_attention_temporal_bwd(const void* qkv, const void* out, const void* dout, void* dqkv, int B, int F, int S, int C,
                                 ctrlv_stream_t stream);

int ctrlv_attention_tokens(const void* qkv, void* out, int n_img, int S, int C, int head_dim, ctrlv_stream_t stream);
int ctrlv_clip_patch_rows(const void* pixels, int dtype_code, int n, int Hpx, int Wpx, int patch, void* rows, int ld,
                          ctrlv_stream_t stream);
int ctrlv_clip_tokens(const void* patch_out, const float* class_emb, const float* pos_emb, int n, int P, int C, void* out,
                      ctrlv_stream_t stream);
int ctrlv_act_rows(void* x, int M, int N, int ld, int kind, ctrlv_stream_t stream);

typedef struct ctrlv_gemm_tokens_desc {
  const void* A;
  const void* W;
  const float* bias;
  const void* R1;
  void* out;
  void* workspace;
  size_t workspace_bytes;
  int32_t M, N, K;
  int32_t lda, ldr1, ldo;
  int32_t act;
  int32_t ws_zeroed;
} ctrlv_gemm_tokens_desc;
int ctrlv_gemm_tokens(const ctrlv_gemm_tokens_desc* d, ctrlv_stream_t stream);
int ctrlv_gemm_tokens_plan(int N, int K, int* bn, int* slices);
size_t ctrlv_gemm_tokens_ws_bytes(int M, int N, int K);

int ctrlv_nchw_to_rows(const void* src, int src_dtype, int n_img, int C, int HW, void* dst, int ldc, int c_off,
                       ctrlv_stream_t stream);
int ctrlv_rows_to_nchw(const void* src, int ldc, int n_img, int C, int HW, void* dst, int dst_dtype,
                       ctrlv_stream_t stream);
int ctrlv_time_conv_rows_to_nchw(const void* src, int ldc, int n_frames, int C, int HW, const float* weight,
                                 const float* bias, void* dst, int dst_dtype, ctrlv_stream_t stream);
int ctrlv_vae_posterior(const void* rows, int ld, int n_img, int L, int HW, const float* quant_weight, const float* quant_bias,
                        const float* noise, float scale, void* moments_out, void* latents_out, int out_dtype,
                        ctrlv_stream_t stream);
#define CTRLV_TIME_CONV_BWD_SCRATCH_FLOATS 16384
int ctrlv_time_conv_rows_to_nchw_bwd(const float* dout, const void* src, int ldc_src, int n_frames, int clip_frames, int C,
                                     int HW, const float* weight, void* drows, int ldc, float* dweight, float* dbias,
                                     float* scratch, ctrlv_stream_t stream);
int ctrlv_im2col3x3(const void* x, int n_img, int H, int W, int Cp, void* col, int Kp, ctrlv_stream_t stream);
int ctrlv_axpby(const void* x, const void* r, float a, float b, void* y, size_t n, ctrlv_stream_t stream);
int ctrlv_axpby_split(const void* x, const void* x_lo, const void* r, float a, float b, void* y, void* y_lo, size_t n,
                      ctrlv_stream_t stream);
int ctrlv_timestep_embedding(const float* t, int n, int dim, void* out, ctrlv_stream_t stream);
int ctrlv_silu(const void* x, void* y, size_t n, ctrlv_stream_t stream);
int ctrlv_cfg_euler_step(float* latents, const void* noise_pred, int pred_dtype, int cfg, const float* guidance,
                         int B, int F, int CHW, float sigma, float sigma_next, void* scaled_next,
                         ctrlv_stream_t stream);

size_t ctrlv_gemm_wgrad_scratch_bytes(const ctrlv_gemm_desc* fwd);
int ctrlv_gemm_wgrad(const ctrlv_gemm_desc* fwd, const void* dY, int ldy, float* dW, float* dbias, float scale,
                     int torch_layout, void* scratch, size_t scratch_bytes, ctrlv_stream_t stream);
int ctrlv_pack_weight(const void* src, int src_dtype, int N, int C, int taps, int form, int geglu, void* dst, int ld_dst,
                      ctrlv_stream_t stream);
size_t ctrlv_colsum_scratch_floats(int M, int N, int vmode, int vdiv);
int ctrlv_colsum(const void* x, int M, int N, int ldx, int vmode, int vdiv, int vmod, float scale, float* out, int ldo,
                 float* scratch, ctrlv_stream_t stream);
int ctrlv_dot_diff(const void* dy, const void* p, const void* q, size_t n, float scale, float* out, float* scratch,
                   ctrlv_stream_t stream);
int ctrlv_groupnorm_bwd_scratch_floats(int n_img, int S, int C, int imgs_per_stat);
int ctrlv_groupnorm_bwd(const void* x, const void* dy, int n_img, int S, int C, int imgs_per_stat,
                        const float* fwd_partials, const float* gamma, const float* beta, int silu, void* dx,
                        float* dgamma, float* dbeta, float* scratch, ctrlv_stream_t stream);
int ctrlv_groupnorm_bwd_add(const void* x, const void* dy, const void* add, int n_img, int S, int C, int imgs_per_stat,
                            const float* fwd_partials, const float* gamma, const float* beta, int silu, void* dx,
                            float* dgamma, float* dbeta, float* scratch, ctrlv_stream_t stream);

size_t ctrlv_layernorm_bwd_scratch_floats(int M, int C);
int ctrlv_layernorm_bwd(const void* x, const void* dy, int M, int C, const float* gamma, float eps, const float* V, int vdiv,
                        int vmod, int ldv, void* dx, float* dgamma, float* dbeta, float* scratch, ctrlv_stream_t stream);
int ctrlv_layernorm_bwd_add(const void* x, const void* dy, const void* add, int M, int C, const float* gamma, float eps,
                            const float* V, int vdiv, int vmod, int ldv, void* dx, float* dgamma, float* dbeta, float* scratch,
                            ctrlv_stream_t stream);
int ctrlv_geglu_bwd(const void* raw, const void* du, size_t M, int I, void* draw, ctrlv_stream_t stream);

typedef struct ctrlv_lora_desc {
  const void* X;
  const void* dY;
  const float* A;
  const float* B;
  float* dA;
  float* dB;
  int M, Cin, N;
  int g, r;
  int ldx, ldy;
  float scale;
} ctrlv_lora_desc;
size_t ctrlv_lora_grad_scratch_bytes(const ctrlv_lora_desc* d);
int ctrlv_lora_grad(const ctrlv_lora_desc* d, void* scratch, size_t scratch_bytes, ctrlv_stream_t stream);
int ctrlv_lora_merge(const void* W, int w_dtype, const float* A, const float* B, int N, int Cin, int r, float scale,
                     float* out, ctrlv_stream_t stream);

#define CTRLV_MAX_BLOCKS 8
typedef struct ctrlv_model_config {
  int32_t kind;
  int32_t in_channels;
  int32_t out_channels;
  int32_t n_blocks;
  int32_t block_out_channels[CTRLV_MAX_BLOCKS];
  int32_t down_cross_attn[CTRLV_MAX_BLOCKS];
// ... 322 lines not shown
```

Baseline: 4.755 steps/s.

## Enable LayerNorm fusion into fused FF kernel by default with LDS-staged gamma/beta

Turns on by default the path that folds the LayerNorm in front of the feed-forward block into the fused FF kernel, so the separate layernorm launch and its intermediate tensor round trip are dropped. The in-kernel LN is reworked into a two-pass mean/variance whose rounding matches the standalone layernorm. Gamma and beta are now staged into LDS via buffer-to-LDS loads, and the kernel gets separate specializations with and without a row-vector table. Routing moves the fp8 FF path ahead of the fused-LN path and excludes split trunk planes, with new alignment checks. The risks are extra register and LDS pressure in the fused kernel and the longer two-pass reduction.

```diff
diff --git a/ctrlv_amd/_lib.py b/ctrlv_amd/_lib.py
--- a/ctrlv_amd/_lib.py
+++ b/ctrlv_amd/_lib.py
@@ -206,6 +206,7 @@
     "ctrlv_ff_fused_w1f_bytes": (c_int, []),
     "ctrlv_ff_fused_pack": (c_int, [c_void_p, c_void_p, c_void_p, c_void_p, c_void_p, c_void_p]),
     "ctrlv_ff_fused_serves": (c_int, [ctypes.POINTER(GemmDesc), c_int]),
+    "ctrlv_ff_fused_ln_serves": (c_int, [ctypes.POINTER(GemmDesc), c_int]),
     "ctrlv_ff_fused": (c_int, [c_void_p, c_int, c_void_p, c_void_p, ctypes.POINTER(GemmDesc), c_void_p]),
     "ctrlv_ff_fused_ln": (c_int, [c_void_p, c_int, c_void_p, c_void_p, c_float, c_void_p, c_int, c_int, c_int, c_void_p,
                                   c_void_p, ctypes.POINTER(GemmDesc), c_void_p]),
@@ -385,7 +386,7 @@
 _libs = {}
 _tls = threading.local()
 _NO_STATUS = {"ctrlv_abi_version", "ctrlv_elem_dtype", "ctrlv_build_id", "ctrlv_last_error", "ctrlv_ff_fused_w1f_bytes",
-              "ctrlv_gemm_gn_partials_serves", "ctrlv_gemm_up_phase_serves", "ctrlv_ff_fused_serves", "ctrlv_plan_num_down_residuals",
+              "ctrlv_gemm_gn_partials_serves", "ctrlv_gemm_up_phase_serves", "ctrlv_ff_fused_serves", "ctrlv_ff_fused_ln_serves", "ctrlv_plan_num_down_residuals",
               "ctrlv_temporal_fused_serves", "ctrlv_gemm_f8_serves", "ctrlv_spatial_entry_fused_serves",
               "ctrlv_gemm_tokens_ws_bytes", "ctrlv_clip_plan_workspace_bytes", "ctrlv_vae_plan_workspace_bytes",
               "ctrlv_pipeline_workspace_bytes", "ctrlv_pipeline_boxes_workspace_bytes", "ctrlv_box_frames_post_ws_bytes",
diff --git a/ctrlv_amd/csrc/abi.hip b/ctrlv_amd/csrc/abi.hip
--- a/ctrlv_amd/csrc/abi.hip
+++ b/ctrlv_amd/csrc/abi.hip
@@ -32,7 +32,7 @@
     if (d.gn_rows < 32 || d.gn_rows > 1024) d.gn_rows = 256;
     d.ln_rows = env("CTRLV_LN_ROWS", 1);
     d.ff_fused = env("CTRLV_FF_FUSED", 1);
-    d.ff_ln = env("CTRLV_FF_LN", 0);
+    d.ff_ln = env("CTRLV_FF_LN", 1);
     d.pp_balanced = env("CTRLV_PP_BALANCED", 1);
     d.pp_cgrp = env("CTRLV_PP_CGRP", 0);
     d.attn_rows = env("CTRLV_ATTN_ROWS", 0);
diff --git a/ctrlv_amd/csrc/common.h b/ctrlv_amd/csrc/common.h
--- a/ctrlv_amd/csrc/common.h
+++ b/ctrlv_amd/csrc/common.h
@@ -79,6 +79,24 @@
   v.x = pack_elx2(f[0], f[1]); v.y = pack_elx2(f[2], f[3]);
   v.z = pack_elx2(f[4], f[5]); v.w = pack_elx2(f[6], f[7]);
   return v;
+}
+__device__ __forceinline__ float ln_mean(float sum, float inv_c) {
+#pragma clang fp contract(off)
+  return sum * inv_c;
+}
+__device__ __forceinline__ float ln_sq_add(float sq, float f, float mean) {
+#pragma clang fp contract(off)
+  const float dl = f - mean;
+  return __builtin_fmaf(dl, dl, sq);
+}
+__device__ __forceinline__ float ln_rstd(float sq_sum, float inv_c, float eps) {
+  return rsqrtf(__builtin_fmaf(sq_sum, inv_c, eps));
+}
+__device__ __forceinline__ float ln_apply(float f, float mean, float rstd, float g, float b) {
+#pragma clang fp contract(off)
+  float o = __builtin_fmaf((f - mean) * rstd, g, b);
+  asm volatile("" : "+v"(o));
+  return o;
 }
 typedef uint8_t lo_t;
 __device__ __forceinline__ uint2 split_lo8(const float* v, const uint4& hi) {
diff --git a/ctrlv_amd/csrc/ff_fused.hip b/ctrlv_amd/csrc/ff_fused.hip
--- a/ctrlv_amd/csrc/ff_fused.hip
+++ b/ctrlv_amd/csrc/ff_fused.hip
@@ -31,7 +31,13 @@
   const float* lnv; int ln_vdiv, ln_vmod, ln_ldv;
 };
 
-template <int EPI, bool LO = false, bool LN = false>
+__device__ __forceinline__ void pin(elx8& v) { asm volatile("" : "+v"(v)); }
+__device__ __forceinline__ float swap_sum(float v) {
+  auto r = __builtin_amdgcn_permlane32_swap(__float_as_uint(v), __float_as_uint(v), false, false);
+  return __uint_as_float(r[0]) + __uint_as_float(r[1]);
+}
+
+template <int EPI, bool LO = false, int LN = 0>
 __global__ __launch_bounds__(512) void ff_fused_kernel(const FfArgs a) {
 #if defined(__HIP_DEVICE_COMPILE__)
   extern __shared__ __attribute__((aligned(1024))) char smem[];
@@ -81,6 +87,9 @@
   int gbase = 0;
   elx8 xr[20];
   u32x4_t ini_b, ini_v;
+  const __amdgpu_buffer_rsrc_t rsLg = __builtin_amdgcn_make_buffer_rsrc((void*)(LN ? a.ln_g : (const float*)a.w1f), 0, LN ? kC * 4 : 0, 0x00020000);
+  const __amdgpu_buffer_rsrc_t rsLb = __builtin_amdgcn_make_buffer_rsrc((void*)(LN ? a.ln_b : (const float*)a.w1f), 0, LN ? kC * 4 : 0, 0x00020000);
+  constexpr int kTileLoads = 22;
   const __amdgpu_buffer_rsrc_t rsVt = __builtin_amdgcn_make_buffer_rsrc(
       (void*)(a.vtab ? a.vtab : (const float*)a.w1f), 0, a.vtab ? (int)((long)a.vmod * a.ldv * 4) : 0, 0x00020000);
   auto tile_loads = [&](int tile) {
@@ -93,6 +102,7 @@
     ini_b = __builtin_amdgcn_raw_buffer_load_b128(rsB2, col4, 0, 0);
     ini_v = __builtin_amdgcn_raw_buffer_load_b128(rsVt, col4, a.vtab ? ((bm / a.vdiv) % a.vmod) * (a.ldv * 4) : 0, 0);
   };
+  auto stg_of = [&](int w) { return smem + kStgOff + w * 4096; };
   tile_loads(blockIdx.x);
   for (int tile = blockIdx.x; tile < tiles; tile += G, gbase += kChunks) {
     const int bm = tile * kTileM;
@@ -100,55 +110,73 @@
 #ifdef CTRLV_FF_STAMP
     unsigned long long st_tb; asm volatile("s_memtime %0\n\ts_waitcnt lgkmcnt(0)" : "=s"(st_tb)::"memory");
 #endif
-    if constexpr (LN) {
-      const float* lv = a.lnv ? a.lnv + (long)((m / a.ln_vdiv) % a.ln_vmod) * a.ln_ldv + 8 * hsel : nullptr;
+    if constexpr (LN != 0) {
+      char* const lns = stg_of(wid);
+#pragma unroll
+      for (int pc = 0; pc < 2; ++pc) {
+        __builtin_amdgcn_raw_ptr_buffer_load_lds(rsLg, LDS_PTR(lns + pc * 1024), 16, pc * 1024 + lane * 16, 0, 0, 0);
+        __builtin_amdgcn_raw_ptr_buffer_load_lds(rsLb, LDS_PTR(lns + 2048 + pc * 1024), 16, pc * 1024 + lane * 16, 0, 0, 0);
+      }
+      const float* lv = nullptr;
+      if constexpr (LN == 2) lv = a.lnv + (long)((m / a.ln_vdiv) % a.ln_vmod) * a.ln_ldv + 8 * hsel;
       auto raw8 = [&](int ks, float* f) {
+        pin(xr[ks]);
         unpack_elx8(__builtin_bit_cast(uint4, xr[ks]), f);
-        if (lv) {
+        if constexpr (LN == 2) {
           const float4 p = *(const float4*)(lv + ks * 16), q = *(const float4*)(lv + ks * 16 + 4);
           f[0] += p.x; f[1] += p.y; f[2] += p.z; f[3] += p.w; f[4] += q.x; f[5] += q.y; f[6] += q.z; f[7] += q.w;
         }
       };
-      float pilot;
-      {
-        float f0[8];
-        raw8(0, f0);
-        pilot = __shfl(f0[0], r32);
-      }
-      float sm = 0.f, sq = 0.f;
+      auto fence = [&](int ks) { if (LN == 1 || (ks & 3) == 3) __builtin_amdgcn_sched_barrier(0); };
+      constexpr float inv_c = 1.0f / kC;
+      float ps[4] = {0.f, 0.f, 0.f, 0.f};
 #pragma unroll
       for (int ks = 0; ks < 20; ++ks) {
         float f[8];
         raw8(ks, f);
 #pragma unroll
-        for (int e = 0; e < 8; ++e) { const float dl = f[e] - pilot; sm += dl; sq += dl * dl; }
-        if (ks % 5 == 4) __builtin_amdgcn_sched_barrier(0);
-      }
-      sm += __shfl_xor(sm, 32);
-      sq += __shfl_xor(sq, 32);
-      const float dm = sm * (1.0f / kC);
-      const float var = sq * (1.0f / kC) - dm * dm;
-      const float mean = pilot + dm, rstd = rsqrtf((var > 0.f ? var : 0.f) + a.ln_eps);
-      const float* gp = a.ln_g + 8 * hsel;
-      const float* bp = a.ln_b + 8 * hsel;
+        for (int e = 0; e < 8; ++e) ps[ks & 3] += f[e];
+        fence(ks);
+      }
+      float mean = ln_mean(swap_sum((ps[0] + ps[2]) + (ps[1] + ps[3])), inv_c);
+      asm volatile("" : "+v"(mean) : : "memory");
+      float pq[4] = {0.f, 0.f, 0.f, 0.f};
 #pragma unroll
       for (int ks = 0; ks < 20; ++ks) {
         float f[8];
         raw8(ks, f);
-        const float4 g0 = *(const float4*)(gp + ks * 16), g1 = *(const float4*)(gp + ks * 16 + 4);
-        const float4 b0 = *(const float4*)(bp + ks * 16), b1v = *(const float4*)(bp + ks * 16 + 4);
+#pragma unroll
+        for (int e = 0; e < 8; ++e) pq[ks & 3] = ln_sq_add(pq[ks & 3], f[e], mean);
+        fence(ks);
+      }
+      float rstd = ln_rstd(swap_sum((pq[0] + pq[2]) + (pq[1] + pq[3])), inv_c, a.ln_eps);
+      asm volatile("" : "+v"(rstd) : : "memory");
+      wait_vmcnt<0>();
+      const unsigned ga = (unsigned)(unsigned long)LDS_PTR(lns) + 32u * hsel;
+#pragma unroll
+      for (int ks = 0; ks < 20; ++ks) {
+        f32x4 g0, g1, b0, b1;
+        asm volatile("ds_read_b128 %0, %1 offset:%2" : "=v"(g0) : "v"(ga), "n"(ks * 64) : "memory");
+        asm volatile("ds_read_b128 %0, %1 offset:%2" : "=v"(g1) : "v"(ga), "n"(ks * 64 + 16) : "memory");
+        asm volatile("ds_read_b128 %0, %1 offset:%2" : "=v"(b0) : "v"(ga), "n"(2048 + ks * 64) : "memory");
+        asm volatile("ds_read_b128 %0, %1 offset:%2" : "=v"(b1) : "v"(ga), "n"(2048 + ks * 64 + 16) : "memory");
+        float f[8], o[8];
+        raw8(ks, f);
+        asm volatile("s_waitcnt lgkmcnt(0)" : "+v"(g0), "+v"(g1), "+v"(b0), "+v"(b1));
         const float gg[8] = {g0.x, g0.y, g0.z, g0.w, g1.x, g1.y, g1.z, g1.w};
-        const float bb[8] = {b0.x, b0.y, b0.z, b0.w, b1v.x, b1v.y, b1v.z, b1v.w};
-#pragma unroll
-        for (int e = 0; e < 8; ++e) f[e] = (f[e] - mean) * rstd * gg[e] + bb[e];
-        uint4 o = pack_elx8(f);
-        if (!(m < M)) o = make_uint4(0, 0, 0, 0);
-        xr[ks] = __builtin_bit_cast(elx8, o);
-        if (ks % 5 == 4) __builtin_amdgcn_sched_barrier(0);
-      }
+        const float bb[8] = {b0.x, b0.y, b0.z, b0.w, b1.x, b1.y, b1.z, b1.w};
+#pragma unroll
+        for (int e = 0; e < 8; ++e) o[e] = ln_apply(f[e], mean, rstd, gg[e], bb[e]);
+        uint4 pk = pack_elx8(o);
+        if (!(m < M)) pk = make_uint4(0, 0, 0, 0);
+        xr[ks] = __builtin_bit_cast(elx8, pk);
+        pin(xr[ks]);
+        fence(ks);
+      }
+      asm volatile("s_waitcnt lgkmcnt(0)" ::: "memory");
     }
     f32x16 acc[1][5];
-    char* const stg = smem + kStgOff + wid * 4096;
+    char* const stg = stg_of(wid);
     {
       const f32x4 b = __builtin_bit_cast(f32x4, ini_b), w = __builtin_bit_cast(f32x4, ini_v);
       if (lane < 40) *(float4*)(stg + lane * 16) = make_float4(b.x + w.x, b.y + w.y, b.z + w.z, b.w + w.w);
@@ -316,7 +344,7 @@
     slot_barrier(false);
     if (hh == 0) {
       FSTAMP(b0);
-      wait_vmcnt<22>();
+      wait_vmcnt<kTileLoads>();
       lds_done_barrier();
 #ifdef CTRLV_FF_STAMP
       FSTAMP(b1);
@@ -376,7 +404,7 @@
   }
 }
 
-template <int EPI, bool LO, bool LN>
+template <int EPI, bool LO, int LN>
 int launch_ff_ln(const FfArgs& a, hipStream_t stream) {
   static bool attr_set[CTRLV_MAX_DEVICES] = {};
   auto kfn = ff_fused_kernel<EPI, LO, LN>;
@@ -399,7 +427,10 @@
 
 template <int EPI, bool LO = false>
 int launch_ff(const FfArgs& a, hipStream_t stream) {
-  return a.ln_g ? launch_ff_ln<EPI, LO, true>(a, stream) : launch_ff_ln<EPI, LO, false>(a, stream);
+  if constexpr (!LO) {
+    if (a.ln_g) return a.lnv ? launch_ff_ln<EPI, LO, 2>(a, stream) : launch_ff_ln<EPI, LO, 1>(a, stream);
+  }
+  return launch_ff_ln<EPI, LO, 0>(a, stream);
 }
 
 }
@@ -464,8 +495,9 @@
   CTRLV_CHECK_ARG(x && w1f && w2f && out_desc && out_desc->out, "ctrlv_ff_fused: null pointer");
   CTRLV_CHECK_ARG((ln_gamma == nullptr) == (ln_beta == nullptr), "ctrlv_ff_fused: LayerNorm needs gamma and beta");
 #ifndef CTRLV_FF_STAMP
-  CTRLV_CHECK_ARG(!ln_V || (ln_gamma && ln_vdiv > 0 && ln_vmod > 0 && ln_ldv >= 320 && ln_ldv % 4 == 0),
+  CTRLV_CHECK_ARG(!ln_V || (ln_gamma && ln_vdiv > 0 && ln_vmod > 0 && ln_ldv >= 320 && ln_ldv % 4 == 0 && ((uintptr_t)ln_V & 15) == 0),
                   "ctrlv_ff_fused: bad LayerNorm row-vector table");
+  CTRLV_CHECK_ARG(!ln_gamma || (((uintptr_t)ln_gamma | (uintptr_t)ln_beta) & 3) == 0, "ctrlv_ff_fused: unaligned gamma / beta");
 #endif
   FfArgs a;
   a.ln_g = ln_gamma; a.ln_b = ln_beta; a.ln_eps = ln_eps;
@@ -481,6 +513,7 @@
     a.o.vmode = 0; a.o.V = nullptr;
   }
   const ctrlv_gemm_desc& d = a.o;
+  CTRLV_CHECK_ARG(!(ln_gamma && pp_split_io(d)), "ctrlv_ff_fused_ln: split trunk planes keep ctrlv_layernorm in front of ctrlv_ff_fused");
   hipStream_t st = (hipStream_t)stream;
 #ifdef CTRLV_ELEM_F16
   if (pp_split_io(d)) {
@@ -511,3 +544,8 @@
   if (ff_check(*out_desc, ldx, false, &fold) != CTRLV_OK) return 0;
   return (out_desc->act || (out_desc->out_f32 & 1)) ? 0 : 1;
 }
+
+extern "C" int ctrlv_ff_fused_ln_serves(const ctrlv_gemm_desc* out_desc, int ldx) {
+  if (!ctrlv_ff_fused_serves(out_desc, ldx)) return 0;
+  return pp_split_io(*out_desc) ? 0 : 1;
+}
diff --git a/ctrlv_amd/csrc/norm.hip b/ctrlv_amd/csrc/norm.hip
--- a/ctrlv_amd/csrc/norm.hip
+++ b/ctrlv_amd/csrc/norm.hip
@@ -405,14 +405,14 @@
       for (int e = 0; e < 8; ++e) sm += f[k][e];
     }
     for (int o = LPR >> 1; o > 0; o >>= 1) sm += __shfl_xor(sm, o);
-    const float mean = sm * inv_c;
+    const float mean = ln_mean(sm, inv_c);
     float sq = 0.f;
 #pragma unroll
     for (int k = 0; k < NCH; ++k)
 #pragma unroll
-      for (int e = 0; e < 8; ++e) { const float dl = f[k][e] - mean; sq += dl * dl; }
+      for (int e = 0; e < 8; ++e) sq = ln_sq_add(sq, f[k][e], mean);
     for (int o = LPR >> 1; o > 0; o >>= 1) sq += __shfl_xor(sq, o);
-    const float rstd = rsqrtf(sq * inv_c + eps);
+    const float rstd = ln_rstd(sq, inv_c, eps);
     if (ok) {
 #pragma unroll
       for (int k = 0; k < NCH; ++k) {
@@ -423,7 +423,7 @@
         const float bb[8] = {b0.x, b0.y, b0.z, b0.w, b1.x, b1.y, b1.z, b1.w};
         float o[8];
 #pragma unroll
-        for (int e = 0; e < 8; ++e) o[e] = (f[k][e] - mean) * rstd * gg[e] + bb[e];
+        for (int e = 0; e < 8; ++e) o[e] = ln_apply(f[k][e], mean, rstd, gg[e], bb[e]);
         *(uint4*)(y + m * C + c0) = pack_elx8(o);
       }
     }
diff --git a/ctrlv_amd/csrc/plan.hip b/ctrlv_amd/csrc/plan.hip
--- a/ctrlv_amd/csrc/plan.hip
+++ b/ctrlv_amd/csrc/plan.hip
@@ -517,12 +517,6 @@
 
 int ln_ff(Ctx& c, const FeedFwd& f, const Norm& nm, const Trk& xraw, const float* lnV, int lnvdiv, int lnvmod, int lnldv,
           el_t* tt, const ctrlv_gemm_desc& proj, const ctrlv_gemm_desc& outd, int C, el_t** u) {
-  if (ctrlv_debug().ff_fused && ctrlv_debug().ff_ln && f.w1f && !xraw.lo && ctrlv_ff_fused_serves(&outd, C)) {
-    return c.launch({CTRLV_FAM_GEMM_LINEAR, 2.0 * outd.M * 320.0 * (2560 + 1280),
-                     (double)outd.M * 320 * 2 * (2 + (outd.R1 ? 1 : 0) + (outd.R2 ? 1 : 0)), outd.M, 320, 320, 0x300}, [&] {
-      return ctrlv_ff_fused_ln(xraw.hi, C, nm.g, nm.b, 1e-5f, lnV, lnvdiv, lnvmod, lnldv, f.w1f, f.w2f, &outd, c.st);
-    });
-  }
   if (c.p->ff_precision == 1 && f.proj8 && f.out8 && !xraw.lo) {
     ctrlv_gemm_desc p8 = proj, o8 = outd;
     p8.W = f.proj8; o8.W = f.out8; o8.lda = 4 * C; o8.S = 0;
@@ -552,6 +546,12 @@
       c.release(mk);
       return rc;
     }
+  }
+  if (ctrlv_debug().ff_fused && ctrlv_debug().ff_ln && f.w1f && !xraw.lo && ctrlv_ff_fused_ln_serves(&outd, C)) {
+    return c.launch({CTRLV_FAM_GEMM_LINEAR, 2.0 * outd.M * 320.0 * (2560 + 1280),
+                     (double)outd.M * 320 * 2 * (2 + (outd.R1 ? 1 : 0) + (outd.R2 ? 1 : 0)), outd.M, 320, 320, 0x300}, [&] {
+      return ctrlv_ff_fused_ln(xraw.hi, C, nm.g, nm.b, 1e-5f, lnV, lnvdiv, lnvmod, lnldv, f.w1f, f.w2f, &outd, c.st);
+    });
   }
   CTRLV_TRY(layernorm(c, xraw, proj.M, C, nm, tt, lnV, lnvdiv, lnvmod, lnldv));
   return ff_pair(c, f, proj, outd, C, u);
diff --git a/ctrlv_amd/models/blocks.py b/ctrlv_amd/models/blocks.py
--- a/ctrlv_amd/models/blocks.py
+++ b/ctrlv_amd/models/blocks.py
@@ -176,15 +176,15 @@
     return True
 
 
-_FF_LN = os.environ.get("CTRLV_FF_LN", "0") not in ("", "0")
+_FF_LN = os.environ.get("CTRLV_FF_LN", "1") not in ("", "0")
 
 
 def _ln_ff(ws, xraw, ln, t, ffp, ubox, out, C, ln_V=None, ln_vdiv=1, ln_vmod=1 << 30, rows_per_image=0, **epi):
-    if _FF_FUSED and _FF_LN and len(ffp) == 6 and _lo(xraw) is None and ops.ff_fused_serves(xraw, out, **_trk_epi(epi, out)):
+    if getattr(ws, "ff_f8", False) and _lo(xraw) is None and _ff_f8_route(ws, xraw, ln, ffp, ubox, out, C, ln_V, ln_vdiv, ln_vmod, epi):
+        return
+    if _FF_FUSED and _FF_LN and len(ffp) == 6 and _lo(xraw) is None and ops.ff_fused_ln_serves(xraw, out, **_trk_epi(epi, out)):
         ops.ff_fused(xraw, ffp[4], ffp[5], out, bias=ffp[3], ln=(ln[0], ln[1], 1e-5), ln_V=ln_V, ln_vdiv=ln_vdiv,
                      ln_vmod=ln_vmod, **_trk_epi(epi, out))
-        return
-    if getattr(ws, "ff_f8", False) and _lo(xraw) is None and _ff_f8_route(ws, xraw, ln, ffp, ubox, out, C, ln_V, ln_vdiv, ln_vmod, epi):
         return
     if ln_V is not None:
         ops.layernorm(xraw, ln[0], ln[1], 1e-5, t, V=ln_V, vdiv=ln_vdiv, vmod=ln_vmod, x_lo=_lo(xraw))
diff --git a/ctrlv_amd/ops.py b/ctrlv_amd/ops.py
--- a/ctrlv_amd/ops.py
+++ b/ctrlv_amd/ops.py
@@ -369,6 +369,11 @@
     return bool(_L(x).ctrlv_ff_fused_serves(ctypes.byref(d), x.stride(0)))
 
 
+def ff_fused_ln_serves(x, out, **epi):
+    d = _ff_out_desc(out, **{k: v for k, v in epi.items() if k != "bias"})
+    return bool(_L(x).ctrlv_ff_fused_ln_serves(ctypes.byref(d), x.stride(0)))
+
+
 def ff_fused(x, w1f, w2f, out, *, bias=None, R1=None, s1=1.0, R2=None, s2=1.0, s_acc=1.0, V=None, vmode=0, vdiv=1,
              vmod=1 << 30, vS=1, ln=None, ln_V=None, ln_vdiv=1, ln_vmod=1 << 30, R1_lo=None, R2_lo=None, out_lo=None):
     _need_rows("ff_fused", x=x, ln_V=ln_V)
diff --git a/include/ctrlv_hip.h b/include/ctrlv_hip.h
--- a/include/ctrlv_hip.h
+++ b/include/ctrlv_hip.h
@@ -98,6 +98,7 @@
                       const float* ln_V, int ln_vdiv, int ln_vmod, int ln_ldv, const void* w1f, const void* w2f,
                       const ctrlv_gemm_desc* out_desc, ctrlv_stream_t stream);
 int ctrlv_ff_fused_serves(const ctrlv_gemm_desc* out_desc, int ldx);
+int ctrlv_ff_fused_ln_serves(const ctrlv_gemm_desc* out_desc, int ldx);
 
 int ctrlv_quant_rows_f8(const void* x, int M, int K, int ldx, const float* gamma, const float* beta, float eps,
                         const float* V, int vdiv, int vmod, int ldv, void* q, int ldq, float* scale, ctrlv_stream_t stream);
```

Result: no change. 4.776 steps/s, median of 6 (+0.4%).
